# w111liang222/lidar-slam-detection

Measured on AMD Instinct MI355X. Metric: registered points/sec (120k-pt scan vs 1e7-pt map, full iterate-to-converge), higher is better.
Workload: dtype f32 per-point geometry / f64 transforms and reductions

## Files before the change

include/lio_hip.h:

```cpp
#ifndef LIO_HIP_H_
#define LIO_HIP_H_

#include <stdint.h>

#ifdef __cplusplus
extern "C" {
#endif

#define LIO_OK 0
#define LIO_E_INVALID (-1)
#define LIO_E_CAPACITY (-2)
#define LIO_E_DEVICE (-3)
#define LIO_E_STATE (-4)

typedef struct lio_map lio_map;
typedef struct lio_scan lio_scan;
typedef struct lio_engine lio_engine;

const char* lio_last_error(void);
const char* lio_last_warning(void);
int lio_device_count(void);
#define LIO_ABI_VERSION 26
int lio_abi_version(void);
void* lio_pinned_alloc(uint64_t bytes);
void lio_pinned_free(void* p);
uint64_t lio_map_bytes(const lio_map*);

lio_map* lio_map_create(int device, float resolution, uint64_t max_points, uint64_t max_voxels, int stencil);
void lio_map_destroy(lio_map*);
int lio_map_set_stencil(lio_map*, int stencil);
int lio_map_insert(lio_map*, const float* world_xyzi, uint64_t n, double travel);
int lio_map_insert_device(lio_map*, const void* d_world_xyzi, uint64_t n, double travel);
int lio_map_clear(lio_map*);
int lio_map_set_lru(lio_map*, uint64_t capacity_voxels, double max_distance);
int lio_map_lru_stats(lio_map*, uint64_t* n_evicted, uint64_t* n_interleaved);
int lio_map_lru_exact_stats(lio_map*, uint64_t* n_recreated, uint64_t* n_batches_not_followed);
int lio_map_set_tie_mode(lio_map*, int mode);
int lio_map_tie_stats(lio_map*, uint64_t* n_boundary_ties, uint64_t* n_unresolved);
int lio_map_pool_stats(lio_map*, uint64_t* pool_top, uint64_t* pool_cap);
int lio_map_stats(lio_map*, uint64_t* n_points, uint64_t* n_voxels);
uint64_t lio_map_knn_candidates(lio_map*);
uint64_t lio_map_knn_touched(lio_map*);
uint64_t lio_map_knn_unique(lio_map*);
int64_t lio_map_dump(lio_map*, float* out_xyzi, uint64_t cap_points);
int lio_map_knn(lio_map*, const float* world_xyzi, uint32_t n, float* out_pts, int32_t* out_cnt);

lio_scan* lio_scan_create(int device, uint32_t max_raw, uint32_t max_ds);
void lio_scan_destroy(lio_scan*);
int lio_scan_reset(lio_scan*);
int lio_scan_upload(lio_scan*, const float* body_xyzi, uint32_t n_raw);
int lio_scan_set_device(lio_scan*, const void* d_body_xyzi, uint32_t n_raw);
int lio_scan_undistort_delta(lio_scan*, const uint32_t* stamp_us, int stamps_on_device, const float delta_pose[16], double scan_period);
int lio_scan_download_raw(lio_scan*, float* out_xyzi, uint32_t cap);
int lio_scan_undistort_poses(lio_scan*, const uint32_t* stamp_us, int stamps_on_device, uint64_t header_stamp_us, const uint64_t* pose_stamp_us,
                             const double* pose_T, uint32_t n_poses);
int lio_scan_undistort_imu(lio_scan*, const uint32_t* stamp_us, int stamps_on_device, const double* poses, uint32_t n_poses, const double* end_pos3,
                           const double* end_rot_xyzw, const double* ril_xyzw, const double* til3, double blind, int filter_num, int undistort);
int lio_scan_voxel_downsample(lio_scan*, float leaf, int sync, uint32_t* n_ds);
int lio_scan_voxel_downsample_batch(lio_scan** scans, int n, float leaf, uint32_t* n_ds);
int lio_scan_set_ds(lio_scan*, const float* ds_body_xyzi, uint32_t n_ds);
int lio_scan_num_ds(lio_scan*);
int lio_scan_download_ds(lio_scan*, float* out_xyzi, uint32_t cap);
int lio_scan_download_world(lio_scan*, float* out_xyzi, uint32_t cap);
const void* lio_scan_ds_device(lio_scan*, uint32_t* n);
int lio_scan_download_match(lio_scan*, uint8_t* selected, float* normvec, int32_t* nn_cnt, float* nn_pts);

typedef struct lio_kernel_times {
    double knn_us, linearize_us, finalize_us;
    uint32_t knn_launches, linearize_launches, finalize_launches;
    uint32_t pad;
} lio_kernel_times;
int lio_scan_enable_kernel_timing(lio_scan*, int on);
int lio_scan_kernel_times(lio_scan*, lio_kernel_times* out, int reset);

typedef struct lio_normal_eq {
    double JtJ[36];
    double Jtr[6];
    double nnT[9];
    double eigvec[9];
    double eigval[3];
    double contri[3];
    double strong[3];
    double sum_abs_res;
    uint32_t n_eff;
    uint32_t n_ds;
    uint32_t n_knn_candidates_lo, n_knn_candidates_hi;
    uint32_t n_tie;
    uint32_t seq;
} lio_normal_eq;

int lio_p2plane_linearize(lio_map*, lio_scan*, const double pose_wi[7], const double ext_il[7], int redo_knn,
                          lio_normal_eq* out);
int lio_scan_set_degeneracy_mode(lio_scan*, int mode);
int lio_p2plane_degeneracy(lio_scan*, const double V[9], double contri[3], double strong[3]);
int lio_p2plane_rows(lio_scan*, const double pose_wi[7], const double ext_il[7], double* h_x6, double* h, uint32_t cap_rows);
int lio_map_incremental(lio_map*, lio_scan*, const double pose_wi[7], const double ext_il[7], float map_leaf,
                        int ekf_inited, double travel);
int lio_map_seed(lio_map*, lio_scan*, const double pose_wi[7], const double ext_il[7], double travel);

lio_engine* lio_engine_create(int device, float resolution, int stencil, uint64_t max_points, uint64_t max_voxels,
                              uint32_t max_raw, uint32_t max_ds);
lio_engine* lio_engine_create_shared(lio_map* shared_map, uint32_t max_raw, uint32_t max_ds);
void lio_engine_destroy(lio_engine*);
lio_map* lio_engine_map(lio_engine*);
lio_scan* lio_engine_scan(lio_engine*);
// ... 19 lines not shown
    float downsample_us, knn_us, linearize_us, insert_us, total_device_us;
    float host_solve_us, total_wall_us;
    int32_t n_knn_pass, n_pass, n_ds, n_eff_last;
    int32_t n_added;
    uint64_t knn_candidates;
    float undistort_us;
    float imu_host_us;
} lio_timings;
int lio_engine_timings(lio_engine*, lio_timings* out);
int lio_engine_enable_timing(lio_engine*, int on);
int lio_engine_flush(lio_engine*);
#define LIO_MAIN_FIRST_SCAN 0
#define LIO_MAIN_SEEDED 1
#define LIO_MAIN_SKIPPED 2
#define LIO_MAIN_UPDATED 3
#define LIO_MAIN_IMU_INIT 4
#define LIO_MAIN_IDLE 5
int lio_fastlio_init(lio_engine*, const double extT[3], const double extR[9], int filter_num, int max_point_num, double scan_period,
                     int undistort);
int lio_fastlio_is_init(lio_engine*);
int lio_fastlio_imu_enqueue(lio_engine*, double stamp, const double gyr[3], const double acc_ms2[3]);
int lio_engine_set_device_loop(lio_engine*, int on);

int lio_fastlio_ins_enqueue(lio_engine*, double stamp, const double vel_imu[3]);
int lio_fastlio_set_wheelspeed(lio_engine*, int enable);
int lio_fastlio_pcl_enqueue(lio_engine*, const float* xyzi, const uint32_t* stamp_us, uint32_t n, double header_stamp);
int lio_fastlio_pcl_stage(lio_engine*, uint32_t n, float** xyzi, uint32_t** stamp_us);
int lio_fastlio_pcl_commit(lio_engine*, uint32_t n, double header_stamp);
int lio_fastlio_pcl_enqueue_device(lio_engine*, const void* d_xyzi, const void* d_stamp_us, uint32_t n, double header_stamp);
int lio_fastlio_main(lio_engine*);
int lio_fastlio_odometry(lio_engine*, double odom_s[16], double odom_e[16]);
int lio_fastlio_state(lio_engine*, double out[20]);
int lio_fastlio_start_state(lio_engine*, double s26[26]);
int lio_fastlio_download_undistorted(lio_engine*, float* out_xyzi, uint32_t cap, uint32_t* n);
typedef int (*lio_meas_fn)(void* ctx, const double* s26, int converge, int* n, double* rows6, double* h, int cap);
int lio_eskf_update_cb(const double s26[26], const double P[529], double R, int max_iter, lio_meas_fn fn, void* ctx, int cap, double s26_out[26],
                       double P_out[529]);
int lio_eskf_update_ws_cb(const double s26[26], const double P[529], double R, int max_iter, lio_meas_fn fn, void* ctx, int cap, const double* ins_vel,
                          int degenerate, double s26_out[26], double P_out[529]);
int lio_state_predict(const double s26[26], const double P[529], double dt, const double Q[12], const double acc[3], const double gyro[3],
                      double s26_out[26], double P_out[529]);
typedef int (*lio_sums_fn)(void* ctx, const double* s26, int converge, double* acc29);
typedef void (*lio_degeneracy_fn)(void* ctx, const double* V9, double* cs6);
int lio_eskf_update_sums_cb(const double s26[26], const double P[529], double R, int max_iter, int degenerate_detect_en, lio_sums_fn fn,
                            lio_degeneracy_fn dfn, void* ctx, double s26_out[26], double P_out[529], lio_pass_log* logs, int cap_logs, int* status);

typedef void (*lio_reduce_fn)(void* ctx, double* buf, int n);
int lio_engine_set_reduce_hook(lio_engine*, lio_reduce_fn fn, void* ctx);
typedef struct lio_comm lio_comm;
int lio_comm_unique_id(uint8_t id[128]);
lio_comm* lio_comm_init(int device, int rank, int world, const uint8_t id[128]);
void lio_comm_destroy(lio_comm*);
int lio_comm_rank(const lio_comm*);
int lio_comm_world(const lio_comm*);
int lio_allgather_normal_eq(lio_comm*, const double* d_local32, double* d_gathered, double* d_sum32, void* stream);
int lio_allgather_records(lio_comm*, const double* d_local, double* d_gathered, uint32_t n_records, void* stream);
int lio_comm_stats(lio_comm*, uint64_t* n_collectives, double* total_us);
int lio_engine_set_joint(lio_engine* e, lio_engine** others, int n_others, lio_comm* comm);
int lio_engine_joint_register(lio_engine* e, const float* raw_body_xyzi, uint32_t n_raw, double lidar_beg_time, double state26[26], double cov[529]);
int lio_engine_joint_register_device(lio_engine* e, const void* d_raw_body_xyzi, uint32_t n_raw, double lidar_beg_time, double state26[26], double cov[529]);
#define LIO_JOB_KEEP_CACHE 1u
#define LIO_JOB_IDLE 2u
#define LIO_JOB_HOST_RAW 4u
#define LIO_JOB_FLAGS_KNOWN 7u
typedef struct lio_scan_job {
    const void* d_raw;
    uint32_t n_raw;
    uint32_t flags;
    double lidar_beg_time;
    const double* state_in;
    const double* cov_in;
    double* state_out;
    int32_t rc;
    int32_t n_ds, n_pass, n_knn_pass;
} lio_scan_job;
int lio_engines_process_batch(lio_engine** engines, int n_engines, lio_scan_job* jobs, int n_jobs);
typedef struct lio_batch lio_batch;
typedef struct lio_batch_result {
    double state[26];
    int32_t status;
    int32_t n_pass, n_knn_pass, n_ds, n_eff, degenerate, radix_passes, err;
    int32_t loop_i, loop_t, loop_converge, pad;
    uint32_t seq, pad2;
} lio_batch_result;
lio_batch* lio_batch_create(lio_map* shared_map, int n_slots, int n_groups, uint32_t max_raw, uint32_t max_ds);
lio_batch* lio_batch_create_joint(lio_map** sub_maps, int n_sub_maps, lio_comm* comm, int n_slots, int n_groups, uint32_t max_raw, uint32_t max_ds);
typedef int (*lio_gather_fn)(void* ctx, const double* d_local, double* d_gathered, uint32_t n_records, void* stream);
int lio_batch_set_gather_hook(lio_batch*, lio_gather_fn fn, void* ctx, int rank, int world);
int lio_batch_exchange_stats(lio_batch*, uint32_t* chunk_points, uint64_t* jobs_rerun, uint64_t* bytes_per_rank_and_round);
lio_batch* lio_batch_create_sequences(int device, float resolution, int stencil, uint64_t max_points, uint64_t max_voxels, int n_slots, int n_groups,
                                      uint32_t max_raw, uint32_t max_ds);
int lio_batch_sequences_step(lio_batch*, lio_scan_job* jobs, int n_jobs, double* cov_out);
int lio_batch_fastlio_main(lio_batch*, int* rc_out);
void lio_batch_destroy(lio_batch*);
int lio_batch_process(lio_batch*, lio_scan_job* jobs, int n_jobs);
typedef struct lio_batch_times {
    double downsample_us, knn_us, linearize_us, step_us;
    uint32_t downsample_launches, knn_launches, linearize_launches, step_launches;
    double insert_us;
    uint32_t insert_launches, pad;
} lio_batch_times;
int lio_batch_enable_kernel_timing(lio_batch*, int on);
int lio_batch_kernel_times(lio_batch*, lio_batch_times* out, int reset);
lio_engine* lio_batch_engine(lio_batch*, int group, int slot);
int lio_engine_set_static_map(lio_engine*, int on);

typedef struct lio_ndt lio_ndt;
lio_ndt* lio_ndt_create(int device, float resolution, int search_method, uint64_t max_points, uint64_t max_voxels, uint32_t max_source_points);
void lio_ndt_destroy(lio_ndt*);
int lio_ndt_set_target(lio_ndt*, const float* xyzi, uint64_t n);
int lio_ndt_set_target_device(lio_ndt*, const void* d_xyzi, uint64_t n);
int lio_ndt_num_voxels(lio_ndt*);
int lio_ndt_voxel_at(lio_ndt*, const float p[3], float mean[3], float cinv[9]);
int lio_ndt_linearize(lio_ndt*, lio_scan* source, const double T[16], int update_corr, int with_derivatives, double H[36], double b[6],
                      double* err, uint32_t* n_corr);
int lio_ndt_fitness_score(lio_ndt*, lio_scan* source, const double T[16], double max_range, double* score, uint32_t* n_inliers);
int lio_ndt_overlap_score(lio_ndt*, lio_scan* source, const double relpose[16], double max_range, double xy_range, double min_z, double* score,
                          double* inlier_ratio);
typedef struct lio_ndt_times {
    double cost_us;
    uint64_t launches, update_launches, pairs, source_points;
} lio_ndt_times;
int lio_ndt_enable_kernel_timing(lio_ndt*, int on);
int lio_ndt_kernel_times(lio_ndt*, lio_ndt_times* out, int reset);
typedef struct lio_ndt_params {
    int32_t max_iterations;
    int32_t lm_max_iterations;
    double rotation_epsilon_deg;
    double transformation_epsilon;
    double lm_init_lambda_factor;
    double max_process_time_ms;
} lio_ndt_params;
void lio_ndt_default_params(lio_ndt_params*);
int lio_ndt_align(lio_ndt*, lio_scan* source, const double guess[16], const lio_ndt_params* params, double out[16], int* iterations,
                  int* converged);

typedef struct lio_align_job {
    lio_ndt* target;
    lio_scan* source;
    const double* guess;
    double out[16];
    int32_t iterations, converged, evaluations, rc;
} lio_align_job;
int lio_ndt_align_batch(lio_ndt*, lio_align_job* jobs, int n_jobs, const lio_ndt_params* params);

typedef struct lio_gicp lio_gicp;
lio_gicp* lio_gicp_create(int device, float grid_resolution, uint32_t max_points, int k_correspondences);
void lio_gicp_destroy(lio_gicp*);
int lio_gicp_set_target(lio_gicp*, const float* xyzi, uint32_t n);
int lio_gicp_set_source(lio_gicp*, const float* xyzi, uint32_t n);
int lio_gicp_set_target_device(lio_gicp*, const void* d_xyzi, uint32_t n);
int lio_gicp_set_source_device(lio_gicp*, const void* d_xyzi, uint32_t n);
int lio_gicp_set_voxel_mode(lio_gicp*, double voxel_resolution, int search_method);
int lio_gicp_voxel_at(lio_gicp*, const float p[3], double mean[3], double cov6[6]);
int lio_gicp_download(lio_gicp*, int which, float* xyzi, double* cov6, uint32_t cap);
int lio_gicp_correspondences(lio_gicp*, int32_t* corr, uint32_t cap);
int lio_gicp_neighbours(lio_gicp*, int which, int32_t* idx, uint32_t cap_points);
int lio_gicp_mahalanobis(lio_gicp*, double* maha6, uint32_t cap);
int lio_gicp_linearize(lio_gicp*, const double T[16], double max_corr_dist, int update_corr, int with_derivatives, double H[36], double b[6], double* err,
                       uint32_t* n_corr);
int lio_gicp_align(lio_gicp*, const double guess[16], const lio_ndt_params* params, double max_corr_dist, double out[16], int* iterations, int* converged);
int lio_gicp_fitness_score(lio_gicp*, const double T[16], double max_range, double* score, uint32_t* nr);

typedef struct lio_pose_estimator lio_pose_estimator;
typedef struct lio_gps_observation {
    double T[16];
    double precision;
    int32_t dimension;
} lio_gps_observation;
lio_pose_estimator* lio_pose_estimator_create(const float imu_ext[16], uint64_t stamp_us, const float pos[3], const float quat_wxyz[4],
                                              double cool_time_duration);
void lio_pose_estimator_destroy(lio_pose_estimator*);
int lio_pose_estimator_predict(lio_pose_estimator*, uint64_t stamp_us, const float acc[3], const float gyro[3]);
int lio_pose_estimator_match(lio_pose_estimator*, lio_ndt* target, lio_scan* source, const lio_ndt_params* params, float observation[7],
                             int* iterations);
int lio_pose_estimator_match_gps(lio_pose_estimator*, lio_ndt* target, lio_scan* source, const lio_ndt_params* params, const lio_gps_observation* gps,
                                 float observation[7], float observation_cov[49], int* iterations);
int lio_pose_estimator_guess(lio_pose_estimator*, const lio_gps_observation* gps, float init_guess[16]);
// ... 568 lines not shown
```

lidar-slam-detection_amd/csrc/batch.hip:

```cpp
#include <sched.h>
#include <stdlib.h>

#include <chrono>
#include <deque>
#include <vector>

#include "eskf.h"
#include "lio_common.h"

using namespace lio;

int engine_resume_update(lio_engine* e, const double* x_now26, const double* x_prop26, const double* P_prop, int i, int converge, int t);
void engine_count_passes(lio_engine* e, int* n_pass, int* n_knn);
int engine_joint_register_device(lio_engine* e, const void* d_raw, uint32_t n_raw, double lidar_beg_time, double state26[26], double cov[529]);
struct lio_comm;
extern "C" int lio_comm_world(const lio_comm*);
extern "C" {
int engine_seq_prepare(lio_engine* e, uint32_t n_raw, double lidar_beg_time, int* ekf_inited);
void engine_seq_params(lio_engine* e, double* laser_cov, int* maximum_iter, int* degenerate_detect_en, float* leaf_surf, float* leaf_map, int* static_map,
                       double* travel, double last_pos_lid[3]);
int engine_seq_finish(lio_engine* e, const double x26[26], const double P529[529], int n_ds, int n_pass, int n_knn, int n_eff, int degenerate, int inserted,
                      uint32_t n_add, uint32_t map_err, uint32_t bound);
int engine_seq_resume(lio_engine* e, const double* x_now26, const double* x_prop26, const double* P_prop, int i, int converge, int t);
int engine_seq_has_lru(lio_engine* e);
int engine_fastlio_front(lio_engine* e, const void** d_raw, uint32_t* n_raw, double* beg, double state26[26], double cov529[529]);
void engine_fastlio_back(lio_engine* e);
}

namespace {

struct Group {
    hipStream_t stream = nullptr;
    std::vector<lio_engine*> eng;
    std::vector<lio_engine*> sub_eng;
    double* d_local32 = nullptr;
    double* d_gathered = nullptr;
    char* d_ds_send = nullptr;
    char* d_ds_all = nullptr;
    int ds_world = 0;
    MapRef* d_rowmaps = nullptr;
    std::vector<MapRef> rowmap_rows;
    char* d_block = nullptr;
    char* h_block = nullptr;
    size_t block_bytes = 0;
    SlotDesc* d_desc = nullptr;
    SlotDesc* h_desc = nullptr;
    EskfDev* d_ctrl = nullptr;
    EskfDev* h_ctrl = nullptr;
    hipGraphExec_t exec[5] = {nullptr, nullptr, nullptr, nullptr, nullptr};
    const void* graph_table = nullptr;
    int graph_stencil = 0;
    lio_batch_result* h_res = nullptr;
    lio_batch_result* h_res_dev = nullptr;
    std::vector<int> job_of_slot;
    float4* d_rawbuf = nullptr;
    MapRef* d_maps = nullptr;
    MapRef* h_maps = nullptr;
    SeqDev* d_seq = nullptr;
    SeqDev* h_seq = nullptr;
    std::vector<int> seq_path;
    int any_lru = 0;
    int n_active = 0;
    int launched_passes = 4;
    uint32_t seq = 0;
    uint32_t max_n_raw = 0;
    BatchTimer* bt = nullptr;
};

}

struct lio_batch {
    lio_map* map = nullptr;
    int device = 0;
    int n_slots = 0;
    uint32_t max_raw = 0, max_ds = 0;
    int pred_passes = 4;
    bool broken = false;
    int use_graph = 1;
    int count_touched = 0;
    std::vector<lio_map*> maps;
    lio_comm* comm = nullptr;
    int world = 1;
    int rank = 0;
    int split_ds = 1;
    uint32_t ds_cap = 0;
    uint32_t ds_seen_max = 0;
    bool ds_cap_full = false;
    uint64_t n_ds_cut = 0;
    int (*gather_hook)(void*, const double*, double*, uint32_t, void*) = nullptr;
    void* gather_ctx = nullptr;
    bool joint = false;
    bool sequences = false;
    std::vector<lio_scan_job> fl_jobs;
    std::vector<double> fl_state, fl_cov;
    std::vector<Group> groups;
    double t_submit = 0, t_wait = 0, t_collect = 0;
    uint64_t n_rounds = 0;
};

static void fill_mapref(MapRef& r, const lio_map* m);

namespace {

const MapRef* joint_rowmaps(lio_batch* b, Group& g) {
    const int M = (int)b->maps.size(), B = b->n_slots;
    if (M < 2) return nullptr;
    for (int m = 1; m < M; m++)
        if (b->maps[m]->stencil_id != b->maps[0]->stencil_id || b->maps[m]->stencil.n != b->maps[0]->stencil.n) return nullptr;
    std::vector<MapRef> now((size_t)M);
    for (int m = 0; m < M; m++) {
        memset(&now[m], 0, sizeof(MapRef));
        fill_mapref(now[m], b->maps[m]);
    }
    bool fresh = g.d_rowmaps != nullptr && (int)g.rowmap_rows.size() == M;
    for (int m = 0; m < M && fresh; m++) fresh = memcmp(&g.rowmap_rows[m], &now[m], sizeof(MapRef)) == 0;
    if (fresh) return g.d_rowmaps;
    std::vector<MapRef> rows((size_t)M * B);
    for (int m = 0; m < M; m++)
        for (int s = 0; s < B; s++) rows[(size_t)m * B + s] = now[m];
    if (!g.d_rowmaps && hipMalloc(reinterpret_cast<void**>(&g.d_rowmaps), sizeof(MapRef) * rows.size()) != hipSuccess) { g.d_rowmaps = nullptr; return nullptr; }
    if (hipMemcpyAsync(g.d_rowmaps, rows.data(), sizeof(MapRef) * rows.size(), hipMemcpyHostToDevice, g.stream) != hipSuccess) return nullptr;
    if (hipStreamSynchronize(g.stream) != hipSuccess) return nullptr;
    g.rowmap_rows = now;
    return g.d_rowmaps;
}

void fill_desc(SlotDesc& d, lio_scan* sc, EskfDev* d_ctrl, lio_batch_result* d_res) {
    d.max_ds = sc->max_ds;
    d.partial_blocks = sc->partial_blocks;
    d.sd = sc->dev;
    d.keys_a = sc->keys_a; d.keys_b = sc->keys_b; d.vals_a = sc->vals_a; d.vals_b = sc->vals_b;
    d.hist = sc->hist; d.blockcnt = sc->blockcnt; d.hpos = sc->hpos; d.longlist = sc->longlist; d.tie_list = sc->tie_list;
    d.sorted = sc->sorted; d.ds_body = sc->ds_body; d.ds_world = sc->ds_world; d.nn_pts = sc->nn_pts; d.normvec = sc->normvec;
    d.nn_cnt = sc->nn_cnt; d.selected = sc->selected; d.partial = sc->partial;
    d.host_nds = sc->host_nds_dev;
    d.ctrl = d_ctrl;
    d.result = d_res;
}

void fill_ctrl(EskfDev& c, const double* x26, const double* P529, double R, int max_iter, int degenerate_detect_en, int joint = 0) {
    c.joint = joint;
    memcpy(c.x, x26, sizeof(double) * 26);
    memcpy(c.P, P529, sizeof(double) * 529);
    for (int k = 0; k < kEkN; k++) c.limit[k] = 0.001;
    c.R = R;
    c.maximum_iter = max_iter;
    c.degenerate_detect_en = degenerate_detect_en;
    c.is_degenerate = 0;
    ek_begin(c);
}

void group_free(Group& g) {
    for (lio_engine* e : g.eng) lio_engine_destroy(e);
    for (lio_engine* e : g.sub_eng) lio_engine_destroy(e);
    if (g.d_local32) hipFree(g.d_local32);
    if (g.d_gathered) hipFree(g.d_gathered);
    if (g.d_ds_send) hipFree(g.d_ds_send);
    if (g.d_ds_all) hipFree(g.d_ds_all);
    if (g.d_rowmaps) hipFree(g.d_rowmaps);
    for (int k = 0; k < 5; k++)
        if (g.exec[k]) hipGraphExecDestroy(g.exec[k]);
    if (g.d_block) hipFree(g.d_block);
    if (g.d_rawbuf) hipFree(g.d_rawbuf);
    if (g.h_block) hipHostFree(g.h_block);
    if (g.d_seq) hipFree(g.d_seq);
    if (g.h_seq) hipHostFree(g.h_seq);
    if (g.h_res) hipHostFree(g.h_res);
    if (g.stream) hipStreamDestroy(g.stream);
    if (g.bt) {
        if (g.bt->created)
            for (int c = 0; c < BatchTimer::kClasses; c++)
                for (int i = 0; i < BatchTimer::kPool; i++) { hipEventDestroy(g.bt->ev[c][i][0]); hipEventDestroy(g.bt->ev[c][i][1]); }
        delete g.bt;
    }
}

const float4* stage_host_raw(lio_batch* b, Group& g, int slot, const lio_scan_job& job, int* rc) {
    *rc = LIO_OK;
    if (!g.d_rawbuf) {
        if (hipMalloc(reinterpret_cast<void**>(&g.d_rawbuf), sizeof(float4) * (size_t)b->max_raw * (size_t)b->n_slots) != hipSuccess) {
            set_error("lio_batch: no memory for the raw ring of LIO_JOB_HOST_RAW jobs (%d x %u points)", b->n_slots, b->max_raw);
            *rc = LIO_E_DEVICE;
            return nullptr;
        }
    }
    float4* dst = g.d_rawbuf + (size_t)slot * b->max_raw;
    if (hipMemcpyAsync(dst, job.d_raw, sizeof(float4) * (size_t)job.n_raw, hipMemcpyHostToDevice, g.stream) != hipSuccess) {
        set_error("lio_batch: copy of a LIO_JOB_HOST_RAW cloud failed: %s", hipGetErrorString(hipGetLastError()));
        *rc = LIO_E_DEVICE;
        return nullptr;
    }
    return dst;
}

int submit(lio_batch* b, Group& g, lio_scan_job* jobs, int first, int n, int passes) {
    const int B = b->n_slots;
    g.seq++;
    g.n_active = 0;
    g.max_n_raw = 0;
    g.launched_passes = passes;
    for (int s = 0; s < B; s++) {
        SlotDesc& d = g.h_desc[s];
        d.active = 0;
        g.job_of_slot[s] = -1;
        if (s >= n) continue;
        lio_scan_job& job = jobs[first + s];
        g.job_of_slot[s] = first + s;
        job.rc = LIO_E_INVALID;
        job.n_ds = job.n_pass = job.n_knn_pass = 0;
        if (job.flags & ~LIO_JOB_FLAGS_KNOWN) { set_error("lio_scan_job.flags = 0x%x: unknown bits (a job array that was not zero-initialised?)", job.flags); continue; }
        if (job.flags & LIO_JOB_IDLE) { job.rc = 0; g.job_of_slot[s] = -1; continue; }
        if (!job.state_in || !job.cov_in || (!job.d_raw && job.n_raw)) continue;
        if (job.n_raw > b->max_raw) { set_error("scan of %u points exceeds max_raw %u", job.n_raw, b->max_raw); job.rc = LIO_E_CAPACITY; continue; }
        if (job.n_raw == 0) { job.rc = 2; continue; }
        d.raw = static_cast<const float4*>(job.d_raw);
        if (job.flags & LIO_JOB_HOST_RAW) {
            int src = LIO_OK;
            d.raw = stage_host_raw(b, g, s, job, &src);
            if (src != LIO_OK) { job.rc = src; continue; }
        }
        d.n_raw = job.n_raw;
        d.nblocks = (job.n_raw + 2047u) / 2048u;
        d.active = 1;
        d.seq = g.seq;
        d.min_ds = 5;
        d.reset_cache = (job.flags & LIO_JOB_KEEP_CACHE) ? 0u : 1u;
        fill_ctrl(g.h_ctrl[s], job.state_in, job.cov_in, 0.001 , 4, 1, b->joint ? 1 : 0);
        g.h_res[s].seq = g.seq - 1;
        g.n_active++;
        if (job.n_raw > g.max_n_raw) g.max_n_raw = job.n_raw;
    }
    const int M = (int)b->maps.size();
    for (int m = 1; m < M; m++)
        for (int s = 0; s < B; s++) {
            SlotDesc& d = g.h_desc[(size_t)m * B + s];
            const SlotDesc& p = g.h_desc[s];
            d.raw = p.raw; d.n_raw = p.n_raw; d.nblocks = p.nblocks; d.active = p.active; d.seq = p.seq; d.min_ds = p.min_ds; d.reset_cache = p.reset_cache;
        }
    if (g.n_active == 0) return LIO_OK;
    const bool timed = g.bt && g.bt->on;
    const MapRef* rowmaps = b->joint ? joint_rowmaps(b, g) : nullptr;
    auto enqueue = [&](BatchTimer* bt) -> int {
        LIO_HIP_TRY(hipMemcpyAsync(g.d_block, g.h_block, g.block_bytes, hipMemcpyHostToDevice, g.stream));
        const uint32_t ds_bound = b->max_raw < b->max_ds ? b->max_raw : b->max_ds;
        int rc = LIO_OK;
        if (b->joint && b->world > 1 && b->split_ds) {
            const int per = (B + b->world - 1) / b->world;
            const int s0 = std::min(B, b->rank * per), s1 = std::min(B, s0 + per);
            if (g.ds_world != b->world) {
                if (g.d_ds_send) hipFree(g.d_ds_send);
                if (g.d_ds_all) hipFree(g.d_ds_all);
                g.d_ds_send = g.d_ds_all = nullptr;
                g.ds_world = 0;
                const size_t chunk = (size_t)per * ds_exchange_slot_bytes(ds_bound);
                LIO_HIP_TRY(hipMalloc(reinterpret_cast<void**>(&g.d_ds_send), chunk));
                LIO_HIP_TRY(hipMalloc(reinterpret_cast<void**>(&g.d_ds_all), chunk * (size_t)b->world));
                g.ds_world = b->world;
            }
            if (bt) bt->begin(0);
            if (s1 > s0) rc = vg_downsample_batch(g.stream, g.d_desc + s0, s1 - s0, b->max_raw, b->max_ds, 0.5f, passes);
            if (bt) bt->end(0);
            if (rc != LIO_OK) return rc;
            if (b->ds_cap == 0) {
                const char* k = getenv("LIO_JOINT_DS_CAP");
                const uint32_t want = k ? (uint32_t)strtoul(k, nullptr, 10) : ((ds_bound / 4u + 1023u) & ~1023u);
                b->ds_cap = std::min(ds_bound, std::max(k ? 1u : 4096u, want));
            }
            const uint32_t cap = b->ds_cap_full ? ds_bound : b->ds_cap;
            rc = p2plane_batch_exchange_ds(b->comm, b->world, b->gather_hook, b->gather_ctx, g.stream, g.d_desc, B, per, s0, s1, cap, g.d_ds_send, g.d_ds_all);
            if (rc == LIO_OK && s0 > 0) rc = scan_begin_rows(g.stream, g.d_desc, s0);
            if (rc == LIO_OK && s1 < B) rc = scan_begin_rows(g.stream, g.d_desc + s1, B - s1);
            if (rc != LIO_OK) return rc;
        } else {
            if (bt) bt->begin(0);
            rc = vg_downsample_batch(g.stream, g.d_desc, B, b->max_raw, b->max_ds, 0.5f, passes);
            if (bt) bt->end(0);
            if (rc != LIO_OK) return rc;
        }
        if (b->joint) {
            rc = p2plane_batch_share(g.stream, g.d_desc, B, M, ds_bound);
            if (rc == LIO_OK) rc = scan_begin_rows(g.stream, g.d_desc + B, B * (M - 1));
            if (rc != LIO_OK) return rc;
            return p2plane_batch_update_joint(b->maps.data(), M, b->comm, b->world, b->gather_hook, b->gather_ctx, g.stream, g.d_desc, B, ds_bound, 5, g.d_local32, g.d_gathered, bt,
                                              rowmaps);
        }
        return p2plane_batch_update(b->map, g.stream, g.d_desc, B, ds_bound, 5, bt, bt ? b->count_touched : 0);
    };
    if (!b->use_graph || timed || b->joint) return enqueue(timed ? g.bt : nullptr);
    if (g.graph_table != b->map->table || g.graph_stencil != b->map->stencil.n) {
        for (int k = 0; k < 5; k++)
            if (g.exec[k]) { hipGraphExecDestroy(g.exec[k]); g.exec[k] = nullptr; }
        g.graph_table = b->map->table;
        g.graph_stencil = b->map->stencil.n;
    }
    if (!g.exec[passes]) {
        hipGraph_t graph = nullptr;
        LIO_HIP_TRY(hipStreamBeginCapture(g.stream, hipStreamCaptureModeThreadLocal));
        const int rc = enqueue(nullptr);
        const hipError_t e2 = hipStreamEndCapture(g.stream, &graph);
        if (rc != LIO_OK) { if (graph) hipGraphDestroy(graph); return rc; }
        LIO_HIP_TRY(e2);
        LIO_HIP_TRY(hipGraphInstantiate(&g.exec[passes], graph, nullptr, nullptr, 0));
        hipGraphDestroy(graph);
    }
    LIO_HIP_TRY(hipGraphLaunch(g.exec[passes], g.stream));
    return LIO_OK;
}

int wait_group(Group& g, int B) {
    for (int s = 0; s < B; s++) {
        if (!g.h_desc[s].active) continue;
        volatile uint32_t* seq = &g.h_res[s].seq;
        for (uint64_t spin = 0; *seq != g.seq; spin++) {
            __builtin_ia32_pause();
            if (spin > 2000 && (spin & 31) == 0) sched_yield();
            if (spin > 40000000ull) {
                LIO_HIP_TRY(hipStreamSynchronize(g.stream));
                if (*seq != g.seq) { set_error("batch slot %d did not report (seq %u, expected %u)", s, *seq, g.seq); return LIO_E_DEVICE; }
                break;
            }
        }
    }
    __atomic_thread_fence(__ATOMIC_ACQUIRE);
    return LIO_OK;
}

}


extern "C" {

static lio_batch* batch_create_impl(lio_map** maps, int n_maps, lio_comm* comm, int n_slots, int n_groups, uint32_t max_raw, uint32_t max_ds) {
    lio_map* map = n_maps > 0 && maps ? maps[0] : nullptr;
    if (!map || n_maps > 64 || n_slots < 1 || n_slots > 256 || n_groups < 1 || n_groups > 8 || max_raw == 0 || max_ds == 0) { set_error("lio_batch_create: bad argument"); return nullptr; }
    for (int m = 1; m < n_maps; m++)
        if (!maps[m] || maps[m]->device != map->device) { set_error("lio_batch_create_joint: the sub-maps of a batch live on one device"); return nullptr; }
    if (hipSetDevice(map->device) != hipSuccess) { set_error("lio_batch_create: no HIP device %d", map->device); return nullptr; }
    lio_batch* b = new lio_batch();
    b->map = map;
    b->device = map->device;
    b->n_slots = n_slots;
    b->max_raw = max_raw;
    b->max_ds = max_ds;
    b->maps.assign(maps, maps + n_maps);
    b->comm = comm;
    b->world = comm ? lio_comm_world(comm) : 1;
    b->rank = comm ? lio_comm_rank(comm) : 0;
    { const char* k = getenv("LIO_JOINT_SPLIT_DS"); b->split_ds = (k && k[0] == '0') ? 0 : 1; }
    b->joint = n_maps > 1 || comm != nullptr;
    b->groups.resize(n_groups);
    { const char* k = getenv("LIO_BATCH_GRAPH"); b->use_graph = (k && k[0] == '0') ? 0 : 1; }
    bool ok = true;
    const int M = n_maps;
    for (Group& g : b->groups) ok = ok && hipStreamCreateWithFlags(&g.stream, hipStreamNonBlocking) == hipSuccess;
    for (Group& g : b->groups) {
        g.job_of_slot.assign(n_slots, -1);
        const size_t desc_bytes = sizeof(SlotDesc) * (size_t)n_slots * (size_t)M;
        g.block_bytes = desc_bytes + sizeof(EskfDev) * (size_t)n_slots;
        ok = ok && hipMalloc(reinterpret_cast<void**>(&g.d_block), g.block_bytes) == hipSuccess;
        ok = ok && hipHostMalloc(reinterpret_cast<void**>(&g.h_block), g.block_bytes, hipHostMallocDefault) == hipSuccess;
        if (ok) {
            g.d_desc = reinterpret_cast<SlotDesc*>(g.d_block);
            g.h_desc = reinterpret_cast<SlotDesc*>(g.h_block);
            g.d_ctrl = reinterpret_cast<EskfDev*>(g.d_block + desc_bytes);
            g.h_ctrl = reinterpret_cast<EskfDev*>(g.h_block + desc_bytes);
        }
        ok = ok && hipHostMalloc(reinterpret_cast<void**>(&g.h_res), sizeof(lio_batch_result) * n_slots, hipHostMallocMapped) == hipSuccess;
        ok = ok && hipHostGetDevicePointer(reinterpret_cast<void**>(&g.h_res_dev), g.h_res, 0) == hipSuccess;
        if (b->joint) {
            ok = ok && hipMalloc(reinterpret_cast<void**>(&g.d_local32), sizeof(double) * 32 * n_slots) == hipSuccess;
            ok = ok && hipMalloc(reinterpret_cast<void**>(&g.d_gathered), sizeof(double) * 32 * n_slots * (size_t)b->world) == hipSuccess;
        }
        if (!ok) break;
        memset(g.h_block, 0, g.block_bytes);
        memset(g.h_res, 0, sizeof(lio_batch_result) * n_slots);
        ok = hipMemset(g.d_block, 0, g.block_bytes) == hipSuccess;
        for (int s = 0; s < n_slots && ok; s++) {
            lio_engine* e = lio_engine_create_shared(map, max_raw, max_ds);
            if (!e) { ok = false; break; }
            lio_engine_set_flags(e, 1, 0, 0.0, -10.0);
            g.eng.push_back(e);
            fill_desc(g.h_desc[s], lio_engine_scan(e), &g.d_ctrl[s], &g.h_res_dev[s]);
        }
        for (int m = 1; m < M && ok; m++)
            for (int s = 0; s < n_slots && ok; s++) {
                lio_engine* e = lio_engine_create_shared(maps[m], max_raw, max_ds);
                if (!e) { ok = false; break; }
                lio_engine_set_flags(e, 1, 0, 0.0, -10.0);
                g.sub_eng.push_back(e);
                fill_desc(g.h_desc[(size_t)m * n_slots + s], lio_engine_scan(e), &g.d_ctrl[s], nullptr);
            }
        for (int s = 0; s < n_slots && ok && b->joint; s++) {
            std::vector<lio_engine*> others;
            for (int m = 1; m < M; m++) others.push_back(g.sub_eng[(size_t)(m - 1) * n_slots + s]);
            ok = lio_engine_set_joint(g.eng[s], others.empty() ? nullptr : others.data(), (int)others.size(), comm) == LIO_OK;
        }
    }
    if (!ok) {
        set_error("lio_batch_create: device setup failed: %s", hipGetErrorString(hipGetLastError()));
        lio_batch_destroy(b);
        return nullptr;
    }
    {
        const char* q = getenv("GPU_MAX_HW_QUEUES");
        if (n_groups > 1 && (!q || atoi(q) < 8))
            set_warning("lio_batch_create: GPU_MAX_HW_QUEUES=%s -- with fewer than 8 hardware queues the %d rounds in flight mostly serialise (~20 %% slower); "
                        "export GPU_MAX_HW_QUEUES=8 before the process's first HIP call", q ? q : "(unset: 4)", n_groups);
    }
    return b;
}

lio_batch* lio_batch_create(lio_map* map, int n_slots, int n_groups, uint32_t max_raw, uint32_t max_ds) {
    return batch_create_impl(&map, map ? 1 : 0, nullptr, n_slots, n_groups, max_raw, max_ds);
}

lio_batch* lio_batch_create_joint(lio_map** sub_maps, int n_sub_maps, lio_comm* comm, int n_slots, int n_groups, uint32_t max_raw, uint32_t max_ds) {
    return batch_create_impl(sub_maps, n_sub_maps, comm, n_slots, n_groups, max_raw, max_ds);
}

int lio_batch_set_gather_hook(lio_batch* b, lio_gather_fn fn, void* ctx, int rank, int world) {
    if (!b || !fn || world < 1 || rank < 0 || rank >= world) return LIO_E_INVALID;
    if (!b->joint || b->comm) { set_error("lio_batch_set_gather_hook: for a batch made by lio_batch_create_joint without a communicator"); return LIO_E_STATE; }
    hipSetDevice(b->map->device);
    for (auto& g : b->groups) {
        LIO_HIP_TRY(hipStreamSynchronize(g.stream));
        if (g.d_gathered) hipFree(g.d_gathered);
        g.d_gathered = nullptr;
        LIO_HIP_TRY(hipMalloc(reinterpret_cast<void**>(&g.d_gathered), sizeof(double) * 32 * b->n_slots * (size_t)world));
    }
    b->gather_hook = fn;
    b->gather_ctx = ctx;
    b->world = world;
    b->rank = rank;
    return LIO_OK;
}

int lio_batch_exchange_stats(lio_batch* b, uint32_t* chunk_points, uint64_t* jobs_rerun, uint64_t* bytes_per_rank_and_round) {
    if (!b) return LIO_E_INVALID;
    const bool on = b->joint && b->world > 1 && b->split_ds;
    if (chunk_points) *chunk_points = on ? b->ds_cap : 0u;
    if (jobs_rerun) *jobs_rerun = b->n_ds_cut;
    if (bytes_per_rank_and_round) {
        const int per = (b->n_slots + b->world - 1) / b->world;
        *bytes_per_rank_and_round = on && b->ds_cap ? (uint64_t)per * ds_exchange_slot_bytes(b->ds_cap) : 0u;
    }
    return LIO_OK;
}

void lio_batch_destroy(lio_batch* b) {
    if (!b) return;
    hipSetDevice(b->device);
    if (getenv("LIO_BATCH_PROFILE") && b->n_rounds)
        fprintf(stderr, "lio_batch: %llu rounds of %d slots; host per round: submit %.1f us, wait %.1f us, collect %.1f us\n", (unsigned long long)b->n_rounds,
                b->n_slots, 1e6 * b->t_submit / b->n_rounds, 1e6 * b->t_wait / b->n_rounds, 1e6 * b->t_collect / b->n_rounds);
    for (Group& g : b->groups) {
        if (g.stream) hipStreamSynchronize(g.stream);
        group_free(g);
    }
    delete b;
}

int lio_batch_enable_kernel_timing(lio_batch* b, int on) {
    if (!b) return LIO_E_INVALID;
    hipSetDevice(b->device);
    for (Group& g : b->groups) {
        if (!g.bt) { g.bt = new BatchTimer(); g.bt->stream = g.stream; }
        if (on && !g.bt->created) {
            for (int c = 0; c < BatchTimer::kClasses; c++)
                for (int i = 0; i < BatchTimer::kPool; i++) {
                    LIO_HIP_TRY(hipEventCreate(&g.bt->ev[c][i][0]));
                    LIO_HIP_TRY(hipEventCreate(&g.bt->ev[c][i][1]));
                }
            g.bt->created = true;
        }
        g.bt->on = on != 0;
    }
    b->count_touched = (on & 2) ? 1 : 0;
    if (b->count_touched && b->map) { const int rc = map_enable_touch_bits(b->map); if (rc != LIO_OK) return rc; }
    return LIO_OK;
}

int lio_batch_kernel_times(lio_batch* b, lio_batch_times* out, int reset) {
    if (!b || !out) return LIO_E_INVALID;
    memset(out, 0, sizeof(*out));
    for (Group& g : b->groups) {
        if (!g.bt) continue;
        out->downsample_us += g.bt->us[0]; out->knn_us += g.bt->us[1]; out->linearize_us += g.bt->us[2]; out->step_us += g.bt->us[3];
        out->downsample_launches += g.bt->launches[0]; out->knn_launches += g.bt->launches[1]; out->linearize_launches += g.bt->launches[2];
        out->step_launches += g.bt->launches[3];
        out->insert_us += g.bt->us[4];
        out->insert_launches += g.bt->launches[4];
        if (reset)
            for (int c = 0; c < BatchTimer::kClasses; c++) { g.bt->us[c] = 0; g.bt->launches[c] = 0; }
    }
    return LIO_OK;
}

lio_engine* lio_batch_engine(lio_batch* b, int group, int slot) {
    if (!b || group < 0 || group >= (int)b->groups.size() || slot < 0 || slot >= b->n_slots) return nullptr;
    return b->groups[group].eng[slot];
}

int lio_batch_process(lio_batch* b, lio_scan_job* jobs, int n_jobs) {
    if (!b || (!jobs && n_jobs) || n_jobs < 0) return LIO_E_INVALID;
    if (b->sequences) { set_error("lio_batch_process: a sequence batch is driven by lio_batch_sequences_step"); return LIO_E_STATE; }
    hipSetDevice(b->device);
    const int B = b->n_slots;
    int next = 0, first_err = 0;
    std::deque<int> inflight;
    std::vector<int> retry;
    auto note = [&](int rc) { if (rc < 0 && !first_err) first_err = rc; };
    auto collect = [&](Group& g) {
        int need_max = 1;
        for (int s = 0; s < B; s++) {
            const int j = g.job_of_slot[s];
            if (j < 0) continue;
            if (!g.h_desc[s].active) { note(jobs[j].rc); continue; }
            lio_scan_job& job = jobs[j];
            const lio_batch_result& r = g.h_res[s];
            if (r.radix_passes > need_max) need_max = r.radix_passes;
            if (r.radix_passes > g.launched_passes) { retry.push_back(j); continue; }
            lio_engine* e = g.eng[s];
            lio_scan* sc = lio_engine_scan(e);
            sc->have_ds = r.n_ds;
            sc->n_raw = g.h_desc[s].n_raw;
            job.n_ds = r.n_ds;
            job.n_pass = r.n_pass;
            job.n_knn_pass = r.n_knn_pass;
            if (r.err & 4) {
                hipMemsetAsync(&sc->dev->err, 0, 4, g.stream);
                b->n_ds_cut++;
                retry.push_back(j);
                continue;
            }
            if (r.err & 1) {
                set_error("downsampled scan exceeds max_ds %u", b->max_ds);
                hipMemsetAsync(&sc->dev->err, 0, 4, g.stream);
                job.rc = LIO_E_CAPACITY;
                note(job.rc);
                continue;
            }
            if ((uint32_t)r.n_ds > b->ds_seen_max) b->ds_seen_max = (uint32_t)r.n_ds;
            if (r.status == EK_SKIPPED) { job.rc = 2; continue; }
            if (r.status == EK_NEEDS_HOST && b->joint && b->gather_hook) {
                set_error("lio_batch (gather hook mode): a scan needs the host-driven joint path, which only exists over a lio_comm");
                job.rc = LIO_E_STATE;
                note(job.rc);
                continue;
            }
            if (r.status == EK_NEEDS_HOST && b->joint) {
                if (!(job.flags & LIO_JOB_KEEP_CACHE)) {
                    scan_forget_cache(sc);
                    for (int m = 1; m < (int)b->maps.size(); m++) scan_forget_cache(lio_engine_scan(g.sub_eng[(size_t)(m - 1) * B + s]));
                }
                double st26[26], cov[529];
                memcpy(st26, job.state_in, sizeof(st26));
                memcpy(cov, job.cov_in, sizeof(cov));
                const void* d_cloud = (job.flags & LIO_JOB_HOST_RAW) ? static_cast<const void*>(g.d_rawbuf + (size_t)s * b->max_raw) : job.d_raw;
                const int rc = engine_joint_register_device(e, d_cloud, job.n_raw, job.lidar_beg_time, st26, cov);
                if (rc < 0) { job.rc = rc; note(rc); continue; }
                engine_count_passes(e, &job.n_pass, &job.n_knn_pass);
                if (job.state_out) memcpy(job.state_out, st26, sizeof(st26));
                job.rc = rc;
                continue;
            }
            if (r.status == EK_NEEDS_HOST) {
                const int rc = engine_resume_update(e, r.state, job.state_in, job.cov_in, r.loop_i, r.loop_converge, r.loop_t);
                if (rc != LIO_OK) { job.rc = rc; note(rc); continue; }
                int np = 0, nk = 0;
                engine_count_passes(e, &np, &nk);
                job.n_pass += np;
                job.n_knn_pass += nk;
                if (job.state_out) lio_engine_get_state(e, job.state_out);
                job.rc = 3;
                continue;
            }
            if (job.state_out) memcpy(job.state_out, r.state, sizeof(double) * 26);
            job.rc = 3;
        }
        if (need_max > 4) need_max = 4;
        b->pred_passes = need_max;
        if (b->joint && b->world > 1 && b->split_ds && b->ds_seen_max && !getenv("LIO_JOINT_DS_CAP")) {
            const uint32_t ds_bound = b->max_raw < b->max_ds ? b->max_raw : b->max_ds;
            const uint32_t want = (b->ds_seen_max + b->ds_seen_max / 4u + 1023u) & ~1023u;
            b->ds_cap = std::min(ds_bound, std::max(4096u, want));
        }
    };
    using clk = std::chrono::steady_clock;
    auto secs = [](clk::time_point a, clk::time_point c) { return std::chrono::duration<double>(c - a).count(); };
    auto bail = [&](int rc) {
        for (auto& gg : b->groups) hipStreamSynchronize(gg.stream);
        inflight.clear();
        return rc;
    };
    for (size_t gi = 0; gi < b->groups.size() && next < n_jobs; gi++) {
        const int n = n_jobs - next < B ? n_jobs - next : B;
        const auto t0 = clk::now();
        const int rc = submit(b, b->groups[gi], jobs, next, n, b->pred_passes);
        b->t_submit += secs(t0, clk::now());
        b->n_rounds++;
        if (rc != LIO_OK) return bail(rc);
        next += n;
        inflight.push_back((int)gi);
    }
    while (!inflight.empty()) {
        const int gi = inflight.front();
        inflight.pop_front();
        Group& g = b->groups[gi];
        const auto t0 = clk::now();
        if (g.n_active) {
            const int rc = wait_group(g, B);
            if (rc != LIO_OK) return bail(rc);
        }
        if (g.bt && g.bt->on) { hipStreamSynchronize(g.stream); g.bt->resolve(); }
        const auto t1 = clk::now();
        collect(g);
        const auto t2 = clk::now();
        b->t_wait += secs(t0, t1);
        b->t_collect += secs(t1, t2);
        if (next < n_jobs) {
            const int n = n_jobs - next < B ? n_jobs - next : B;
            const int rc = submit(b, g, jobs, next, n, b->pred_passes);
            b->t_submit += secs(t2, clk::now());
            b->n_rounds++;
            if (rc != LIO_OK) return bail(rc);
            next += n;
            inflight.push_back(gi);
        }
    }
    const std::vector<int> todo = retry;
    retry.clear();
    b->ds_cap_full = true;
    for (const int j : todo) {
        Group& g = b->groups[0];
        int rc = submit(b, g, jobs, j, 1, 4);
        if (rc == LIO_OK && g.n_active) rc = wait_group(g, B);
        if (rc != LIO_OK) { b->ds_cap_full = false; return bail(rc); }
        collect(g);
    }
    b->ds_cap_full = false;
    for (const int j : retry) { jobs[j].rc = LIO_E_DEVICE; note(LIO_E_DEVICE); }
    return first_err;
}

static void fill_mapref(MapRef& r, const lio_map* m) {
    r.table = m->table; r.cap = m->cap; r.pending = m->pending; r.created = m->created; r.pool = m->pool; r.pool_seq = m->pool_seq; r.tie_mode = m->tie_mode; r.md = m->dev;
    r.slot_of_point = m->slot_of_point; r.stage = m->stage; r.pool_cap = m->pool_cap;
    r.touch = m->touch; r.prev_touch = m->prev_touch; r.lru_log = m->lru_log; r.log_mask = m->lru_log_cap ? m->lru_log_cap - 1 : 0;
    r.free_items = m->free_items; r.free_in = m->free_in; r.free_cap = m->free_cap;
    r.first_touch = m->first_touch; r.lru_g = m->lru_g; r.lru_rec = m->lru_rec;
    r.lru_capacity = (uint32_t)m->lru_capacity; r.lru_max_distance = m->lru_max_distance;
    r.mask = m->table_mask; r.inv_res = m->inv_res; r.res = m->res; r.key_mode = m->key_mode; r.max_voxels = (uint32_t)m->max_voxels;
    r.stencil_id = m->stencil_id;
}

lio_batch* lio_batch_create_sequences(int device, float resolution, int stencil, uint64_t max_points, uint64_t max_voxels, int n_slots, int n_groups,
                                      uint32_t max_raw, uint32_t max_ds) {
    if (n_slots < 1 || n_slots > 256 || n_groups < 1 || n_groups > 8 || max_raw == 0 || max_ds == 0 || max_points == 0 || max_voxels == 0) {
        set_error("lio_batch_create_sequences: bad argument");
        return nullptr;
    }
    const uint32_t ds_bound = max_raw < max_ds ? max_raw : max_ds;
    if (ds_bound > max_points || ds_bound > (1u << 20)) { set_error("lio_batch_create_sequences: a scan's %u downsampled points exceed the maps' insert scratch", ds_bound); return nullptr; }
    if (hipSetDevice(device) != hipSuccess) { set_error("lio_batch_create_sequences: no HIP device %d", device); return nullptr; }
    lio_batch* b = new lio_batch();
    b->device = device;
    b->n_slots = n_slots;
    b->max_raw = max_raw;
    b->max_ds = max_ds;
    b->sequences = true;
    { const char* k = getenv("LIO_BATCH_GRAPH"); b->use_graph = (k && k[0] == '0') ? 0 : 1; }
    b->groups.resize(n_groups);
    bool ok = true;
    for (Group& g : b->groups) ok = ok && hipStreamCreateWithFlags(&g.stream, hipStreamNonBlocking) == hipSuccess;
    for (Group& g : b->groups) {
        g.job_of_slot.assign(n_slots, -1);
        g.seq_path.assign(n_slots, 0);
        const size_t desc_bytes = sizeof(SlotDesc) * (size_t)n_slots, ctrl_bytes = sizeof(EskfDev) * (size_t)n_slots;
        g.block_bytes = desc_bytes + ctrl_bytes + sizeof(MapRef) * (size_t)n_slots;
        ok = ok && hipMalloc(reinterpret_cast<void**>(&g.d_block), g.block_bytes) == hipSuccess;
        ok = ok && hipHostMalloc(reinterpret_cast<void**>(&g.h_block), g.block_bytes, hipHostMallocDefault) == hipSuccess;
        ok = ok && hipMalloc(reinterpret_cast<void**>(&g.d_seq), sizeof(SeqDev) * (size_t)n_slots) == hipSuccess;
        ok = ok && hipHostMalloc(reinterpret_cast<void**>(&g.h_seq), sizeof(SeqDev) * (size_t)n_slots, hipHostMallocDefault) == hipSuccess;
        ok = ok && hipHostMalloc(reinterpret_cast<void**>(&g.h_res), sizeof(lio_batch_result) * n_slots, hipHostMallocMapped) == hipSuccess;
        ok = ok && hipHostGetDevicePointer(reinterpret_cast<void**>(&g.h_res_dev), g.h_res, 0) == hipSuccess;
        if (!ok) break;
        g.d_desc = reinterpret_cast<SlotDesc*>(g.d_block);
        g.h_desc = reinterpret_cast<SlotDesc*>(g.h_block);
        g.d_ctrl = reinterpret_cast<EskfDev*>(g.d_block + desc_bytes);
        g.h_ctrl = reinterpret_cast<EskfDev*>(g.h_block + desc_bytes);
        g.d_maps = reinterpret_cast<MapRef*>(g.d_block + desc_bytes + ctrl_bytes);
        g.h_maps = reinterpret_cast<MapRef*>(g.h_block + desc_bytes + ctrl_bytes);
        memset(g.h_block, 0, g.block_bytes);
        memset(g.h_res, 0, sizeof(lio_batch_result) * n_slots);
        memset(g.h_seq, 0, sizeof(SeqDev) * (size_t)n_slots);
        ok = hipMemset(g.d_block, 0, g.block_bytes) == hipSuccess && hipMemset(g.d_seq, 0, sizeof(SeqDev) * (size_t)n_slots) == hipSuccess;
        for (int s = 0; s < n_slots && ok; s++) {
            lio_engine* e = lio_engine_create(device, resolution, stencil, max_points, max_voxels, max_raw, max_ds);
            if (!e) { ok = false; break; }
            lio_engine_set_device_loop(e, 1);
            g.eng.push_back(e);
            fill_desc(g.h_desc[s], lio_engine_scan(e), &g.d_ctrl[s], &g.h_res_dev[s]);
        }
    }
    if (!ok) {
        set_error("lio_batch_create_sequences: device setup failed: %s", hipGetErrorString(hipGetLastError()));
        lio_batch_destroy(b);
        return nullptr;
    }
    b->map = lio_engine_map(b->groups[0].eng[0]);
    return b;
}

int lio_batch_sequences_step(lio_batch* b, lio_scan_job* jobs, int n_jobs, double* cov_out) {
    if (!b || !jobs) return LIO_E_INVALID;
    if (!b->sequences) { set_error("lio_batch_sequences_step: for a batch made by lio_batch_create_sequences"); return LIO_E_STATE; }
    if (b->broken) { set_error("lio_batch_sequences_step: an earlier step failed after part of it had run on the device; the sessions' maps hold that sweep, their engines do not -- destroy the batch"); return LIO_E_STATE; }
    const int B = b->n_slots, G = (int)b->groups.size();
    if (n_jobs != B * G) { set_error("lio_batch_sequences_step: %d jobs for %d sessions (job j is the next scan of session j; LIO_JOB_IDLE marks a session without one)", n_jobs, B * G); return LIO_E_INVALID; }
    hipSetDevice(b->device);
    int first_err = 0;
// ... 352 lines not shown
```

lidar-slam-detection_amd/csrc/lio_common.h:

```cpp
#pragma once
#include <hip/hip_runtime.h>
#include <stdint.h>
#include <stdio.h>
#include <string.h>

#include "../../include/lio_hip.h"
#include "eskf_dev.h"

struct LruEntry;

namespace lio {

#if defined(__HIP_DEVICE_COMPILE__)
#define LIO_PIN4(r) asm volatile("" : "+v"((r).x), "+v"((r).y), "+v"((r).z), "+v"((r).w))
#define LIO_PIN1(r) asm volatile("" : "+v"(r))
#else
#define LIO_PIN4(r) ((void)(r))
#define LIO_PIN1(r) ((void)(r))
#endif
__host__ __device__ __forceinline__ void pin_loaded(float4& r) { LIO_PIN4(r); }
__host__ __device__ __forceinline__ void pin_loaded(uint4& r) { LIO_PIN4(r); }
__host__ __device__ __forceinline__ void pin_loaded(uint32_t& r) { LIO_PIN1(r); }
__host__ __device__ __forceinline__ void pin_loaded(float& r) { LIO_PIN1(r); }

template <int CTRL>
__device__ inline double dpp_f64(double v) {
    const unsigned long long u = (unsigned long long)__double_as_longlong(v);
    const uint32_t lo = (uint32_t)__builtin_amdgcn_update_dpp(0, (int)(uint32_t)u, CTRL, 0xF, 0xF, false);
    const uint32_t hi = (uint32_t)__builtin_amdgcn_update_dpp(0, (int)(uint32_t)(u >> 32), CTRL, 0xF, 0xF, false);
    return __longlong_as_double((long long)(((unsigned long long)hi << 32) | lo));
}

void set_error(const char* fmt, ...);
void set_warning(const char* fmt, ...);

#define LIO_HIP_TRY(expr)                                                                         \
    do {                                                                                          \
        hipError_t e__ = (expr);                                                                  \
        if (e__ != hipSuccess) {                                                                  \
            ::lio::set_error("%s:%d: %s -> %s", __FILE__, __LINE__, #expr, hipGetErrorString(e__)); \
            return LIO_E_DEVICE;                                                                  \
        }                                                                                         \
    } while (0)

constexpr uint64_t kEmptyKey = 0xFFFFFFFFFFFFFFFFull;
constexpr uint64_t kTombKey = 0xFFFFFFFFFFFFFFFEull;
constexpr uint32_t kNoIdx = 0xFFFFFFFFu;
constexpr int kMaxStencil = 75;
constexpr int kLinThreads = 64;
constexpr int kAcc = 29;

struct __attribute__((aligned(16))) Slot {
    unsigned long long key;
    uint32_t ptr;
    uint32_t cnt;
};

struct MapDev {
    unsigned long long pool_top;
    unsigned long long n_points;
    uint32_t n_voxels;
    uint32_t err;
    uint32_t n_add;
    uint32_t n_tombs;
    unsigned long long log_head, log_tail, log_head_prev;
    unsigned long long n_evicted;
    unsigned long long n_lru_interleaved;
    unsigned long long n_lru_recreated;
    unsigned long long n_lru_inexact;
    int free_top[24];
    int free_in_top[24];
    uint32_t seq_cur;
    uint32_t seq_acc;
    unsigned long long n_tie_boundary;
    unsigned long long n_tie_unresolved;
    uint32_t* touch_bits;
    unsigned long long knn_cand[64 * 16];
};

struct PoseArgs {
    double qw[4];
    double tw[3];
    double ql[4];
    double tl[3];
};

struct ScanDev {
    uint32_t bbox_min[3];
    uint32_t bbox_max[3];
    uint32_t n_valid;
    uint32_t n_long;
    uint32_t n_tie;
    uint32_t n_tie_done;
    uint32_t lin_ticket;
    uint32_t seq;
    uint32_t n_ds;
    uint32_t n_ds_prev;
    uint32_t cache_n;
    uint32_t passthrough;
    uint32_t nbits;
    uint32_t err;
    int32_t minb[3];
    int32_t mul1, mul2;
    uint32_t total_cells;
    uint32_t n_monster;
};

struct StencilArgs {
    int n;
    signed char off[kMaxStencil][3];
};

struct SlotDesc {
    const float4* raw;
    uint32_t n_raw;
    uint32_t nblocks;
    uint32_t active;
    uint32_t seq;
    uint32_t max_ds, partial_blocks;
    uint32_t min_ds;
    uint32_t reset_cache;
    ScanDev* sd;
    uint32_t *keys_a, *keys_b, *vals_a, *vals_b, *hist, *blockcnt, *hpos, *longlist, *tie_list;
    float4 *sorted, *ds_body, *ds_world, *nn_pts, *normvec;
    int32_t* nn_cnt;
    uint8_t* selected;
    double* partial;
    uint32_t* host_nds;
    EskfDev* ctrl;
    lio_batch_result* result;
};

struct MapRef {
    Slot* table;
    uint32_t* cap;
    uint32_t* pending;
    float* created;
    float4* pool;
    uint32_t* pool_seq;
    MapDev* md;
    uint32_t* slot_of_point;
    float4* stage;
    unsigned long long pool_cap;
    unsigned long long stamp_base;
    unsigned long long* touch;
    unsigned long long* prev_touch;
    struct ::LruEntry* lru_log;
    unsigned long long log_mask;
    uint32_t* free_items;
    uint32_t* free_in;
    unsigned long long* first_touch;
    uint32_t* lru_g;
    uint32_t* lru_rec;
    uint32_t free_cap;
    uint32_t lru_capacity;
    float lru_max_distance;
    uint32_t mask;
    float inv_res, res;
    int key_mode;
    uint32_t max_voxels;
    int tie_mode;
    int stencil_id;
    uint32_t do_insert;
    uint32_t ekf_inited;
    float map_leaf;
    double travel_prev;
    double last_pos_lid[3];
};

struct SeqDev {
    double travel;
    uint32_t go;
    uint32_t map_err;
    uint32_t n_add;
    uint32_t n_voxels;
    unsigned long long n_points;
    double P[kEkN * kEkN];
};

}

struct LruEntry {
    unsigned long long stamp;
    uint32_t slot, pad;
};
constexpr int kStampIdxBits = 26;
constexpr unsigned long long kStampIdxMask = (1ull << kStampIdxBits) - 1ull;
constexpr uint32_t kLruRecCap = 4096;

struct lio_map {
    uint64_t lru_capacity;
    float lru_max_distance;
    unsigned long long* touch;
    unsigned long long* prev_touch;
    LruEntry* lru_log;
    uint64_t lru_log_cap;
    uint32_t* free_items;
    uint32_t* free_in;
    unsigned long long* first_touch;
    uint32_t *lru_g, *lru_rec;
    uint32_t free_cap;
    uint64_t tomb_bound;
    lio::Slot* table2;
    uint32_t *cap2, *pending2, *remap;
    float* created2;
    unsigned long long *touch2, *prev_touch2;
    int device;
    hipStream_t stream;
    float res, inv_res;
    int key_mode;
    uint64_t max_points, max_voxels, pool_cap;
    uint32_t table_cap, table_mask;
    lio::Slot* table;
// ... 17 lines not shown
    lio::StencilArgs stencil;
    int stencil_id;
    int own_stream;
    uint64_t n_batches;
    uint64_t bytes;
};

namespace lio {
struct KernelTimer;
namespace ground {
const float4* inliers_view(lio_ground* g, uint32_t* n);
}
}
struct lio_scan {
    lio::KernelTimer* kt;
    int force_degeneracy;
    int device;
    hipStream_t stream;
    uint32_t max_raw, max_ds;
    uint32_t n_raw;
    const float4* raw;
    float4* raw_own;
    float4* ds_body;
    float4* ds_world;
    float4* nn_pts;
    int32_t* nn_cnt;
    uint8_t* selected;
    float4* normvec;
    uint32_t *keys_a, *keys_b, *vals_a, *vals_b;
    uint32_t* hist;
    uint32_t* blockcnt;
    uint32_t* hpos;
    uint32_t* longlist;
    uint32_t* tie_list;
    float4* sorted;
    double* partial;
    uint32_t partial_blocks;
    lio::ScanDev* dev;
    lio::ScanDev* host_dev;
    lio_normal_eq* d_result;
    uint32_t* host_nds;
    int pred_passes;
    lio::SlotDesc* d_batch_desc = nullptr;
    lio::SlotDesc* h_batch_desc = nullptr;
    uint32_t batch_desc_cap = 0;
    uint32_t* host_nds_dev;
    lio_normal_eq* h_result;
    lio_normal_eq* h_result_dev;
    uint32_t seq_expected;
    int have_ds;
    uint32_t resize_min;
    uint64_t bytes;
};

namespace lio {
constexpr int kMaxImuPoses = 128;
struct ImuPoseDev {
    double off;
    double acc[3], gyr[3], vel[3], pos[3], R[9];
};
struct UndistortArgs {
    double pos_e[3], rot_e[4], ril[4], til[3];
    double blind2;
    int n_poses, filter_num, undistort;
};
struct DeltaArgs {
    float t[3];
    float aa[3];
    double scan_period;
};
constexpr int kMaxPoseList = 64;
struct PoseListArgs {
    int n_poses;
    unsigned long long limit[kMaxPoseList];
    DeltaArgs d[kMaxPoseList];
};
int undistort_poses_launch(hipStream_t stream, const float4* d_in, const uint32_t* d_stamp_us, uint32_t n, float4* d_out, const PoseListArgs& args,
                           uint32_t* d_tile_max);
int undistort_delta_launch(hipStream_t stream, const float4* d_in, const uint32_t* d_stamp_us, uint32_t n, float4* d_out, const DeltaArgs& args);
int undistort_launch(hipStream_t stream, const float4* d_in, const uint32_t* d_stamp_us, uint32_t n, float4* d_out, const ImuPoseDev* d_poses,
                     const UndistortArgs& args, unsigned long long* d_block_min );

int vg_downsample(lio_scan* s, float leaf, int passes );
int vg_downsample_batch(hipStream_t st, const SlotDesc* d_slots, int n_slots, uint32_t max_raw, uint32_t max_ds, float leaf, int passes);
int knn_batch_launch(lio_map* m, hipStream_t st, const SlotDesc* d_slots, int n_slots, uint32_t grid_x, int count_touched);
struct BatchTimer {
    static constexpr int kClasses = 5;
    static constexpr int kPool = 256;
    hipEvent_t ev[kClasses][kPool][2];
    int used[kClasses] = {0, 0, 0, 0, 0};
    double us[kClasses] = {0, 0, 0, 0, 0};
    uint32_t launches[kClasses] = {0, 0, 0, 0, 0};
    bool on = false, created = false;
    hipStream_t stream = nullptr;
    void begin(int c) { if (on && used[c] < kPool) hipEventRecord(ev[c][used[c]][0], stream); }
    void end(int c) { if (on && used[c] < kPool) { hipEventRecord(ev[c][used[c]][1], stream); used[c]++; } }
    void resolve() {
        for (int c = 0; c < kClasses; c++) {
            for (int i = 0; i < used[c]; i++) {
                float ms = 0.f;
                if (hipEventElapsedTime(&ms, ev[c][i][0], ev[c][i][1]) == hipSuccess) { us[c] += (double)ms * 1000.0; launches[c]++; }
            }
            used[c] = 0;
        }
    }
};
int p2plane_batch_update(lio_map* m, hipStream_t st, const SlotDesc* d_slots, int n_slots, uint32_t ds_bound, int n_passes, BatchTimer* bt, int count_touched);
int knn_seq_launch(hipStream_t st, const MapRef* d_maps, const SlotDesc* d_slots, int n_slots, uint32_t grid_x, const StencilArgs* stencils, const int* stencil_ids,
                   int n_stencils);
int p2plane_seq_update(hipStream_t st, const MapRef* d_maps, const SlotDesc* d_slots, int n_slots, uint32_t ds_bound, int n_passes, const StencilArgs* stencils,
                       const int* stencil_ids, int n_stencils, BatchTimer* bt);
int p2plane_seq_insert(hipStream_t st, const MapRef* d_maps, const SlotDesc* d_slots, SeqDev* d_seq, int n_slots, uint32_t ds_bound, int any_lru);
int map_insert_seq(hipStream_t st, const MapRef* d_maps, const SeqDev* d_seq, int n_slots, uint32_t bound, int any_lru);
int map_rebuild(lio_map* m, hipStream_t stream);
}
struct lio_comm;
namespace lio {
int p2plane_batch_share(hipStream_t st, const SlotDesc* d_descs, int n_slots, int n_maps, uint32_t ds_bound);
int p2plane_batch_update_joint(lio_map** maps, int n_maps, ::lio_comm* comm, int world, int (*gather_hook)(void*, const double*, double*, uint32_t, void*), void* gather_ctx, hipStream_t st, const SlotDesc* d_descs, int n_slots, uint32_t ds_bound,
                               int n_passes, double* d_local32, double* d_gathered, BatchTimer* bt, const MapRef* d_rowmaps = nullptr);
int scan_begin_rows(hipStream_t st, const SlotDesc* d_descs, int n_rows);
size_t ds_exchange_slot_bytes(uint32_t cap);
int p2plane_batch_exchange_ds(::lio_comm* comm, int world, int (*gather_hook)(void*, const double*, double*, uint32_t, void*), void* gather_ctx, hipStream_t st,
                              const SlotDesc* d_descs, int n_slots, int per, int s0, int s1, uint32_t cap, char* d_send, char* d_all);
int scan_begin(lio_scan* s);
int scan_set_nds(lio_scan* s, uint32_t n);
void kt_begin(lio_scan* s, int which);
void kt_end(lio_scan* s, int which);
int map_enable_touch_bits(lio_map* m);
lio_map* map_create_mode(int device, float resolution, uint64_t max_points, uint64_t max_voxels, int stencil, int key_mode);
int map_insert_dev(lio_map* m, hipStream_t stream, const float4* d_pts, uint64_t n, const uint32_t* d_n, double travel);
int map_knn_plane(lio_map* m, lio_scan* s, const PoseArgs& pose, int redo_knn);
int knn_batch(lio_map* m, const float4* d_q, uint32_t n, float4* d_out, int32_t* d_cnt, uint32_t* d_tie);
int map_knn_exact(lio_map* m, lio_scan* s, const PoseArgs& pose, uint32_t n_tie_host);
int p2plane_reduce(lio_map* m, lio_scan* s, const PoseArgs& pose, int redo_knn);
int p2plane_degeneracy(lio_scan* s);
int incremental_classify(lio_map* m, lio_scan* s, const PoseArgs& pose, float map_leaf, int ekf_inited, int seed_all);
PoseArgs make_pose(const double pose_wi[7], const double ext_il[7]);
}

extern "C" {
int p2plane_linearize_begin(lio_map* m, lio_scan* s, const double pose_wi[7], const double ext_il[7], int redo_knn);
int p2plane_linearize_end(lio_map* m, lio_scan* s, const double pose_wi[7], const double ext_il[7], int redo_knn, lio_normal_eq* out);
int scan_share_ds(lio_scan* dst, lio_scan* src, uint32_t n);
int scan_forget_cache(lio_scan* s);
int map_clear(lio_map* m);
int map_incremental_async(lio_map* m, lio_scan* s, const double pose_wi[7], const double ext_il[7], float map_leaf, int ekf_inited, double travel);
int map_settle(lio_map* m);
int map_settle_if_done(lio_map* m);
}
```

lidar-slam-detection_amd/csrc/p2plane.hip:

```cpp
#include "knn_dev.h"
#include "lio_common.h"

namespace lio {


__device__ inline void body_to_world_d(const PoseArgs& P, const float4 pb, double pi[3], float4& pw) {
    const double vx = (double)pb.x, vy = (double)pb.y, vz = (double)pb.z;
    double ux = P.ql[1] * vz - P.ql[2] * vy, uy = P.ql[2] * vx - P.ql[0] * vz, uz = P.ql[0] * vy - P.ql[1] * vx;
    ux += ux; uy += uy; uz += uz;
    double cx = P.ql[1] * uz - P.ql[2] * uy, cy = P.ql[2] * ux - P.ql[0] * uz, cz = P.ql[0] * uy - P.ql[1] * ux;
    pi[0] = ((vx + P.ql[3] * ux) + cx) + P.tl[0];
    pi[1] = ((vy + P.ql[3] * uy) + cy) + P.tl[1];
    pi[2] = ((vz + P.ql[3] * uz) + cz) + P.tl[2];
    ux = P.qw[1] * pi[2] - P.qw[2] * pi[1]; uy = P.qw[2] * pi[0] - P.qw[0] * pi[2]; uz = P.qw[0] * pi[1] - P.qw[1] * pi[0];
    ux += ux; uy += uy; uz += uz;
    cx = P.qw[1] * uz - P.qw[2] * uy; cy = P.qw[2] * ux - P.qw[0] * uz; cz = P.qw[0] * uy - P.qw[1] * ux;
    pw.x = (float)(((pi[0] + P.qw[3] * ux) + cx) + P.tw[0]);
    pw.y = (float)(((pi[1] + P.qw[3] * uy) + cy) + P.tw[1]);
    pw.z = (float)(((pi[2] + P.qw[3] * uz) + cz) + P.tw[2]);
    pw.w = pb.w;
}

__device__ inline bool esti_plane_dev(const float4 pt[5], float threshold, float pabcd[4]) {
    float A[5][3], b[5];
// ... 449 lines not shown
            if (comp < kAcc && l == 0) acc[comp] = s;
        }
    }
    __syncthreads();
    EK_STAMP(1);
    if (tid == 0) d.sd->n_tie = 0;
    const int log0 = c.n_log;
    if (skip) {
        if (tid == 0) c.status = EK_SKIPPED;
    } else if (tid < 64) {
        ek_measure_head(c, w, acc, c.converge);
        EK_STAMP(20);
        if constexpr (JOINT) {
            if (w.flag[1]) {
                if (tid == 0) { c.status = EK_NEEDS_HOST; c.n_pass--; if (c.converge) c.n_knn--; w.flag[0] = 0; w.flag[5] = 1; }
                EK_SYNC();
            } else {
                ek_measure_tail(c, w);
            }
        } else {
            if (!w.flag[1]) ek_measure_tail(c, w);
            EK_STAMP(21);
        }
    } else if (tid < 128) {
        ek_step_prep(c, w);
    }
    __syncthreads();
    EK_STAMP(2);
    if (!JOINT && !skip && w.flag[1]) {
        double s6[6] = {0, 0, 0, 0, 0, 0};
        for (uint32_t i = tid; i < n; i += kStepThreads) {
            if (!d.selected[i]) continue;
            const float4 nv = d.normvec[i];
            double f0 = (double)nv.x, f1 = (double)nv.y, f2 = (double)nv.z;
            const double nn = sqrt(f0 * f0 + f1 * f1 + f2 * f2);
            if (nn > 0) { f0 /= nn; f1 /= nn; f2 /= nn; }
#pragma unroll
            for (int e = 0; e < 3; e++) {
                const float dotp = (float)fabs(f0 * w.eigvec[0 * 3 + e] + f1 * w.eigvec[1 * 3 + e] + f2 * w.eigvec[2 * 3 + e]);
                if (dotp > 0.1736f) s6[e] += (double)dotp;
                if (dotp > 0.7070f) s6[3 + e] += (double)dotp;
            }
        }
#pragma unroll
        for (int e = 0; e < 6; e++) {
            const double v = wave_sum(s6[e]);
            if ((tid & 63) == 0) red6[tid >> 6][e] = v;
        }
        __syncthreads();
        if (tid < 6) {
            double v = 0.0;
            for (int k = 0; k < kStepThreads / 64; k++) v += red6[k][tid];
            w.cs[tid] = v;
        }
        __syncthreads();
        if (tid < 64) ek_measure_tail(c, w);
    }
    if (tid >= 64) return;
    EK_STAMP(3);
    if (!skip && c.status == EK_RUNNING && w.flag[0]) ek_step_solve(c, w);
    EK_SYNC();
    EK_STAMP(5);
    {
        const double* src = reinterpret_cast<const double*>(&c);
        double* dst = reinterpret_cast<double*>(&cg);
        for (int k = tid; k < kCoreWords; k += 64) dst[k] = src[k];
        constexpr int kLogWords = (int)(sizeof(EkPassLog) / 8);
        const int log1 = c.n_log < kEkMaxPass ? c.n_log : kEkMaxPass;
        for (int e = log0; e < log1 + (c.status == EK_NEEDS_HOST ? 1 : 0) && e < kEkMaxPass; e++) {
            const double* ls = reinterpret_cast<const double*>(&c.log[e]);
            double* ld = reinterpret_cast<double*>(&cg.log[e]);
            for (int k = tid; k < kLogWords; k += 64) ld[k] = ls[k];
        }
    }
    EK_STAMP(6);
    if (c.status != EK_RUNNING) {
        lio_batch_result* r = d.result;
        if (tid < 26) r->state[tid] = c.x[tid];
        if (tid == 32) {
            r->status = c.status; r->n_pass = c.n_pass; r->n_knn_pass = c.n_knn; r->n_ds = (int32_t)n;
            r->n_eff = c.n_eff_last; r->degenerate = c.is_degenerate; r->radix_passes = (int32_t)((d.sd->nbits + 7u) >> 3); r->err = (int32_t)d.sd->err;
            r->loop_i = c.i; r->loop_t = c.t; r->loop_converge = c.converge; r->pad = 0;
        }
        __threadfence_system();
        EK_SYNC();
        if (tid == 0) *reinterpret_cast<volatile uint32_t*>(&r->seq) = d.seq;
    }
    EK_STAMP(7);
}

#ifdef LIO_STEP_TRACE
extern "C" int lio_debug_step_trace(unsigned long long* out64, int reset) {
    hipDeviceSynchronize();
    if (hipMemcpyFromSymbol(out64, HIP_SYMBOL(g_ek_trace), 64 * sizeof(unsigned long long)) != hipSuccess) return -1;
    if (reset) { unsigned long long z[64] = {0}; hipMemcpyToSymbol(HIP_SYMBOL(g_ek_trace), z, sizeof(z)); }
    return 0;
}
#endif


__global__ void __launch_bounds__(256) share_ds_batch(const SlotDesc* __restrict__ descs, uint32_t n_slots) {
    const uint32_t slot = blockIdx.y % n_slots, m = 1u + blockIdx.y / n_slots;
    const SlotDesc& src = descs[slot];
    const SlotDesc& dst = descs[(size_t)m * n_slots + slot];
    if (!src.active) return;
    const uint32_t n = src.sd->n_ds;
    for (uint32_t i = blockIdx.x * blockDim.x + threadIdx.x; i < n; i += gridDim.x * blockDim.x) dst.ds_body[i] = src.ds_body[i];
    if (blockIdx.x == 0 && threadIdx.x == 0) {
        dst.sd->n_ds_prev = dst.sd->cache_n;
        dst.sd->n_ds = n;
        dst.sd->err = src.sd->err;
        dst.sd->n_tie = 0;
    }
}

int lio_allgather_records_internal(::lio_comm* c, const double* d_local, double* d_gathered, uint32_t n_records, hipStream_t st);
constexpr uint32_t kDsHdrBytes = 256;

__global__ void __launch_bounds__(256) pack_ds_batch(const SlotDesc* __restrict__ descs, uint32_t s0, char* __restrict__ send, size_t slot_bytes, uint32_t cap) {
    const SlotDesc& d = descs[s0 + blockIdx.y];
    char* chunk = send + (size_t)blockIdx.y * slot_bytes;
    uint32_t* hdr = reinterpret_cast<uint32_t*>(chunk);
    float4* pts = reinterpret_cast<float4*>(chunk + kDsHdrBytes);
    uint32_t n = d.active ? d.sd->n_ds : 0u;
    const bool cut = n > cap;
    if (cut) n = cap;
    if (blockIdx.x == 0 && threadIdx.x == 0) {
        hdr[0] = n;
        hdr[1] = d.active ? (d.sd->err | (cut ? 4u : 0u)) : 0u;
        hdr[2] = d.active ? d.sd->nbits : 0u;
        hdr[3] = d.active;
        if (cut) d.sd->err |= 4u;
    }
    for (uint32_t i = blockIdx.x * blockDim.x + threadIdx.x; i < n; i += gridDim.x * blockDim.x) pts[i] = d.ds_body[i];
}
__global__ void __launch_bounds__(256) unpack_ds_batch(const SlotDesc* __restrict__ descs, uint32_t s0, uint32_t s1, const char* __restrict__ all, size_t slot_bytes) {
    const uint32_t slot = blockIdx.y;
    if (slot >= s0 && slot < s1) return;
    const SlotDesc& d = descs[slot];
    if (!d.active) return;
    const char* chunk = all + (size_t)slot * slot_bytes;
    const uint32_t* hdr = reinterpret_cast<const uint32_t*>(chunk);
    const float4* pts = reinterpret_cast<const float4*>(chunk + kDsHdrBytes);
    const uint32_t n = hdr[0];
    for (uint32_t i = blockIdx.x * blockDim.x + threadIdx.x; i < n; i += gridDim.x * blockDim.x) d.ds_body[i] = pts[i];
    if (blockIdx.x == 0 && threadIdx.x == 0) {
        d.sd->n_ds_prev = d.sd->cache_n;
        d.sd->n_ds = n;
        d.sd->err = hdr[1];
        d.sd->nbits = hdr[2];
        d.sd->n_tie = 0;
    }
}

size_t ds_exchange_slot_bytes(uint32_t cap) { return ((size_t)kDsHdrBytes + (size_t)cap * sizeof(float4) + 255u) & ~(size_t)255u; }

int p2plane_batch_exchange_ds(::lio_comm* comm, int world, int (*gather_hook)(void*, const double*, double*, uint32_t, void*), void* gather_ctx, hipStream_t st,
                              const SlotDesc* d_descs, int n_slots, int per, int s0, int s1, uint32_t cap, char* d_send, char* d_all) {
    const size_t slot_bytes = ds_exchange_slot_bytes(cap);
    uint32_t bx = (cap + 255u) / 256u;
    if (bx > 64u) bx = 64u;
    if (bx == 0) bx = 1;
    if (s1 > s0) hipLaunchKernelGGL(pack_ds_batch, dim3(bx, (uint32_t)(s1 - s0)), 256, 0, st, d_descs, (uint32_t)s0, d_send, slot_bytes, cap);
    LIO_HIP_TRY(hipGetLastError());
    const size_t n_records = (size_t)per * slot_bytes / 256u;
    if (n_records > 0xFFFFFFFFull) { set_error("joint batch: a rank's share of a round's downsampled clouds exceeds the transport's record count"); return LIO_E_CAPACITY; }
// ... 369 lines not shown
```

lidar-slam-detection_amd/csrc/voxelgrid.hip:

```cpp
#include "device_prims.h"

namespace lio {

constexpr int kThreads = 256;
constexpr int kItems = 8;
constexpr int kTile = kThreads * kItems;
constexpr int kWaves = kThreads / 64;

__device__ __forceinline__ void vg_bbox_atomic_body(const float4* __restrict__ in, uint32_t n, ScanDev* sd) {
    float mn0 = INFINITY, mn1 = INFINITY, mn2 = INFINITY, mx0 = -INFINITY, mx1 = -INFINITY, mx2 = -INFINITY;
    uint32_t cnt = 0;
    const uint32_t stride = gridDim.x * blockDim.x;
    for (uint32_t i = blockIdx.x * blockDim.x + threadIdx.x; i < n; i += 4u * stride) {
        float4 q[4];
#pragma unroll
        for (int k = 0; k < 4; k++) {
            const uint32_t j = i + (uint32_t)k * stride;
            q[k] = in[j < n ? j : i];
        }
#pragma unroll
        for (int k = 0; k < 4; k++) {
            const float4 p = q[k];
            if (i + (uint32_t)k * stride < n && isfinite(p.x) && isfinite(p.y) && isfinite(p.z)) {
                mn0 = fminf(mn0, p.x); mx0 = fmaxf(mx0, p.x);
                mn1 = fminf(mn1, p.y); mx1 = fmaxf(mx1, p.y);
                mn2 = fminf(mn2, p.z); mx2 = fmaxf(mx2, p.z);
                cnt++;
            }
        }
    }
#pragma unroll
    for (int off = 32; off > 0; off >>= 1) {
        mn0 = fminf(mn0, __shfl_xor(mn0, off)); mx0 = fmaxf(mx0, __shfl_xor(mx0, off));
        mn1 = fminf(mn1, __shfl_xor(mn1, off)); mx1 = fmaxf(mx1, __shfl_xor(mx1, off));
        mn2 = fminf(mn2, __shfl_xor(mn2, off)); mx2 = fmaxf(mx2, __shfl_xor(mx2, off));
        cnt += __shfl_xor(cnt, off);
    }
    __shared__ float red[kWaves][6];
    __shared__ uint32_t redc[kWaves];
    const int wave = threadIdx.x >> 6, lane = threadIdx.x & 63;
    if (lane == 0) {
        red[wave][0] = mn0; red[wave][1] = mn1; red[wave][2] = mn2;
        red[wave][3] = mx0; red[wave][4] = mx1; red[wave][5] = mx2;
        redc[wave] = cnt;
    }
    __syncthreads();
    if (threadIdx.x == 0) {
        for (int w = 1; w < kWaves; w++) {
            mn0 = fminf(mn0, red[w][0]); mn1 = fminf(mn1, red[w][1]); mn2 = fminf(mn2, red[w][2]);
            mx0 = fmaxf(mx0, red[w][3]); mx1 = fmaxf(mx1, red[w][4]); mx2 = fmaxf(mx2, red[w][5]);
            cnt += redc[w];
        }
        if (cnt > 0) {
            atomicMin(&sd->bbox_min[0], f2ord(mn0)); atomicMax(&sd->bbox_max[0], f2ord(mx0));
            atomicMin(&sd->bbox_min[1], f2ord(mn1)); atomicMax(&sd->bbox_max[1], f2ord(mx1));
            atomicMin(&sd->bbox_min[2], f2ord(mn2)); atomicMax(&sd->bbox_max[2], f2ord(mx2));
            atomicAdd(&sd->n_valid, cnt);
        }
    }
}

__device__ __forceinline__ void vg_bbox_body(const float4* __restrict__ in, uint32_t n, uint32_t* __restrict__ parts) {
    float mn0 = INFINITY, mn1 = INFINITY, mn2 = INFINITY, mx0 = -INFINITY, mx1 = -INFINITY, mx2 = -INFINITY;
    uint32_t cnt = 0;
    const uint32_t base = blockIdx.x * kTile;
    float4 p[kItems];
#pragma unroll
    for (int r = 0; r < kItems; r++) {
        const uint32_t i = base + r * kThreads + threadIdx.x;
        if (i < n) p[r] = in[i];
    }
#pragma unroll
    for (int r = 0; r < kItems; r++) {
        const uint32_t i = base + r * kThreads + threadIdx.x;
        if (i < n && isfinite(p[r].x) && isfinite(p[r].y) && isfinite(p[r].z)) {
            mn0 = fminf(mn0, p[r].x); mx0 = fmaxf(mx0, p[r].x);
            mn1 = fminf(mn1, p[r].y); mx1 = fmaxf(mx1, p[r].y);
            mn2 = fminf(mn2, p[r].z); mx2 = fmaxf(mx2, p[r].z);
            cnt++;
        }
    }
#pragma unroll
    for (int off = 32; off > 0; off >>= 1) {
        mn0 = fminf(mn0, __shfl_xor(mn0, off)); mx0 = fmaxf(mx0, __shfl_xor(mx0, off));
        mn1 = fminf(mn1, __shfl_xor(mn1, off)); mx1 = fmaxf(mx1, __shfl_xor(mx1, off));
        mn2 = fminf(mn2, __shfl_xor(mn2, off)); mx2 = fmaxf(mx2, __shfl_xor(mx2, off));
        cnt += __shfl_xor(cnt, off);
    }
    __shared__ float red[kWaves][6];
    __shared__ uint32_t redc[kWaves];
    const int wave = threadIdx.x >> 6, lane = threadIdx.x & 63;
    if (lane == 0) {
        red[wave][0] = mn0; red[wave][1] = mn1; red[wave][2] = mn2;
        red[wave][3] = mx0; red[wave][4] = mx1; red[wave][5] = mx2;
        redc[wave] = cnt;
    }
    __syncthreads();
    if (threadIdx.x == 0) {
        for (int w = 1; w < kWaves; w++) {
            mn0 = fminf(mn0, red[w][0]); mn1 = fminf(mn1, red[w][1]); mn2 = fminf(mn2, red[w][2]);
            mx0 = fmaxf(mx0, red[w][3]); mx1 = fmaxf(mx1, red[w][4]); mx2 = fmaxf(mx2, red[w][5]);
            cnt += redc[w];
        }
        uint4* out = reinterpret_cast<uint4*>(parts + 8u * blockIdx.x);
        out[0] = make_uint4(f2ord(mn0), f2ord(mn1), f2ord(mn2), f2ord(mx0));
        out[1] = make_uint4(f2ord(mx1), f2ord(mx2), cnt, 0u);
    }
}

struct VgGrid {
    int minb[3];
    int mul1, mul2;
    uint32_t total;
    uint32_t pass;
};

__device__ inline VgGrid vg_derive(const uint32_t bmin[3], const uint32_t bmax[3], uint32_t n_valid, float inv) {
    VgGrid g;
    g.pass = 0;
    if (n_valid == 0) {
        g.minb[0] = g.minb[1] = g.minb[2] = 0;
        g.mul1 = g.mul2 = 0;
        g.total = 0;
        return g;
    }
    float mn[3], mx[3];
    for (int a = 0; a < 3; a++) { mn[a] = ord2f(bmin[a]); mx[a] = ord2f(bmax[a]); }
    const long long dx = (long long)((mx[0] - mn[0]) * inv) + 1;
    const long long dy = (long long)((mx[1] - mn[1]) * inv) + 1;
    const long long dz = (long long)((mx[2] - mn[2]) * inv) + 1;
    long long divb[3];
    for (int a = 0; a < 3; a++) {
        g.minb[a] = (int)floorf(mn[a] * inv);
        divb[a] = (long long)((int)floorf(mx[a] * inv)) - g.minb[a] + 1;
    }
    const long long total = divb[0] * divb[1] * divb[2];
    if (dx * dy * dz > 2147483647LL || total > 0xFFFFFFF0LL) g.pass = 1;
    g.mul1 = (int)divb[0];
    g.mul2 = (int)(divb[0] * divb[1]);
    g.total = g.pass ? 0u : (uint32_t)total;
    return g;
}

template <bool FOLD>
__device__ __forceinline__ void vg_keys_body(const float4* __restrict__ in, uint32_t n, float inv, ScanDev* sd,
                                                           uint32_t* __restrict__ keys, uint32_t* __restrict__ hist,
                                                           uint32_t nblocks, const uint32_t* __restrict__ parts, uint32_t bx = 0xFFFFFFFFu) {
    if (bx == 0xFFFFFFFFu) bx = blockIdx.x;
    const uint32_t base = bx * kTile;
    float4 p[kItems];
#pragma unroll
    for (int r = 0; r < kItems; r++) {
        const uint32_t i = base + r * kThreads + threadIdx.x;
        if (i < n) p[r] = in[i];
    }
    __shared__ uint32_t h[256];
    __shared__ uint32_t sbox[kWaves][8];
    h[threadIdx.x] = 0;
    uint32_t bmin[3] = {0xFFFFFFFFu, 0xFFFFFFFFu, 0xFFFFFFFFu}, bmax[3] = {0u, 0u, 0u}, n_valid = 0;
    if (!FOLD) {
        for (int a = 0; a < 3; a++) { bmin[a] = sd->bbox_min[a]; bmax[a] = sd->bbox_max[a]; }
        n_valid = sd->n_valid;
        __syncthreads();
    } else {
    for (uint32_t b = threadIdx.x; b < nblocks; b += kThreads) {
        const uint4 r0 = reinterpret_cast<const uint4*>(parts)[2 * b], r1 = reinterpret_cast<const uint4*>(parts)[2 * b + 1];
        if (r1.z) {
            bmin[0] = min(bmin[0], r0.x); bmin[1] = min(bmin[1], r0.y); bmin[2] = min(bmin[2], r0.z);
            bmax[0] = max(bmax[0], r0.w); bmax[1] = max(bmax[1], r1.x); bmax[2] = max(bmax[2], r1.y);
            n_valid += r1.z;
        }
    }
#pragma unroll
    for (int off = 32; off > 0; off >>= 1) {
#pragma unroll
        for (int a = 0; a < 3; a++) { bmin[a] = min(bmin[a], (uint32_t)__shfl_xor((int)bmin[a], off)); bmax[a] = max(bmax[a], (uint32_t)__shfl_xor((int)bmax[a], off)); }
        n_valid += (uint32_t)__shfl_xor((int)n_valid, off);
    }
    if ((threadIdx.x & 63) == 0) {
        uint32_t* o = sbox[threadIdx.x >> 6];
        o[0] = bmin[0]; o[1] = bmin[1]; o[2] = bmin[2]; o[3] = bmax[0]; o[4] = bmax[1]; o[5] = bmax[2]; o[6] = n_valid;
    }
    __syncthreads();
#pragma unroll
    for (int a = 0; a < 3; a++) { bmin[a] = 0xFFFFFFFFu; bmax[a] = 0u; }
    n_valid = 0;
#pragma unroll
    for (int w = 0; w < kWaves; w++) {
#pragma unroll
        for (int a = 0; a < 3; a++) { bmin[a] = min(bmin[a], sbox[w][a]); bmax[a] = max(bmax[a], sbox[w][3 + a]); }
        n_valid += sbox[w][6];
    }
    }
    const VgGrid g = vg_derive(bmin, bmax, n_valid, inv);
    if (bx == 0 && threadIdx.x == 0) {
        if (FOLD) {
            for (int a = 0; a < 3; a++) { sd->bbox_min[a] = bmin[a]; sd->bbox_max[a] = bmax[a]; }
            sd->n_valid = n_valid;
        }
        sd->n_ds_prev = sd->cache_n;
        sd->passthrough = g.pass;
        sd->total_cells = g.total;
        sd->nbits = g.total ? (32 - __clz(g.total)) : 0;
        sd->minb[0] = g.minb[0]; sd->minb[1] = g.minb[1]; sd->minb[2] = g.minb[2];
        sd->mul1 = g.mul1; sd->mul2 = g.mul2;
    }
#pragma unroll
    for (int r = 0; r < kItems; r++) {
        const uint32_t i = base + r * kThreads + threadIdx.x;
        if (i >= n) continue;
        uint32_t key = g.total;
        if (g.total && isfinite(p[r].x) && isfinite(p[r].y) && isfinite(p[r].z)) {
            const int i0 = (int)(floorf(p[r].x * inv) - (float)g.minb[0]);
            const int i1 = (int)(floorf(p[r].y * inv) - (float)g.minb[1]);
            const int i2 = (int)(floorf(p[r].z * inv) - (float)g.minb[2]);
            key = (uint32_t)(i0 + i1 * g.mul1 + i2 * g.mul2);
        }
        keys[i] = key;
        atomicAdd(&h[key & 255u], 1u);
    }
    __syncthreads();
    hist[bx * 256u + threadIdx.x] = h[threadIdx.x];
}

__device__ inline uint32_t active_passes(const ScanDev* sd) { return (sd->nbits + 7u) >> 3; }

__device__ __forceinline__ void radix_hist_body(const uint32_t* __restrict__ ka, const uint32_t* __restrict__ kb, uint32_t n,
                                                              int pass, uint32_t* __restrict__ hist, uint32_t nblocks, const ScanDev* sd, uint32_t bx = 0xFFFFFFFFu) {
    if (bx == 0xFFFFFFFFu) bx = blockIdx.x;
    uint32_t nbits_w = sd->nbits;
    const uint32_t* keys = (pass & 1) ? kb : ka;
    const int shift = pass * 8;
    __shared__ uint32_t h[256];
    const uint32_t base = bx * kTile;
    uint4 kq[kItems / 4];
#pragma unroll
    for (int r = 0; r < kItems / 4; r++) {
        const uint32_t i = base + 4u * (uint32_t)(r * kThreads + threadIdx.x);
        kq[r] = *reinterpret_cast<const uint4*>(keys + (i + 3u < n ? i : 0u));
    }
    pin_loaded(nbits_w);
#pragma unroll
    for (int r = 0; r < kItems / 4; r++) pin_loaded(kq[r]);
    if ((uint32_t)pass >= ((nbits_w + 7u) >> 3)) return;
    h[threadIdx.x] = 0;
    __syncthreads();
#pragma unroll
    for (int r = 0; r < kItems / 4; r++) {
        const uint32_t i = base + 4u * (uint32_t)(r * kThreads + threadIdx.x);
        if (i + 3u < n) {
            atomicAdd(&h[(kq[r].x >> shift) & 255u], 1u);
            atomicAdd(&h[(kq[r].y >> shift) & 255u], 1u);
            atomicAdd(&h[(kq[r].z >> shift) & 255u], 1u);
            atomicAdd(&h[(kq[r].w >> shift) & 255u], 1u);
        } else {
            for (uint32_t e = 0; e < 3u; e++)
                if (i + e < n) atomicAdd(&h[(keys[i + e] >> shift) & 255u], 1u);
        }
    }
    __syncthreads();
    hist[bx * 256u + threadIdx.x] = h[threadIdx.x];
}

template <bool PREFIXED>
__device__ __forceinline__ void radix_scatter_body(uint32_t* __restrict__ ka, uint32_t* __restrict__ va,
                                                                 uint32_t* __restrict__ kb, uint32_t* __restrict__ vb, uint32_t n, int pass,
                                                                 const uint32_t* __restrict__ hist, uint32_t nblocks, const ScanDev* sd, uint32_t bx = 0xFFFFFFFFu) {
    if (bx == 0xFFFFFFFFu) bx = blockIdx.x;
    uint32_t nbits_w = sd->nbits;
    const uint32_t* kin = (pass & 1) ? kb : ka;
    const uint32_t* vin = (pass & 1) ? vb : va;
    uint32_t* kout = (pass & 1) ? ka : kb;
    uint32_t* vout = (pass & 1) ? va : vb;
    const int shift = pass * 8;
    const int tid = threadIdx.x, wave = tid >> 6, lane = tid & 63;
    __shared__ uint32_t wcnt[kWaves][256];
    __shared__ uint32_t wsum[kWaves];
    const uint32_t base = bx * kTile + wave * (64 * kItems);
    uint32_t k[kItems], v[kItems];
    bool ok[kItems];
#pragma unroll
    for (int r = 0; r < kItems; r++) {
        const uint32_t i = base + r * 64 + lane;
        ok[r] = i < n;
        const uint32_t ic = ok[r] ? i : 0u;
        k[r] = kin[ic];
        v[r] = i;
    }
    if (pass != 0) {
#pragma unroll
        for (int r = 0; r < kItems; r++) v[r] = vin[ok[r] ? base + r * 64 + lane : 0u];
    }
    pin_loaded(nbits_w);
#pragma unroll
    for (int r = 0; r < kItems; r++) { pin_loaded(k[r]); pin_loaded(v[r]); }
    if ((uint32_t)pass >= ((nbits_w + 7u) >> 3)) return;
#pragma unroll
    for (int r = 0; r < kItems; r++)
        if (!ok[r]) { k[r] = 0u; v[r] = 0u; }
    uint32_t tot = 0, pre = 0;
    if (PREFIXED) {
        pre = hist[(size_t)bx * 256u + tid];
        tot = hist[(size_t)nblocks * 256u + tid];
    } else {
        const uint32_t* col = hist + tid;
        uint32_t b = 0;
        for (; b + 16 <= nblocks; b += 16) {
            uint32_t hv[16];
#pragma unroll
            for (int k = 0; k < 16; k++) hv[k] = col[(size_t)(b + k) * 256u];
#pragma unroll
            for (int k = 0; k < 16; k++) {
                tot += hv[k];
                pre += (b + k < bx) ? hv[k] : 0u;
            }
        }
        for (; b + 4 <= nblocks; b += 4) {
            const uint32_t h0 = col[(size_t)b * 256u], h1 = col[(size_t)(b + 1) * 256u], h2 = col[(size_t)(b + 2) * 256u], h3 = col[(size_t)(b + 3) * 256u];
            tot += (h0 + h1) + (h2 + h3);
            pre += (b < bx ? h0 : 0u) + (b + 1 < bx ? h1 : 0u) + (b + 2 < bx ? h2 : 0u) + (b + 3 < bx ? h3 : 0u);
        }
        for (; b < nblocks; b++) {
            const uint32_t h0 = col[(size_t)b * 256u];
            tot += h0;
            pre += b < bx ? h0 : 0u;
        }
    }
    uint32_t inc = tot;
#pragma unroll
    for (int off = 1; off < 64; off <<= 1) {
        const uint32_t t = __shfl_up(inc, off);
        if (lane >= off) inc += t;
    }
    if (lane == 63) wsum[wave] = inc;
    for (int j = tid; j < kWaves * 256; j += kThreads) (&wcnt[0][0])[j] = 0;
    __syncthreads();
    uint32_t gbase = inc - tot + pre;
    for (int w = 0; w < wave; w++) gbase += wsum[w];

    const unsigned long long lt = (lane == 0) ? 0ull : (~0ull >> (64 - lane));
    uint32_t below[kItems], total[kItems];
#pragma unroll
    for (int r = 0; r < kItems; r++) {
        const uint32_t d = (k[r] >> shift) & 255u;
// ... 5 lines not shown
    }
    __syncthreads();
    {
        uint32_t g = gbase;
#pragma unroll
        for (int w = 0; w < kWaves; w++) {
            const uint32_t t = wcnt[w][tid];
            wcnt[w][tid] = g;
            g += t;
        }
    }
    __syncthreads();
#pragma unroll
    for (int r = 0; r < kItems; r++) {
        const uint32_t d = (k[r] >> shift) & 255u;
        uint32_t pos = 0;
        if (ok[r]) pos = wcnt[wave][d] + below[r];
        __builtin_amdgcn_wave_barrier();
        if (ok[r] && below[r] == 0) wcnt[wave][d] += total[r];
        __builtin_amdgcn_wave_barrier();
        if (ok[r]) { kout[pos] = k[r]; vout[pos] = v[r]; }
    }
}

__device__ __forceinline__ void vg_count_heads_body(const uint32_t* __restrict__ ka, const uint32_t* __restrict__ kb, uint32_t n,
                                                                  const ScanDev* sd, uint32_t* __restrict__ blockcnt, uint32_t bx = 0xFFFFFFFFu) {
    if (bx == 0xFFFFFFFFu) bx = blockIdx.x;
    const uint32_t* keys = (active_passes(sd) & 1) ? kb : ka;
    __shared__ uint32_t c;
    if (threadIdx.x == 0) c = 0;
    __syncthreads();
    const uint32_t total = sd->total_cells;
    const uint32_t base = bx * kTile;
    uint32_t mine = 0;
    uint32_t kc[kItems], kp[kItems];
#pragma unroll
    for (int r = 0; r < kItems; r++) {
        const uint32_t i = base + r * kThreads + threadIdx.x;
        const uint32_t ic = i < n ? i : (n ? n - 1u : 0u);
        kc[r] = keys[ic];
        kp[r] = keys[ic ? ic - 1u : 0u];
    }
#pragma unroll
    for (int r = 0; r < kItems; r++) {
        const uint32_t i = base + r * kThreads + threadIdx.x;
        const bool head = i < n && kc[r] < total && (i == 0 || kp[r] != kc[r]);
        mine += __popcll(__ballot(head));
    }
    if ((threadIdx.x & 63) == 0) atomicAdd(&c, mine);
    __syncthreads();
    if (threadIdx.x == 0) blockcnt[bx] = c;
}

constexpr uint32_t kLongRun = 32;
constexpr int kStageItems = 4;
constexpr int kStages = kItems / kStageItems;
constexpr uint32_t kStagePts = kStageItems * kThreads;
static_assert(kStageItems % 4 == 0 && kItems % kStageItems == 0, "the gathers go out four at a time");
constexpr uint32_t kMonsterRun = 2048;
constexpr uint32_t kMonsterBlocks = 16;
constexpr uint32_t kMonsterBlocksBatch = 16;

__device__ __forceinline__ void vg_heads_body(const float4* __restrict__ in, const uint32_t* __restrict__ ka,
                                                            const uint32_t* __restrict__ kb, const uint32_t* __restrict__ va,
                                                            const uint32_t* __restrict__ vb, uint32_t n, ScanDev* sd,
                                                            const uint32_t* __restrict__ blockcnt, uint32_t* __restrict__ hpos,
                                                            float4* __restrict__ sorted, float4* __restrict__ out, uint32_t* __restrict__ longlist,
                                                            uint32_t max_ds, uint32_t* __restrict__ host_nds,
                                                            uint32_t launched_passes, uint32_t last_block, uint32_t bx = 0xFFFFFFFFu) {
    if (bx == 0xFFFFFFFFu) bx = blockIdx.x;
    const int tid = threadIdx.x, wave = tid >> 6, lane = tid & 63;
    if (sd->passthrough) {
        if (bx == 0 && tid == 0) host_nds[2] = 0u;
        if (n > max_ds) {
            if (bx == 0 && tid == 0) { sd->err |= 1u; sd->n_ds = 0; host_nds[0] = 0; host_nds[1] = 1u; }
            return;
        }
        const uint32_t base = bx * kTile;
        for (int r = 0; r < kItems; r++) {
            const uint32_t i = base + r * kThreads + tid;
            if (i < n) out[i] = in[i];
        }
        if (bx == 0 && tid == 0) { sd->n_ds = n; host_nds[0] = n; host_nds[1] = 0u; }
        return;
    }
    const uint32_t act = active_passes(sd);
    const bool odd = act & 1;
    const uint32_t* keys = odd ? kb : ka;
    const uint32_t* vals = odd ? vb : va;
    const bool sorted_ok = act != 0u && act <= launched_passes;
    __shared__ uint32_t red[kWaves];
    __shared__ uint32_t n_lq;
    uint32_t pre = 0;
    for (uint32_t b = tid; b < bx; b += kThreads) pre += blockcnt[b];
#pragma unroll
    for (int off = 32; off > 0; off >>= 1) pre += __shfl_xor(pre, off);
    if (lane == 0) red[wave] = pre;
    __syncthreads();
    uint32_t run = 0;
    for (int w = 0; w < kWaves; w++) run += red[w];
    __syncthreads();
    const uint32_t run0 = run;

    const uint32_t total = sd->total_cells;
    const uint32_t n_valid = sd->n_valid;
    const uint32_t base = bx * kTile;
    const unsigned long long lt = (lane == 0) ? 0ull : (~0ull >> (64 - lane));
    uint32_t kc[kItems], kp[kItems], vv[kItems];
#pragma unroll
    for (int r = 0; r < kItems; r++) {
        const uint32_t i = base + r * kThreads + tid;
        const uint32_t ic = i < n ? i : (n ? n - 1u : 0u);
        kc[r] = keys[ic];
        kp[r] = keys[ic ? ic - 1u : 0u];
        vv[r] = vals[ic];
    }
    uint32_t efirst[kStages + 1], eprev[kStages + 1];
    bool ecross[kStages + 1];
#pragma unroll
    for (int e = 0; e <= kStages; e++) {
        const uint32_t g = base + (uint32_t)e * kStagePts;
        efirst[e] = keys[g < n ? g : n - 1u];
        eprev[e] = keys[(g < n ? g : n) ? (g < n ? g : n) - 1u : 0u];
    }
#pragma unroll
    for (int e = 0; e <= kStages; e++) {
        const uint32_t g = base + (uint32_t)e * kStagePts;
        ecross[e] = g != 0u && g < n && efirst[e] < total && eprev[e] == efirst[e];
    }
    __shared__ uint32_t wcnt[kItems][kWaves];
    __shared__ uint16_t tab[kTile];
    unsigned long long hm[kItems];
#pragma unroll
    for (int r = 0; r < kItems; r++) {
        const uint32_t i = base + r * kThreads + tid;
        const bool head = i < n && kc[r] < total && (i == 0 || kp[r] != kc[r]);
        hm[r] = __ballot(head);
        if (lane == 0) wcnt[r][wave] = (uint32_t)__popcll(hm[r]);
    }
    __syncthreads();
    uint32_t hcum[kStages + 1];
    hcum[0] = 0;
#pragma unroll
    for (int r = 0; r < kItems; r++) {
        uint32_t woff = 0, rtot = 0;
#pragma unroll
        for (int w = 0; w < kWaves; w++) {
            const uint32_t t = wcnt[r][w];
            if (w < wave) woff += t;
            rtot += t;
        }
        if ((hm[r] >> lane) & 1ull) {
            const uint32_t slot = run + woff + (uint32_t)__popcll(hm[r] & lt);
            if (slot < max_ds) hpos[slot] = base + r * kThreads + tid;
            tab[slot - run0] = (uint16_t)(r * kThreads + tid);
        }
        run += rtot;
        if ((r + 1) % kStageItems == 0) hcum[(r + 1) / kStageItems] = run - run0;
    }
    __shared__ float4 pts[kStagePts];
    __shared__ uint16_t lq[kStagePts / kLongRun];
    if (sorted_ok) {
#pragma unroll
        for (int st = 0; st < kStages; st++) {
            const bool left_cross = ecross[st], right_cross = ecross[st + 1];
            const uint32_t kfirst = efirst[st], klast = eprev[st + 1];
// ... 222 lines not shown
            for (int k = 0; k < kAhead; k++) {
                const uint32_t c0 = c + (uint32_t)k * 64u;
                if (c0 >= rb) break;
                pk[0][lane] = p[k].x; pk[1][lane] = p[k].y; pk[2][lane] = p[k].z; pk[3][lane] = p[k].w;
                const uint32_t cn = c0 + 64u * kAhead;
                if (cn < rb) p[k] = sorted[(cn + lane) < rb ? cn + lane : rb - 1];
                __builtin_amdgcn_fence(__ATOMIC_RELEASE, "wavefront");
                __builtin_amdgcn_wave_barrier();
                __builtin_amdgcn_fence(__ATOMIC_ACQUIRE, "wavefront");
                const int m = (rb - c0) < 64u ? (int)(rb - c0) : 64;
                if (lane < 4) {
                    const float* q = pk[lane];
                    int j = 0;
                    for (; j + 4 <= m; j += 4) {
                        const float4 a = *reinterpret_cast<const float4*>(q + j);
                        t = t + a.x; t = t + a.y; t = t + a.z; t = t + a.w;
                    }
                    for (; j < m; j++) t = t + q[j];
                }
                __builtin_amdgcn_fence(__ATOMIC_RELEASE, "wavefront");
                __builtin_amdgcn_wave_barrier();
                __builtin_amdgcn_fence(__ATOMIC_ACQUIRE, "wavefront");
            }
        }
        const float cnt = (float)(rb - ra);
        if (lane < 4) reinterpret_cast<float*>(&out[v])[lane] = t / cnt;
    }
}

__global__ void scan_set_nds_kernel(ScanDev* sd, uint32_t n) {
    sd->n_ds_prev = sd->cache_n;
    sd->n_ds = n;
}

__device__ __forceinline__ void scan_begin_body(ScanDev* sd, int32_t* __restrict__ nn_cnt, uint32_t min_ds, uint32_t reset) {
    const uint32_t n = sd->n_ds, hi = sd->n_ds_prev;
    const uint32_t lo = reset ? 0u : n;
    if (n >= min_ds) {
        for (uint32_t i = lo + blockIdx.x * blockDim.x + threadIdx.x; i < hi; i += gridDim.x * blockDim.x) nn_cnt[i] = 0;
        if (blockIdx.x == 0 && threadIdx.x == 0) sd->cache_n = n;
    }
    if (blockIdx.x == 0 && threadIdx.x < 3) {
        sd->bbox_min[threadIdx.x] = 0xFFFFFFFFu;
        sd->bbox_max[threadIdx.x] = 0u;
        if (threadIdx.x == 0) { sd->n_valid = 0; sd->n_long = 0; sd->n_monster = 0; }
    }
}


#ifndef LIO_VG_XCD
#define LIO_VG_XCD 1
#endif
__device__ __forceinline__ void vg_slot_tile(uint32_t n_slots, uint32_t& slot, uint32_t& bx) {
    slot = blockIdx.y;
    bx = blockIdx.x;
#if LIO_VG_XCD
    const uint32_t T = gridDim.x, L = blockIdx.x + T * blockIdx.y, full = n_slots & ~7u;
    if (L < full * T) {
        const uint32_t j = L >> 3;
        slot = (j / T) * 8u + (L & 7u);
        bx = j % T;
    }
#endif
}

__global__ void __launch_bounds__(kThreads) vg_bbox_kernel(const float4* __restrict__ in, uint32_t n, uint32_t* __restrict__ parts) { vg_bbox_body(in, n, parts); }
__global__ void __launch_bounds__(kThreads) vg_bbox_batch(const SlotDesc* __restrict__ slots) {
    const SlotDesc& d = slots[blockIdx.y];
    if (!d.active) return;
    vg_bbox_atomic_body(d.raw, d.n_raw, d.sd);
}
__global__ void __launch_bounds__(kThreads) vg_keys_kernel(const float4* __restrict__ in, uint32_t n, float inv, ScanDev* sd,
                                                           uint32_t* __restrict__ keys, uint32_t* __restrict__ hist,
                                                           uint32_t nblocks, const uint32_t* __restrict__ parts) {
    vg_keys_body<true>(in, n, inv, sd, keys, hist, nblocks, parts);
}
__global__ void __launch_bounds__(kThreads) vg_keys_batch(const SlotDesc* __restrict__ slots, float inv) {
    uint32_t slot, bx;
    vg_slot_tile(gridDim.y, slot, bx);
    const SlotDesc& d = slots[slot];
    if (!d.active || bx >= d.nblocks) return;
    vg_keys_body<false>(d.raw, d.n_raw, inv, d.sd, d.keys_a, d.hist, d.nblocks, nullptr, bx);
}
__global__ void __launch_bounds__(kThreads) radix_hist_kernel(const uint32_t* __restrict__ ka, const uint32_t* __restrict__ kb, uint32_t n,
                                                              int pass, uint32_t* __restrict__ hist, uint32_t nblocks, const ScanDev* sd) {
    radix_hist_body(ka, kb, n, pass, hist, nblocks, sd);
}
__global__ void __launch_bounds__(kThreads) radix_hist_batch(const SlotDesc* __restrict__ slots, int pass) {
    uint32_t slot, bx;
    vg_slot_tile(gridDim.y, slot, bx);
    const SlotDesc& d = slots[slot];
    if (!d.active || bx >= d.nblocks) return;
    radix_hist_body(d.keys_a, d.keys_b, d.n_raw, pass, d.hist, d.nblocks, d.sd, bx);
}
__global__ void __launch_bounds__(kThreads) radix_scatter_kernel(uint32_t* __restrict__ ka, uint32_t* __restrict__ va,
                                                                 uint32_t* __restrict__ kb, uint32_t* __restrict__ vb, uint32_t n, int pass,
                                                                 const uint32_t* __restrict__ hist, uint32_t nblocks, const ScanDev* sd) {
    radix_scatter_body<false>(ka, va, kb, vb, n, pass, hist, nblocks, sd);
}
__global__ void __launch_bounds__(kThreads) radix_scatter_batch(const SlotDesc* __restrict__ slots, int pass) {
    uint32_t slot, bx;
    vg_slot_tile(gridDim.y, slot, bx);
    const SlotDesc& d = slots[slot];
    if (!d.active || bx >= d.nblocks) return;
    radix_scatter_body<true>(d.keys_a, d.vals_a, d.keys_b, d.vals_b, d.n_raw, pass, d.hist, d.nblocks, d.sd, bx);
}
__global__ void __launch_bounds__(256) radix_prefix_batch(const SlotDesc* __restrict__ slots, int pass) {
    const SlotDesc& d = slots[blockIdx.x];
    if (!d.active) return;
    if ((uint32_t)pass >= active_passes(d.sd)) return;
    const uint32_t nb = d.nblocks;
    uint32_t* col = d.hist + threadIdx.x;
    uint32_t run = 0;
    for (uint32_t b = 0; b < nb; b += 16) {
        uint32_t hv[16];
#pragma unroll
        for (int k = 0; k < 16; k++) hv[k] = col[(size_t)(b + k < nb ? b + k : b) * 256u];
#pragma unroll
        for (int k = 0; k < 16; k++)
            if (b + k < nb) {
                col[(size_t)(b + k) * 256u] = run;
                run += hv[k];
            }
    }
    col[(size_t)nb * 256u] = run;
}
__global__ void __launch_bounds__(kThreads) vg_count_heads_kernel(const uint32_t* __restrict__ ka, const uint32_t* __restrict__ kb, uint32_t n,
                                                                  const ScanDev* sd, uint32_t* __restrict__ blockcnt) {
    vg_count_heads_body(ka, kb, n, sd, blockcnt);
}
__global__ void __launch_bounds__(kThreads) vg_count_heads_batch(const SlotDesc* __restrict__ slots) {
    uint32_t slot, bx;
    vg_slot_tile(gridDim.y, slot, bx);
    const SlotDesc& d = slots[slot];
    if (!d.active || bx >= d.nblocks) return;
    vg_count_heads_body(d.keys_a, d.keys_b, d.n_raw, d.sd, d.blockcnt, bx);
}
__global__ void __launch_bounds__(kThreads) vg_heads_kernel(const float4* __restrict__ in, const uint32_t* __restrict__ ka,
                                                            const uint32_t* __restrict__ kb, const uint32_t* __restrict__ va,
                                                            const uint32_t* __restrict__ vb, uint32_t n, ScanDev* sd,
                                                            const uint32_t* __restrict__ blockcnt, uint32_t* __restrict__ hpos,
                                                            float4* __restrict__ sorted, float4* __restrict__ out, uint32_t* __restrict__ longlist,
                                                            uint32_t max_ds, uint32_t* __restrict__ host_nds, uint32_t launched_passes) {
    vg_heads_body(in, ka, kb, va, vb, n, sd, blockcnt, hpos, sorted, out, longlist, max_ds, host_nds, launched_passes, gridDim.x - 1);
}
__global__ void __launch_bounds__(kThreads) vg_heads_batch(const SlotDesc* __restrict__ slots, uint32_t launched_passes) {
    uint32_t slot, bx;
    vg_slot_tile(gridDim.y, slot, bx);
    const SlotDesc& d = slots[slot];
    if (!d.active || bx >= d.nblocks) return;
    vg_heads_body(d.raw, d.keys_a, d.keys_b, d.vals_a, d.vals_b, d.n_raw, d.sd, d.blockcnt, d.hpos, d.sorted, d.ds_body, d.longlist, d.max_ds, d.host_nds,
                  launched_passes, d.nblocks - 1, bx);
}
__global__ void __launch_bounds__(kThreads) vg_centroid_long_kernel(const float4* __restrict__ sorted, const uint32_t* __restrict__ hpos,
                                                                    const ScanDev* __restrict__ sd, float4* __restrict__ out,
                                                                    const uint32_t* __restrict__ longlist, uint32_t max_ds, uint32_t n_long_blocks) {
    vg_centroid_long_body<0>(sorted, hpos, sd, out, longlist, max_ds, n_long_blocks);
}
__global__ void __launch_bounds__(kThreads) vg_centroid_long_batch(const SlotDesc* __restrict__ slots) {
    const SlotDesc& d = slots[blockIdx.y];
    if (!d.active) return;
    vg_centroid_long_body<1>(d.sorted, d.hpos, d.sd, d.ds_body, d.longlist, d.max_ds, gridDim.x);
}
__global__ void __launch_bounds__(kThreads) vg_centroid_both_batch(const SlotDesc* __restrict__ slots) {
    const SlotDesc& d = slots[blockIdx.y];
    if (!d.active) return;
    vg_centroid_long_body<0>(d.sorted, d.hpos, d.sd, d.ds_body, d.longlist, d.max_ds, gridDim.x - kMonsterBlocksBatch);
}
__global__ void __launch_bounds__(kThreads) vg_centroid_monster_batch(const SlotDesc* __restrict__ slots) {
    const SlotDesc& d = slots[blockIdx.y];
    if (!d.active || d.sd->n_monster == 0) return;
    vg_centroid_long_body<2>(d.sorted, d.hpos, d.sd, d.ds_body, d.longlist, d.max_ds, 0u);
}
__global__ void scan_begin_kernel(ScanDev* sd, int32_t* __restrict__ nn_cnt, uint32_t min_ds) { scan_begin_body(sd, nn_cnt, min_ds, 0u); }
__global__ void scan_begin_batch(const SlotDesc* __restrict__ slots) {
    const SlotDesc& d = slots[blockIdx.y];
    if (!d.active) return;
    scan_begin_body(d.sd, d.nn_cnt, d.min_ds, d.reset_cache);
}

int vg_downsample(lio_scan* s, float leaf, int passes) {
    const uint32_t n = s->n_raw;
    const float inv = 1.0f / leaf;
    hipStream_t st = s->stream;
    const uint32_t nblocks = (n + kTile - 1) / kTile;
    if (n == 0) {
        hipLaunchKernelGGL(scan_set_nds_kernel, 1, 1, 0, st, s->dev, 0u);
        s->host_nds[0] = 0;
        s->host_nds[1] = 0;
        s->host_nds[2] = 0;
        return LIO_OK;
    }
    uint32_t* parts = reinterpret_cast<uint32_t*>(s->sorted);
    hipLaunchKernelGGL(vg_bbox_kernel, nblocks, kThreads, 0, st, s->raw, n, parts);
    hipLaunchKernelGGL(vg_keys_kernel, nblocks, kThreads, 0, st, s->raw, n, inv, s->dev, s->keys_a, s->hist, nblocks, parts);
    for (int pass = 0; pass < passes; pass++) {
        if (pass > 0) hipLaunchKernelGGL(radix_hist_kernel, nblocks, kThreads, 0, st, s->keys_a, s->keys_b, n, pass, s->hist, nblocks, s->dev);
        hipLaunchKernelGGL(radix_scatter_kernel, nblocks, kThreads, 0, st, s->keys_a, s->vals_a, s->keys_b, s->vals_b, n, pass, s->hist, nblocks,
                           s->dev);
    }
    hipLaunchKernelGGL(vg_count_heads_kernel, nblocks, kThreads, 0, st, s->keys_a, s->keys_b, n, s->dev, s->blockcnt);
    hipLaunchKernelGGL(vg_heads_kernel, nblocks, kThreads, 0, st, s->raw, s->keys_a, s->keys_b, s->vals_a, s->vals_b, n, s->dev, s->blockcnt,
                       s->hpos, s->sorted, s->ds_body, s->longlist, s->max_ds, s->host_nds_dev, (uint32_t)passes);
    hipLaunchKernelGGL(vg_centroid_long_kernel, 256 + kMonsterBlocks, kThreads, 0, st, s->sorted, s->hpos, s->dev, s->ds_body, s->longlist, s->max_ds, 256u);
    LIO_HIP_TRY(hipGetLastError());
    return LIO_OK;
}

int vg_downsample_batch(hipStream_t st, const SlotDesc* d_slots, int n_slots, uint32_t max_raw, uint32_t max_ds, float leaf, int passes) {
    const float inv = 1.0f / leaf;
    const uint32_t nblocks = (max_raw + kTile - 1) / kTile;
    if (nblocks == 0 || n_slots <= 0) return LIO_OK;
    const uint32_t B = (uint32_t)n_slots;
    hipLaunchKernelGGL(vg_bbox_batch, dim3(nblocks < 48 ? nblocks : 48, B), kThreads, 0, st, d_slots);
    hipLaunchKernelGGL(vg_keys_batch, dim3(nblocks, B), kThreads, 0, st, d_slots, inv);
    for (int pass = 0; pass < passes; pass++) {
        if (pass > 0) hipLaunchKernelGGL(radix_hist_batch, dim3(nblocks, B), kThreads, 0, st, d_slots, pass);
        hipLaunchKernelGGL(radix_prefix_batch, dim3(B), 256, 0, st, d_slots, pass);
        hipLaunchKernelGGL(radix_scatter_batch, dim3(nblocks, B), kThreads, 0, st, d_slots, pass);
    }
    hipLaunchKernelGGL(vg_count_heads_batch, dim3(nblocks, B), kThreads, 0, st, d_slots);
    hipLaunchKernelGGL(vg_heads_batch, dim3(nblocks, B), kThreads, 0, st, d_slots, (uint32_t)passes);
    static const bool split = []() { const char* e = getenv("LIO_VG_MONSTER_SPLIT"); return e && e[0] == '1'; }();
    if (split) {
        hipLaunchKernelGGL(vg_centroid_long_batch, dim3(64, B), kThreads, 0, st, d_slots);
        hipLaunchKernelGGL(vg_centroid_monster_batch, dim3(kMonsterBlocksBatch, B), kThreads, 0, st, d_slots);
    } else {
        hipLaunchKernelGGL(vg_centroid_both_batch, dim3(64 + kMonsterBlocksBatch, B), kThreads, 0, st, d_slots);
    }
    hipLaunchKernelGGL(scan_begin_batch, dim3(16, B), 256, 0, st, d_slots);
    LIO_HIP_TRY(hipGetLastError());
    return LIO_OK;
}

int scan_begin_rows(hipStream_t st, const SlotDesc* d_descs, int n_rows) {
    if (n_rows <= 0) return LIO_OK;
    hipLaunchKernelGGL(scan_begin_batch, dim3(16, (uint32_t)n_rows), 256, 0, st, d_descs);
    LIO_HIP_TRY(hipGetLastError());
    return LIO_OK;
}

int scan_begin(lio_scan* s) {
    hipLaunchKernelGGL(scan_begin_kernel, 64, 256, 0, s->stream, s->dev, s->nn_cnt, s->resize_min);
    LIO_HIP_TRY(hipGetLastError());
    return LIO_OK;
}

int scan_set_nds(lio_scan* s, uint32_t n) {
    hipLaunchKernelGGL(scan_set_nds_kernel, 1, 1, 0, s->stream, s->dev, n);
    LIO_HIP_TRY(hipGetLastError());
    return LIO_OK;
}

}
```

lidar-slam-detection_amd/python/lsd_amd/capi.py:

```python
import ctypes as C
import os

import numpy as np

_HERE = os.path.dirname(os.path.abspath(__file__))
os.environ.setdefault("GPU_MAX_HW_QUEUES", "8")
LIB_PATH = os.environ.get("LIO_HIP_LIB") or os.path.join(_HERE, "liblio_hip.so")

LIO_OK, LIO_E_INVALID, LIO_E_CAPACITY, LIO_E_DEVICE, LIO_E_STATE = 0, -1, -2, -3, -4
MAIN_FIRST_SCAN, MAIN_SEEDED, MAIN_SKIPPED, MAIN_UPDATED, MAIN_IMU_INIT, MAIN_IDLE = 0, 1, 2, 3, 4, 5

SYMBOLS = [
    "lio_last_warning",
    "lio_last_error", "lio_device_count", "lio_map_bytes",
    "lio_map_create", "lio_map_destroy", "lio_map_set_lru", "lio_map_lru_stats", "lio_map_lru_exact_stats", "lio_map_set_tie_mode", "lio_map_tie_stats", "lio_map_clear", "lio_map_pool_stats", "lio_map_set_stencil", "lio_map_insert", "lio_map_insert_device", "lio_map_stats",
    "lio_abi_version", "lio_pinned_alloc", "lio_pinned_free",
    "lio_map_dump", "lio_map_knn", "lio_map_knn_candidates", "lio_map_knn_touched", "lio_map_knn_unique",
    "lio_scan_create", "lio_scan_destroy", "lio_scan_reset", "lio_scan_upload", "lio_scan_set_device", "lio_scan_undistort_delta", "lio_scan_undistort_poses", "lio_scan_undistort_imu", "lio_scan_download_raw", "lio_scan_voxel_downsample", "lio_scan_voxel_downsample_batch", "lio_scan_set_ds",
    "lio_scan_num_ds", "lio_scan_download_ds", "lio_scan_download_world", "lio_scan_download_match",
    "lio_p2plane_linearize", "lio_scan_set_degeneracy_mode", "lio_p2plane_degeneracy", "lio_engine_set_reduce_hook", "lio_p2plane_rows", "lio_map_incremental", "lio_map_seed",
    "lio_engine_create", "lio_engine_create_shared", "lio_engine_destroy", "lio_engine_map", "lio_engine_scan", "lio_engine_set_state", "lio_engine_get_state",
    "lio_engine_set_cov", "lio_engine_get_cov", "lio_engine_set_flags", "lio_engine_travel", "lio_engine_is_degenerate",
    "lio_engine_update", "lio_engine_pass_log", "lio_engine_process_scan", "lio_engine_process_scan_device", "lio_engine_timings", "lio_engine_flush",
    "lio_engine_enable_timing", "lio_comm_unique_id", "lio_comm_init", "lio_comm_destroy", "lio_comm_rank", "lio_comm_world", "lio_allgather_normal_eq", "lio_comm_stats", "lio_engine_set_joint", "lio_engine_joint_register", "lio_engine_joint_register_device", "lio_allgather_records", "lio_engines_process_batch", "lio_batch_create", "lio_batch_create_joint", "lio_batch_create_sequences", "lio_batch_sequences_step", "lio_batch_fastlio_main", "lio_batch_set_gather_hook", "lio_batch_exchange_stats", "lio_batch_destroy", "lio_batch_process", "lio_batch_engine", "lio_batch_enable_kernel_timing", "lio_batch_kernel_times", "lio_engine_set_static_map", "lio_scan_enable_kernel_timing", "lio_scan_kernel_times",
    "lio_state_boxplus", "lio_state_boxminus",
    "lio_localmap_create", "lio_localmap_destroy", "lio_localmap_add_keyframe", "lio_localmap_num_keyframes", "lio_localmap_update",
    "lio_localmap_download",
    "lio_localmap_nearest", "lio_localmap_gather", "lio_localmap_z_mean", "lio_localmap_download_gather", "lio_localmap_gather_device", "lio_localmap_store_frame",
    "lio_localmap_frame", "lio_estimate_matcher_params", "lio_localmap_estimate_pose", "lio_scan_ds_device", "lio_gicp_set_target_device", "lio_gicp_set_source_device",
    "lio_cloud_create", "lio_cloud_destroy", "lio_cloud_clear", "lio_cloud_size", "lio_cloud_append_scan", "lio_cloud_append_host",
    "lio_cloud_voxel_downsample", "lio_cloud_download", "lio_cloud_scratch_bytes", "lio_cloud_last_times",
    "lio_knn_index_create", "lio_knn_index_destroy", "lio_knn_index_build", "lio_knn_index_query", "lio_knn_index_colour", "lio_knn_index_last_times",
    "lio_ground_default_params", "lio_ground_draw", "lio_ground_create", "lio_ground_destroy", "lio_ground_detect_scan", "lio_ground_detect_host",
    "lio_ground_download_indices", "lio_ground_download_normals", "lio_ground_download_inliers", "lio_ground_download_draws", "lio_ground_last_run",
    "lio_ground_last_times",
    "lio_bev_create", "lio_bev_destroy", "lio_bev_preprocess_host", "lio_bev_preprocess_cloud", "lio_bev_upload_pixels", "lio_bev_convert", "lio_bev_get_info",
    "lio_bev_download_pixel_coords", "lio_bev_download_kept", "lio_bev_download_pixels", "lio_bev_download_nodes", "lio_bev_download_equalised",
    "lio_bev_download_image", "lio_bev_grey_table", "lio_bev_last_times",
    "lio_keyframe_decide", "lio_keyframer_default_params", "lio_keyframer_create", "lio_keyframer_destroy", "lio_keyframer_reset", "lio_keyframer_push_host",
    "lio_keyframer_pending", "lio_keyframer_pop", "lio_radius_outlier_host", "lio_keyframe_filter_host", "lio_keyframer_fitness_host",
    "lio_keyframer_append_local_map_host", "lio_keyframer_download_local_map", "lio_keyframer_last_times",
    "lio_pose_estimator_create", "lio_pose_estimator_destroy", "lio_pose_estimator_predict", "lio_pose_estimator_match", "lio_pose_estimator_match_gps", "lio_pose_estimator_guess", "lio_pose_estimator_observe",
    "lio_pose_estimator_match_gps_only", "lio_pose_estimator_get_timed_pose", "lio_pose_estimator_predict_nostate",
    "lio_pose_estimator_correct", "lio_pose_estimator_get_dt", "lio_pose_estimator_get", "lio_pose_estimator_set", "lio_pose_estimator_matrix",
    "lio_fastlio_init", "lio_fastlio_is_init", "lio_fastlio_imu_enqueue", "lio_engine_set_device_loop", "lio_fastlio_ins_enqueue", "lio_fastlio_set_wheelspeed", "lio_fastlio_pcl_enqueue", "lio_fastlio_pcl_enqueue_device", "lio_fastlio_pcl_stage", "lio_fastlio_pcl_commit",
    "lio_fastlio_main", "lio_fastlio_odometry", "lio_fastlio_state", "lio_fastlio_start_state", "lio_fastlio_download_undistorted",
    "lio_state_predict", "lio_eskf_update_cb", "lio_eskf_update_ws_cb", "lio_eskf_update_sums_cb",
    "lio_ndt_create", "lio_ndt_destroy", "lio_ndt_set_target", "lio_ndt_set_target_device", "lio_ndt_num_voxels", "lio_ndt_fitness_score", "lio_ndt_overlap_score", "lio_ndt_voxel_at",
    "lio_ndt_linearize", "lio_ndt_default_params", "lio_ndt_align", "lio_ndt_align_batch", "lio_ndt_enable_kernel_timing", "lio_ndt_kernel_times",
    "lio_gicp_create", "lio_gicp_destroy", "lio_gicp_set_target", "lio_gicp_set_source", "lio_gicp_set_voxel_mode", "lio_gicp_voxel_at", "lio_gicp_download", "lio_gicp_correspondences", "lio_gicp_neighbours", "lio_gicp_mahalanobis", "lio_gicp_linearize", "lio_gicp_align", "lio_gicp_fitness_score",
    "lio_loop_default_params", "lio_loop_find_candidates", "lio_loop_information_matrix", "lio_loop_create", "lio_loop_destroy", "lio_loop_reset",
    "lio_loop_add_keyframe_host", "lio_loop_set_pose", "lio_loop_num_keyframes", "lio_loop_download_keyframe", "lio_loop_detect", "lio_loop_edges",
    "lio_loop_last_report", "lio_loop_last_times", "lio_loop_align_candidates", "lio_loop_align_fine", "lio_loop_pair_information",
    "lio_overlap_default_params", "lio_overlap_connection_count", "lio_overlap_find_candidates", "lio_overlap_create", "lio_overlap_destroy",
    "lio_overlap_gate_batch", "lio_overlap_align_pairs", "lio_overlap_accumulate", "lio_overlap_download_accum", "lio_overlap_detect",
    "lio_overlap_last_report", "lio_overlap_last_times",
    "lio_sc_create", "lio_sc_destroy", "lio_sc_reset", "lio_sc_num_frames", "lio_sc_add_frames_host", "lio_sc_download_frame", "lio_sc_describe_host", "lio_sc_set_active",
    "lio_sc_distance", "lio_sc_search", "lio_sc_global_search_host", "lio_sc_shift_to_yaw", "lio_sc_last_dropped", "lio_sc_last_times",
    "lio_sc_set_positions", "lio_sc_local_search", "lio_sc_last_local", "lio_update_origin",
    "lio_graph_default_params", "lio_graph_create", "lio_graph_destroy", "lio_graph_reset", "lio_graph_add_node", "lio_graph_set_fixed", "lio_graph_set_estimate",
    "lio_graph_num_nodes", "lio_graph_get_fixed", "lio_graph_add_edge", "lio_graph_remove_edge", "lio_graph_optimize", "lio_graph_estimates", "lio_graph_edges",
    "lio_graph_chi2", "lio_graph_linearize", "lio_graph_last_times", "lio_se3_from_mqt", "lio_se3_to_mqt", "lio_graph_edge_error",
    "lio_graph_add_prior", "lio_graph_set_kernel", "lio_graph_priors", "lio_graph_prior_error", "lio_graph_remove_gnss_outliers",
    "lio_graph_remove_node", "lio_graph_node_live", "lio_graph_edge_records", "lio_loop_retire",
    "lio_graph_estimate_gnss_moment", "lio_graph_moment_begin", "lio_graph_moment_end", "lio_graph_moment_get", "lio_graph_moment_linearize",
    "lio_render_create", "lio_render_destroy", "lio_render_clear", "lio_render_set_cameras", "lio_render_set_active", "lio_render_frame", "lio_render_size",
    "lio_render_download", "lio_render_download_voxels", "lio_render_download_points", "lio_render_download_last_image", "lio_render_last_times",
    "lio_utm_create", "lio_utm_destroy", "lio_utm_zone", "lio_utm_forward", "lio_utm_inverse", "lio_utm_longitude0", "lio_grid_convergence",
    "lio_transform_from_rpyt", "lio_quat_of_transform", "lio_interpolate_transform", "lio_rtk_transform_utm", "lio_rtk_transform_origin",
    "lio_rtk_track_create", "lio_rtk_track_destroy", "lio_rtk_track_set_origin", "lio_rtk_track_origin", "lio_rtk_track_feed", "lio_rtk_track_size",
    "lio_rtk_track_interpolate",
    "lio_gnss_queue_create", "lio_gnss_queue_destroy", "lio_gnss_queue_set_origin", "lio_gnss_queue_push", "lio_gnss_queue_size", "lio_gnss_queue_stamps",
    "lio_gnss_queue_flush",
    "lio_scan_merge_create", "lio_scan_merge_destroy", "lio_scan_merge_set_transform", "lio_scan_merge_run_host", "lio_scan_merge_download",
    "lio_scan_merge_device", "lio_scan_merge_last_times",
    "lio_calib_subsample", "lio_se3f_exp", "lio_se3f_log", "lio_se3f_mul", "lio_se3f_inverse", "lio_se3f_matrix", "lio_se3f_from_matrix",
    "lio_calib_interpolate", "lio_dfo_default_params", "lio_dfo_direct_l", "lio_dfo_nelder_mead", "lio_calib_default_params",
    "lio_calib_ins_create", "lio_calib_ins_destroy", "lio_calib_ins_reset", "lio_calib_ins_add_scan", "lio_calib_ins_add_odom", "lio_calib_ins_counts",
    "lio_calib_ins_set_transform", "lio_calib_ins_scan_matrices", "lio_calib_ins_combined", "lio_calib_ins_error", "lio_calib_ins_error_terms",
    "lio_calib_ins_calibrate", "lio_calib_ins_progress", "lio_calib_ins_result", "lio_calib_ins_last_times",
    "lio_calib_ground_default_params", "lio_calib_ground_create", "lio_calib_ground_destroy", "lio_calib_ground_crop_host",
    "lio_calib_ground_set_points_host", "lio_calib_ground_fit", "lio_calib_ground_download_indices", "lio_calib_ground_download_points",
    "lio_calib_ground_download_draws", "lio_calib_ground_last_run", "lio_calib_ground_last_times",
]
ABI_VERSION = 22
ABI_REQUIRED = 23
RTK_INTERPOLATED, RTK_EXACT, RTK_NO_ORIGIN, RTK_TOO_FEW, RTK_EARLY, RTK_LATE = 0, 1, 2, 3, 4, 5


class NormalEq(C.Structure):
    _fields_ = [("JtJ", C.c_double * 36), ("Jtr", C.c_double * 6), ("nnT", C.c_double * 9), ("eigvec", C.c_double * 9),
                ("eigval", C.c_double * 3), ("contri", C.c_double * 3), ("strong", C.c_double * 3), ("sum_abs_res", C.c_double),
                ("n_eff", C.c_uint32), ("n_ds", C.c_uint32), ("n_knn_candidates_lo", C.c_uint32), ("n_knn_candidates_hi", C.c_uint32),
                ("n_tie", C.c_uint32), ("seq", C.c_uint32)]


class BatchTimes(C.Structure):
    _fields_ = [("downsample_us", C.c_double), ("knn_us", C.c_double), ("linearize_us", C.c_double), ("step_us", C.c_double),
                ("downsample_launches", C.c_uint32), ("knn_launches", C.c_uint32), ("linearize_launches", C.c_uint32), ("step_launches", C.c_uint32),
                ("insert_us", C.c_double), ("insert_launches", C.c_uint32), ("pad", C.c_uint32)]


class PassLog(C.Structure):
    _fields_ = [("knn", C.c_int32), ("n_eff", C.c_int32), ("valid", C.c_int32), ("degenerate", C.c_int32), ("sum_abs_res", C.c_double),
                ("JtJ", C.c_double * 36), ("Jtr", C.c_double * 6), ("dx", C.c_double * 23)]


# ... 212 lines not shown
    sig("lio_map_destroy", None, vp)
    sig("lio_map_set_stencil", cint, vp, cint)
    sig("lio_map_insert", cint, vp, f32p, u64, dbl)
    sig("lio_map_insert_device", cint, vp, vp, u64, dbl)
    sig("lio_map_stats", cint, vp, C.POINTER(u64), C.POINTER(u64))
    sig("lio_map_dump", C.c_int64, vp, f32p, u64)
    sig("lio_map_set_lru", cint, vp, u64, dbl)
    sig("lio_map_lru_stats", cint, vp, C.POINTER(u64), C.POINTER(u64))
    sig("lio_map_lru_exact_stats", cint, vp, C.POINTER(u64), C.POINTER(u64))
    sig("lio_map_clear", cint, vp)
    sig("lio_map_set_tie_mode", cint, vp, cint)
    sig("lio_map_tie_stats", cint, vp, C.POINTER(u64), C.POINTER(u64))
    sig("lio_map_pool_stats", cint, vp, C.POINTER(u64), C.POINTER(u64))
    sig("lio_map_knn_candidates", u64, vp)
    sig("lio_map_knn_touched", u64, vp)
    sig("lio_map_knn_unique", u64, vp)
    sig("lio_map_knn", cint, vp, f32p, u32, f32p, i32p)
    sig("lio_scan_create", vp, cint, u32, u32)
    sig("lio_scan_destroy", None, vp)
    sig("lio_scan_reset", cint, vp)
    sig("lio_scan_upload", cint, vp, f32p, u32)
    sig("lio_scan_set_device", cint, vp, vp, u32)
    sig("lio_scan_undistort_delta", cint, vp, vp, cint, f32p, C.c_double)
    sig("lio_scan_undistort_poses", cint, vp, vp, cint, u64, C.POINTER(u64), f64p, u32)
    sig("lio_scan_undistort_imu", cint, vp, vp, cint, f64p, u32, f64p, f64p, f64p, f64p, dbl, cint, cint)
    sig("lio_scan_download_raw", cint, vp, f32p, u32)
    sig("lio_scan_voxel_downsample", cint, vp, flt, cint, C.POINTER(u32))
    sig("lio_scan_voxel_downsample_batch", cint, C.POINTER(vp), cint, flt, C.POINTER(u32))
    sig("lio_scan_set_ds", cint, vp, f32p, u32)
    sig("lio_scan_num_ds", cint, vp)
    sig("lio_scan_download_ds", cint, vp, f32p, u32)
    sig("lio_scan_download_world", cint, vp, f32p, u32)
    sig("lio_scan_download_match", cint, vp, u8p, f32p, i32p, f32p)
    sig("lio_p2plane_linearize", cint, vp, vp, f64p, f64p, cint, C.POINTER(NormalEq))
    sig("lio_scan_set_degeneracy_mode", cint, vp, cint)
    sig("lio_p2plane_degeneracy", cint, vp, f64p, f64p, f64p)
    sig("lio_engine_set_reduce_hook", cint, vp, REDUCE_FN, vp)
    sig("lio_p2plane_rows", cint, vp, f64p, f64p, f64p, f64p, u32)
    sig("lio_map_incremental", cint, vp, vp, f64p, f64p, flt, cint, dbl)
    sig("lio_map_seed", cint, vp, vp, f64p, f64p, dbl)
    sig("lio_engine_create", vp, cint, flt, cint, u64, u64, u32, u32)
    sig("lio_engine_create_shared", vp, vp, u32, u32)
    sig("lio_engine_destroy", None, vp)
    sig("lio_engine_map", vp, vp)
    sig("lio_engine_scan", vp, vp)
    sig("lio_engine_set_state", cint, vp, f64p)
    sig("lio_engine_get_state", cint, vp, f64p)
    sig("lio_engine_set_cov", cint, vp, f64p)
    sig("lio_engine_get_cov", cint, vp, f64p)
    sig("lio_engine_set_flags", cint, vp, cint, cint, dbl, dbl)
    sig("lio_engine_travel", dbl, vp)
    sig("lio_engine_is_degenerate", cint, vp)
    sig("lio_engine_update", cint, vp)
    sig("lio_engine_pass_log", cint, vp, cint, C.POINTER(PassLog))
    sig("lio_engine_process_scan", cint, vp, f32p, u32, dbl)
    sig("lio_engine_process_scan_device", cint, vp, vp, u32, dbl)
    sig("lio_engine_timings", cint, vp, C.POINTER(Timings))
    sig("lio_engine_flush", cint, vp)
    sig("lio_engine_enable_timing", cint, vp, cint)
    sig("lio_engines_process_batch", cint, C.POINTER(vp), cint, C.POINTER(ScanJob), cint)
    sig("lio_comm_unique_id", cint, C.POINTER(C.c_uint8))
    sig("lio_comm_init", vp, cint, cint, cint, C.POINTER(C.c_uint8))
    sig("lio_comm_destroy", None, vp)
    sig("lio_comm_rank", cint, vp)
    sig("lio_comm_world", cint, vp)
    sig("lio_allgather_normal_eq", cint, vp, vp, vp, vp, vp)
    sig("lio_comm_stats", cint, vp, C.POINTER(u64), f64p)
    sig("lio_engine_set_joint", cint, vp, C.POINTER(vp), cint, vp)
    sig("lio_engine_joint_register", cint, vp, f32p, u32, dbl, f64p, f64p)
    sig("lio_engine_joint_register_device", cint, vp, vp, u32, dbl, f64p, f64p)
    sig("lio_allgather_records", cint, vp, vp, vp, u32, vp)
    sig("lio_batch_create_joint", vp, C.POINTER(vp), cint, vp, cint, cint, u32, u32)
    sig("lio_batch_set_gather_hook", cint, vp, GATHER_FN, vp, cint, cint)
    sig("lio_batch_exchange_stats", cint, vp, C.POINTER(C.c_uint32), C.POINTER(C.c_uint64), C.POINTER(C.c_uint64))
    sig("lio_batch_create", vp, vp, cint, cint, u32, u32)
    sig("lio_batch_create_sequences", vp, cint, C.c_float, cint, u64, u64, cint, cint, u32, u32)
    sig("lio_batch_sequences_step", cint, vp, C.POINTER(ScanJob), cint, C.POINTER(C.c_double))
    sig("lio_batch_fastlio_main", cint, vp, C.POINTER(cint))
    sig("lio_batch_destroy", None, vp)
    sig("lio_batch_process", cint, vp, C.POINTER(ScanJob), cint)
    sig("lio_batch_engine", vp, vp, cint, cint)
    sig("lio_batch_enable_kernel_timing", cint, vp, cint)
    sig("lio_batch_kernel_times", cint, vp, C.POINTER(BatchTimes), cint)
    sig("lio_engine_set_static_map", cint, vp, cint)
    sig("lio_localmap_create", vp, cint, u64, u32, u32)
    sig("lio_localmap_destroy", None, vp)
    sig("lio_localmap_add_keyframe", cint, vp, f32p, u32, f32p)
    sig("lio_localmap_num_keyframes", cint, vp)
    sig("lio_localmap_update", cint, vp, vp, f64p, dbl, dbl, dbl, flt, C.POINTER(cint), C.POINTER(u32))
    sig("lio_localmap_download", cint, vp, f32p, u32)
    sig("lio_localmap_nearest", cint, vp, f64p, u32, i32p, f32p)
    sig("lio_localmap_gather", cint, vp, i32p, u32, C.POINTER(u32), f64p)
    sig("lio_localmap_z_mean", cint, vp, vp, u32, f64p)
    sig("lio_localmap_download_gather", cint, vp, f32p, u32)
    sig("lio_localmap_gather_device", vp, vp, C.POINTER(u32))
    sig("lio_localmap_store_frame", cint, vp, cint, vp, u32)
    sig("lio_localmap_frame", vp, vp, cint, C.POINTER(u32))
    sig("lio_estimate_matcher_params", None, C.POINTER(NdtParams))
    sig("lio_localmap_estimate_pose", cint, vp, vp, vp, u32, f64p, C.POINTER(EstimateReport), f64p)
    sig("lio_scan_ds_device", vp, vp, C.POINTER(u32))
    sig("lio_cloud_create", vp, cint, u64)
    sig("lio_cloud_destroy", None, vp)
    sig("lio_cloud_clear", cint, vp)
    sig("lio_cloud_size", cint, vp, C.POINTER(u64))
    sig("lio_cloud_append_scan", cint, vp, vp, f64p, flt, cint, dbl, dbl)
    sig("lio_cloud_append_host", cint, vp, f32p, u64, f64p, flt, cint, dbl, dbl)
    sig("lio_cloud_voxel_downsample", cint, vp, flt, C.POINTER(u64))
    sig("lio_cloud_download", C.c_int64, vp, f32p, u64)
    sig("lio_cloud_scratch_bytes", cint, vp, C.POINTER(u64))
    sig("lio_cloud_last_times", cint, vp, f64p, f64p)
    sig("lio_knn_index_create", vp, cint)
    sig("lio_knn_index_destroy", None, vp)
    sig("lio_knn_index_build", cint, vp, f32p, C.POINTER(C.c_uint32), u64, C.POINTER(u64))
    sig("lio_knn_index_query", cint, vp, f32p, u64, cint, i32p, f32p)
    sig("lio_knn_index_colour", cint, vp, f32p, u64, cint, u8p)
    sig("lio_knn_index_last_times", cint, vp, f64p, f64p)
    gp, u32p = C.POINTER(GroundParams), C.POINTER(u32)
    sig("lio_ground_default_params", None, gp, cint)
    sig("lio_ground_draw", None, u32, u32, u32, u32p)
    sig("lio_ground_create", vp, cint)
    sig("lio_ground_destroy", None, vp)
    sig("lio_ground_detect_scan", cint, vp, vp, gp, cint, C.POINTER(cint), f32p, u32p, u32p, u32p)
    sig("lio_ground_detect_host", cint, vp, f32p, u64, gp, C.POINTER(cint), f32p, u32p, u32p, u32p)
    sig("lio_ground_download_indices", C.c_int64, vp, cint, u32p, u64)
    sig("lio_ground_download_normals", C.c_int64, vp, f32p, u64)
    sig("lio_ground_download_inliers", C.c_int64, vp, f32p, u64)
    sig("lio_ground_download_draws", C.c_int64, vp, u32p, u32p, f32p, u64)
    sig("lio_ground_last_run", cint, vp, C.POINTER(cint), C.POINTER(cint), C.POINTER(cint), C.POINTER(cint))
    sig("lio_ground_last_times", cint, vp, f64p, f64p)
    kp, kr, u64p = C.POINTER(KeyframerParams), C.POINTER(KeyframeReport), C.POINTER(u64)
    sig("lio_keyframe_decide", cint, f64p, f64p, dbl, dbl, C.POINTER(cint), C.POINTER(cint), f64p, f64p)
    sig("lio_keyframer_default_params", None, kp)
    sig("lio_keyframer_create", vp, cint, kp)
    sig("lio_keyframer_destroy", None, vp)
    sig("lio_keyframer_reset", cint, vp)
    sig("lio_keyframer_push_host", cint, vp, f32p, u32p, u32, u64, f64p, f64p, u64p, f64p, u32, kr)
    sig("lio_keyframer_pending", cint, vp)
    sig("lio_keyframer_pop", C.c_int64, vp, f32p, u64, f64p, u64p, f64p, u32p, u32p)
    sig("lio_radius_outlier_host", C.c_int64, vp, f32p, u64, dbl, cint, u32p, u64, u32p)
    sig("lio_keyframe_filter_host", C.c_int64, vp, f32p, u64, dbl, cint, dbl, u32p, u64, u32p, u32p)
    sig("lio_keyframer_fitness_host", cint, vp, f32p, u32, f64p, f64p, u32p)
    sig("lio_keyframer_append_local_map_host", cint, vp, f32p, u32, f64p)
    sig("lio_keyframer_download_local_map", C.c_int64, vp, f32p, u64)
    sig("lio_keyframer_last_times", cint, vp, f64p, f64p, f64p, f64p)
    u16p = C.POINTER(C.c_uint16)
    sig("lio_bev_create", vp, cint)
    sig("lio_bev_destroy", None, vp)
    sig("lio_bev_preprocess_host", cint, vp, f32p, u64, dbl)
    sig("lio_bev_preprocess_cloud", cint, vp, vp, dbl)
    sig("lio_bev_upload_pixels", cint, vp, u32p, f32p, f32p, u64, u32, u32)
    sig("lio_bev_convert", cint, vp, dbl, dbl)
    sig("lio_bev_get_info", cint, vp, C.POINTER(BevInfo))
    sig("lio_bev_download_pixel_coords", C.c_int64, vp, i32p, u64)
    sig("lio_bev_download_kept", C.c_int64, vp, u32p, u64)
    sig("lio_bev_download_pixels", C.c_int64, vp, u32p, f32p, f32p, u64)
    sig("lio_bev_download_nodes", C.c_int64, vp, u32p, i32p, f64p, u64)
    sig("lio_bev_download_equalised", C.c_int64, vp, f32p, u64)
    sig("lio_bev_download_image", C.c_int64, vp, u16p, u64)
    sig("lio_bev_grey_table", None, u16p)
    sig("lio_bev_last_times", cint, vp, f64p, f64p)
    sig("lio_pose_estimator_create", vp, f32p, u64, f32p, f32p, dbl)
    sig("lio_pose_estimator_destroy", None, vp)
    sig("lio_pose_estimator_predict", cint, vp, u64, f32p, f32p)
    sig("lio_pose_estimator_match", cint, vp, vp, vp, C.POINTER(NdtParams), f32p, C.POINTER(cint))
    sig("lio_pose_estimator_match_gps", cint, vp, vp, vp, C.POINTER(NdtParams), C.POINTER(GpsObservation), f32p, f32p, C.POINTER(cint))
    sig("lio_pose_estimator_guess", cint, vp, C.POINTER(GpsObservation), f32p)
# ... 258 lines not shown
```

lidar-slam-detection_amd/python/lsd_amd/lio.py:

```python
import ctypes as C

import numpy as np

from . import capi
from .capi import check, f32, f64, lib, ptr

STATE_DIM = 26
DOF = 23
G_LEN = 9.809


def default_state():
    s = np.zeros(STATE_DIM)
    s[6] = 1.0
    s[10] = 1.0
    s[23] = G_LEN
    return s


def init_cov():
    P = np.eye(23)
    for i in (6, 7, 8, 9, 10, 11):
        P[i, i] = 0.00001
    for i in (15, 16, 17):
# ... 1682 lines not shown
        u = (C.c_uint8 * 128)()
        check(lib().lio_comm_unique_id(u), "comm unique id")
        return bytes(u)

    def allgather(self, d_local, d_gathered, d_sum=None, stream=None):
        check(lib().lio_allgather_normal_eq(self.h, d_local, d_gathered, d_sum, stream), "allgather")

    def stats(self):
        n, t = C.c_uint64(), C.c_double()
        check(lib().lio_comm_stats(self.h, C.byref(n), C.byref(t)))
        return n.value, t.value

    def close(self):
        if getattr(self, "h", None) and lib is not None:
            lib().lio_comm_destroy(self.h)
        self.h = None

    __del__ = close


class Batch:

    def __init__(self, shared_map, n_slots=8, n_groups=3, max_raw=262144, max_ds=100000, sub_maps=None, comm=None):
        self.map = shared_map
        self.n_slots, self.n_groups = n_slots, n_groups
        self._keep = (list(sub_maps or []), comm)
        if sub_maps or comm is not None:
            ms = [shared_map] + list(sub_maps or [])
            hs = (C.c_void_p * len(ms))(*[m.h for m in ms])
            self.h = lib().lio_batch_create_joint(hs, len(ms), comm.h if comm is not None else None, n_slots, n_groups, max_raw, max_ds)
        else:
            self.h = lib().lio_batch_create(shared_map.h, n_slots, n_groups, max_raw, max_ds)
        if not self.h:
            raise capi.LioError("lio_batch_create failed: " + lib().lio_last_error().decode())

    def close(self):
        if getattr(self, "h", None) and lib is not None:
            lib().lio_batch_destroy(self.h)
        self.h = None

    __del__ = close

    def set_gather_hook(self, fn, rank, world):

        def _cb(_ctx, d_local, d_gathered, n, stream):
            try:
                return int(fn(int(d_local or 0), int(d_gathered or 0), int(n), int(stream or 0)) or 0)
            except Exception:
                import traceback

                traceback.print_exc()
                return -1

        self._gather = capi.GATHER_FN(_cb)
        check(lib().lio_batch_set_gather_hook(self.h, self._gather, None, int(rank), int(world)), "set_gather_hook")

    def exchange_stats(self):
        cap, again, nbytes = C.c_uint32(0), C.c_uint64(0), C.c_uint64(0)
        check(lib().lio_batch_exchange_stats(self.h, C.byref(cap), C.byref(again), C.byref(nbytes)))
        return {"chunk_points": cap.value, "jobs_rerun": again.value, "bytes_per_rank_and_round": nbytes.value}

    def enable_kernel_timing(self, on=True):
        check(lib().lio_batch_enable_kernel_timing(self.h, int(on)))

    def kernel_times(self, reset=True):
        t = capi.BatchTimes()
        check(lib().lio_batch_kernel_times(self.h, C.byref(t), int(reset)))
        return {k: getattr(t, k) for k, _ in t._fields_}

    def engine(self, group, slot):
        h = lib().lio_batch_engine(self.h, group, slot)
        if not h:
            raise capi.LioError("no such slot")
        e = Engine.__new__(Engine)
        e.h = h
        e._own = False
        e.map = self.map
        e.scan = Scan(max_ds=100000, _borrow=lib().lio_engine_scan(h))
        return e

    def process(self, jobs):
        return process_batch(None, jobs, batch=self)


JOB_KEEP_CACHE = 1
JOB_IDLE = 2
JOB_HOST_RAW = 4


class PinnedCloud:

    def __init__(self, pts):
        pts = np.ascontiguousarray(pts, dtype=np.float32).reshape(-1, 4)
        self.n = len(pts)
        self.nbytes = max(pts.nbytes, 16)
        self.ptr = lib().lio_pinned_alloc(self.nbytes)
        if not self.ptr:
            raise MemoryError((lib().lio_last_error() or b'').decode())
        self.array = np.ctypeslib.as_array(C.cast(self.ptr, C.POINTER(C.c_float)), shape=(max(self.n, 1), 4))[: self.n]
        self.array[...] = pts

    def __del__(self):
        try:
            if getattr(self, "ptr", None):
                self.array = None
                lib().lio_pinned_free(self.ptr)
                self.ptr = None
        except Exception:
            pass


class SequenceBatch:

    def __init__(self, n_slots=8, n_groups=1, resolution=0.5, stencil=19, max_points=2_000_000, max_voxels=1_000_000, max_raw=262144, max_ds=100000, device=0):
        self.n_slots, self.n_groups = n_slots, n_groups
        self.n = n_slots * n_groups
        self.h = lib().lio_batch_create_sequences(device, resolution, stencil, max_points, max_voxels, n_slots, n_groups, max_raw, max_ds)
        if not self.h:
            raise capi.LioError("lio_batch_create_sequences failed: " + lib().lio_last_error().decode())
        self.arr = (capi.ScanJob * self.n)()
        self.states_in = np.zeros((self.n, STATE_DIM))
        self.covs_in = np.zeros((self.n, 23 * 23))
        self.states_out = np.zeros((self.n, STATE_DIM))
        self.covs_out = np.zeros((self.n, 23 * 23))
        for i in range(self.n):
            a = self.arr[i]
            a.state_in = self.states_in[i].ctypes.data_as(C.POINTER(C.c_double))
            a.cov_in = self.covs_in[i].ctypes.data_as(C.POINTER(C.c_double))
            a.state_out = self.states_out[i].ctypes.data_as(C.POINTER(C.c_double))

    def close(self):
        if getattr(self, "h", None) and lib is not None:
            lib().lio_batch_destroy(self.h)
        self.h = None

    __del__ = close

    def engine(self, session):
        h = lib().lio_batch_engine(self.h, session // self.n_slots, session % self.n_slots)
        if not h:
            raise capi.LioError("no such session")
        e = Engine.__new__(Engine)
        e.h = h
        e._own = False
        e.map = Map(_borrow=lib().lio_engine_map(h))
        e.scan = Scan(max_ds=100000, _borrow=lib().lio_engine_scan(h))
        return e

    def enable_kernel_timing(self, on=True):
        check(lib().lio_batch_enable_kernel_timing(self.h, int(on)))

    def kernel_times(self, reset=True):
        t = capi.BatchTimes()
        check(lib().lio_batch_kernel_times(self.h, C.byref(t), int(reset)))
        return {k: getattr(t, k) for k, _ in t._fields_}

    def fastlio_main(self):
        if not hasattr(self, "_fl_rc"):
            self._fl_rc = (C.c_int * self.n)()
        rc = lib().lio_batch_fastlio_main(self.h, self._fl_rc)
        return rc, list(self._fl_rc)

    def load(self, jobs):
        assert len(jobs) == self.n
        for i, j in enumerate(jobs):
            a = self.arr[i]
# ... 834 lines not shown
```

Baseline: 6.131 billion.

## Predict voxel-grid cell box from prior scans to skip bbox pass

Adds a predicted-box path to the batched voxel downsample. The batch keeps a union of per-scan cell bounds from earlier rounds and uses it to compute voxel keys directly, which skips the separate bbox reduction kernel. The true bbox is then checked inside the prefix kernel, and scans whose cells fall outside the box are flagged and redone on the exact path. This is on by default (box_mode=1) and adds separate graph instances, an ABI bump, and a risk of redo rounds when scans move outside the predicted box.

```diff
diff --git a/include/lio_hip.h b/include/lio_hip.h
--- a/include/lio_hip.h
+++ b/include/lio_hip.h
@@ -20,7 +20,7 @@
 const char* lio_last_error(void);
 const char* lio_last_warning(void);
 int lio_device_count(void);
-#define LIO_ABI_VERSION 26
+#define LIO_ABI_VERSION 27
 int lio_abi_version(void);
 void* lio_pinned_alloc(uint64_t bytes);
 void lio_pinned_free(void* p);
@@ -206,6 +206,7 @@
     int32_t n_pass, n_knn_pass, n_ds, n_eff, degenerate, radix_passes, err;
     int32_t loop_i, loop_t, loop_converge, pad;
     uint32_t seq, pad2;
+    int32_t cell_lo[3], cell_hi[3];
 } lio_batch_result;
 lio_batch* lio_batch_create(lio_map* shared_map, int n_slots, int n_groups, uint32_t max_raw, uint32_t max_ds);
 lio_batch* lio_batch_create_joint(lio_map** sub_maps, int n_sub_maps, lio_comm* comm, int n_slots, int n_groups, uint32_t max_raw, uint32_t max_ds);
@@ -218,6 +219,10 @@
 int lio_batch_fastlio_main(lio_batch*, int* rc_out);
 void lio_batch_destroy(lio_batch*);
 int lio_batch_process(lio_batch*, lio_scan_job* jobs, int n_jobs);
+void lio_box_union(int32_t* state7, const int32_t* cells6, int n);
+int lio_box_decide(int32_t* state7, int passes, int drop, int32_t* minb3, int32_t* divb3);
+int lio_batch_set_box_prediction(lio_batch*, int mode, const int32_t* minb3, const int32_t* divb3);
+int lio_batch_box_stats(lio_batch*, uint64_t* rounds_exact, uint64_t* rounds_predicted, uint64_t* scans_flagged);
 typedef struct lio_batch_times {
     double downsample_us, knn_us, linearize_us, step_us;
     uint32_t downsample_launches, knn_launches, linearize_launches, step_launches;
diff --git a/lidar-slam-detection_amd/csrc/batch.hip b/lidar-slam-detection_amd/csrc/batch.hip
--- a/lidar-slam-detection_amd/csrc/batch.hip
+++ b/lidar-slam-detection_amd/csrc/batch.hip
@@ -48,6 +48,7 @@
     EskfDev* d_ctrl = nullptr;
     EskfDev* h_ctrl = nullptr;
     hipGraphExec_t exec[5] = {nullptr, nullptr, nullptr, nullptr, nullptr};
+    hipGraphExec_t exec_pred[5] = {nullptr, nullptr, nullptr, nullptr, nullptr};
     const void* graph_table = nullptr;
     int graph_stencil = 0;
     lio_batch_result* h_res = nullptr;
@@ -62,6 +63,7 @@
     int any_lru = 0;
     int n_active = 0;
     int launched_passes = 4;
+    int launched_pred = 0;
     uint32_t seq = 0;
     uint32_t max_n_raw = 0;
     BatchTimer* bt = nullptr;
@@ -75,6 +77,10 @@
     int n_slots = 0;
     uint32_t max_raw = 0, max_ds = 0;
     int pred_passes = 4;
+    int box_mode = 1;
+    int32_t box_state[7] = {0, 0, 0, 0, 0, 0, 0};
+    int32_t forced_box[6] = {0, 0, 0, 0, 0, 0};
+    uint64_t n_rounds_exact = 0, n_rounds_pred = 0, n_box_miss = 0;
     bool broken = false;
     int use_graph = 1;
     int count_touched = 0;
@@ -158,8 +164,10 @@
     if (g.d_ds_send) hipFree(g.d_ds_send);
     if (g.d_ds_all) hipFree(g.d_ds_all);
     if (g.d_rowmaps) hipFree(g.d_rowmaps);
-    for (int k = 0; k < 5; k++)
+    for (int k = 0; k < 5; k++) {
         if (g.exec[k]) hipGraphExecDestroy(g.exec[k]);
+        if (g.exec_pred[k]) hipGraphExecDestroy(g.exec_pred[k]);
+    }
     if (g.d_block) hipFree(g.d_block);
     if (g.d_rawbuf) hipFree(g.d_rawbuf);
     if (g.h_block) hipHostFree(g.h_block);
@@ -193,12 +201,14 @@
     return dst;
 }
 
-int submit(lio_batch* b, Group& g, lio_scan_job* jobs, int first, int n, int passes) {
+int submit(lio_batch* b, Group& g, lio_scan_job* jobs, int first, int n, int passes, const int32_t* box = nullptr) {
     const int B = b->n_slots;
+    const int pred = box ? 1 : 0;
     g.seq++;
     g.n_active = 0;
     g.max_n_raw = 0;
     g.launched_passes = passes;
+    g.launched_pred = pred;
     for (int s = 0; s < B; s++) {
         SlotDesc& d = g.h_desc[s];
         d.active = 0;
@@ -225,6 +235,8 @@
         d.seq = g.seq;
         d.min_ds = 5;
         d.reset_cache = (job.flags & LIO_JOB_KEEP_CACHE) ? 0u : 1u;
+        d.box_pred = (uint32_t)pred;
+        for (int a = 0; a < 3; a++) { d.box_min[a] = box ? box[a] : 0; d.box_div[a] = box ? box[3 + a] : 0; }
         fill_ctrl(g.h_ctrl[s], job.state_in, job.cov_in, 0.001 , 4, 1, b->joint ? 1 : 0);
         g.h_res[s].seq = g.seq - 1;
         g.n_active++;
@@ -238,6 +250,7 @@
             d.raw = p.raw; d.n_raw = p.n_raw; d.nblocks = p.nblocks; d.active = p.active; d.seq = p.seq; d.min_ds = p.min_ds; d.reset_cache = p.reset_cache;
         }
     if (g.n_active == 0) return LIO_OK;
+    (pred ? b->n_rounds_pred : b->n_rounds_exact)++;
     const bool timed = g.bt && g.bt->on;
     const MapRef* rowmaps = b->joint ? joint_rowmaps(b, g) : nullptr;
     auto enqueue = [&](BatchTimer* bt) -> int {
@@ -273,7 +286,7 @@
             if (rc != LIO_OK) return rc;
         } else {
             if (bt) bt->begin(0);
-            rc = vg_downsample_batch(g.stream, g.d_desc, B, b->max_raw, b->max_ds, 0.5f, passes);
+            rc = vg_downsample_batch(g.stream, g.d_desc, B, b->max_raw, b->max_ds, 0.5f, passes, pred);
             if (bt) bt->end(0);
             if (rc != LIO_OK) return rc;
         }
@@ -288,22 +301,25 @@
     };
     if (!b->use_graph || timed || b->joint) return enqueue(timed ? g.bt : nullptr);
     if (g.graph_table != b->map->table || g.graph_stencil != b->map->stencil.n) {
-        for (int k = 0; k < 5; k++)
+        for (int k = 0; k < 5; k++) {
             if (g.exec[k]) { hipGraphExecDestroy(g.exec[k]); g.exec[k] = nullptr; }
+            if (g.exec_pred[k]) { hipGraphExecDestroy(g.exec_pred[k]); g.exec_pred[k] = nullptr; }
+        }
         g.graph_table = b->map->table;
         g.graph_stencil = b->map->stencil.n;
     }
-    if (!g.exec[passes]) {
+    hipGraphExec_t& exec = pred ? g.exec_pred[passes] : g.exec[passes];
+    if (!exec) {
         hipGraph_t graph = nullptr;
         LIO_HIP_TRY(hipStreamBeginCapture(g.stream, hipStreamCaptureModeThreadLocal));
         const int rc = enqueue(nullptr);
         const hipError_t e2 = hipStreamEndCapture(g.stream, &graph);
         if (rc != LIO_OK) { if (graph) hipGraphDestroy(graph); return rc; }
         LIO_HIP_TRY(e2);
-        LIO_HIP_TRY(hipGraphInstantiate(&g.exec[passes], graph, nullptr, nullptr, 0));
+        LIO_HIP_TRY(hipGraphInstantiate(&exec, graph, nullptr, nullptr, 0));
         hipGraphDestroy(graph);
     }
-    LIO_HIP_TRY(hipGraphLaunch(g.exec[passes], g.stream));
+    LIO_HIP_TRY(hipGraphLaunch(exec, g.stream));
     return LIO_OK;
 }
 
@@ -453,6 +469,9 @@
     if (getenv("LIO_BATCH_PROFILE") && b->n_rounds)
         fprintf(stderr, "lio_batch: %llu rounds of %d slots; host per round: submit %.1f us, wait %.1f us, collect %.1f us\n", (unsigned long long)b->n_rounds,
                 b->n_slots, 1e6 * b->t_submit / b->n_rounds, 1e6 * b->t_wait / b->n_rounds, 1e6 * b->t_collect / b->n_rounds);
+    if (getenv("LIO_BATCH_PROFILE") && b->n_rounds && !b->sequences)
+        fprintf(stderr, "lio_batch: downsample chain: %llu rounds exact, %llu on the predicted box, %llu scans flagged and redone exact\n",
+                (unsigned long long)b->n_rounds_exact, (unsigned long long)b->n_rounds_pred, (unsigned long long)b->n_box_miss);
     for (Group& g : b->groups) {
         if (g.stream) hipStreamSynchronize(g.stream);
         group_free(g);
@@ -499,6 +518,63 @@
 lio_engine* lio_batch_engine(lio_batch* b, int group, int slot) {
     if (!b || group < 0 || group >= (int)b->groups.size() || slot < 0 || slot >= b->n_slots) return nullptr;
     return b->groups[group].eng[slot];
+}
+
+static int box_passes(const int32_t lo[3], const int32_t hi[3]) {
+    const long long lim = 1LL << 24;
+    unsigned long long total = 1;
+    for (int a = 0; a < 3; a++) {
+        const long long l = lo[a], h = hi[a], dv = h - l + 1;
+        if (dv < 1 || dv > lim || l <= -lim || l >= lim || h <= -lim || h >= lim) return 0;
+        total *= (unsigned long long)dv;
+        if (total > 0xFFFFFFF0ull) return 0;
+    }
+    int nbits = 0;
+    while (nbits < 32 && (total >> nbits)) nbits++;
+    return (nbits + 7) >> 3;
+}
+
+void lio_box_union(int32_t* st, const int32_t* cells6, int n) {
+    if (!st || !cells6) return;
+    for (int i = 0; i < n; i++) {
+        const int32_t* c = cells6 + 6 * (size_t)i;
+        if (c[0] > c[3] || c[1] > c[4] || c[2] > c[5]) continue;
+        for (int a = 0; a < 3; a++) {
+            st[1 + a] = st[0] ? std::min(st[1 + a], c[a]) : c[a];
+            st[4 + a] = st[0] ? std::max(st[4 + a], c[3 + a]) : c[3 + a];
+        }
+        st[0] = 1;
+    }
+}
+
+int lio_box_decide(int32_t* st, int passes, int drop, int32_t* minb3, int32_t* divb3) {
+    if (!st || !st[0]) return 0;
+    const int need = box_passes(st + 1, st + 4);
+    if (need == 0 || need > passes) {
+        if (drop) st[0] = 0;
+        return 0;
+    }
+    for (int a = 0; a < 3; a++) {
+        if (minb3) minb3[a] = st[1 + a];
+        if (divb3) divb3[a] = st[4 + a] - st[1 + a] + 1;
+    }
+    return 1;
+}
+
+int lio_batch_set_box_prediction(lio_batch* b, int mode, const int32_t* minb3, const int32_t* divb3) {
+    if (!b || mode < 0 || mode > 2 || (mode == 2 && (!minb3 || !divb3))) return LIO_E_INVALID;
+    b->box_mode = mode;
+    b->box_state[0] = 0;
+    for (int a = 0; a < 3 && mode == 2; a++) { b->forced_box[a] = minb3[a]; b->forced_box[3 + a] = divb3[a]; }
+    return LIO_OK;
+}
+
+int lio_batch_box_stats(lio_batch* b, uint64_t* rounds_exact, uint64_t* rounds_predicted, uint64_t* scans_flagged) {
+    if (!b) return LIO_E_INVALID;
+    if (rounds_exact) *rounds_exact = b->n_rounds_exact;
+    if (rounds_predicted) *rounds_predicted = b->n_rounds_pred;
+    if (scans_flagged) *scans_flagged = b->n_box_miss;
+    return LIO_OK;
 }
 
 int lio_batch_process(lio_batch* b, lio_scan_job* jobs, int n_jobs) {
@@ -518,10 +594,22 @@
             if (!g.h_desc[s].active) { note(jobs[j].rc); continue; }
             lio_scan_job& job = jobs[j];
             const lio_batch_result& r = g.h_res[s];
-            if (r.radix_passes > need_max) need_max = r.radix_passes;
-            if (r.radix_passes > g.launched_passes) { retry.push_back(j); continue; }
             lio_engine* e = g.eng[s];
             lio_scan* sc = lio_engine_scan(e);
+            if (g.launched_pred) {
+                const int own = box_passes(r.cell_lo, r.cell_hi);
+                if (own > need_max) need_max = own;
+                if (r.err & (int32_t)kErrBoxMiss) {
+                    hipMemsetAsync(&sc->dev->err, 0, 4, g.stream);
+                    b->n_box_miss++;
+                    retry.push_back(j);
+                    continue;
+                }
+            } else {
+                if (r.radix_passes > need_max) need_max = r.radix_passes;
+                if (r.radix_passes > g.launched_passes) { retry.push_back(j); continue; }
+            }
+            if (b->box_mode == 1 && !b->joint) lio_box_union(b->box_state, r.cell_lo, 1);
             sc->have_ds = r.n_ds;
             sc->n_raw = g.h_desc[s].n_raw;
             job.n_ds = r.n_ds;
@@ -586,6 +674,19 @@
             b->ds_cap = std::min(ds_bound, std::max(4096u, want));
         }
     };
+    int32_t box6[6];
+    auto round_box = [&]() -> const int32_t* {
+        if (b->joint || b->box_mode == 0) return nullptr;
+        if (b->box_mode == 1) return lio_box_decide(b->box_state, b->pred_passes, 1, box6, box6 + 3) ? box6 : nullptr;
+        int32_t st[7] = {1, 0, 0, 0, 0, 0, 0};
+        for (int a = 0; a < 3; a++) {
+            const long long hi = (long long)b->forced_box[a] + b->forced_box[3 + a] - 1;
+            if (hi < INT32_MIN || hi > INT32_MAX) return nullptr;
+            st[1 + a] = b->forced_box[a];
+            st[4 + a] = (int32_t)hi;
+        }
+        return lio_box_decide(st, b->pred_passes, 0, box6, box6 + 3) ? box6 : nullptr;
+    };
     using clk = std::chrono::steady_clock;
     auto secs = [](clk::time_point a, clk::time_point c) { return std::chrono::duration<double>(c - a).count(); };
     auto bail = [&](int rc) {
@@ -596,7 +697,7 @@
     for (size_t gi = 0; gi < b->groups.size() && next < n_jobs; gi++) {
         const int n = n_jobs - next < B ? n_jobs - next : B;
         const auto t0 = clk::now();
-        const int rc = submit(b, b->groups[gi], jobs, next, n, b->pred_passes);
+        const int rc = submit(b, b->groups[gi], jobs, next, n, b->pred_passes, round_box());
         b->t_submit += secs(t0, clk::now());
         b->n_rounds++;
         if (rc != LIO_OK) return bail(rc);
@@ -620,7 +721,7 @@
         b->t_collect += secs(t1, t2);
         if (next < n_jobs) {
             const int n = n_jobs - next < B ? n_jobs - next : B;
-            const int rc = submit(b, g, jobs, next, n, b->pred_passes);
+            const int rc = submit(b, g, jobs, next, n, b->pred_passes, round_box());
             b->t_submit += secs(t2, clk::now());
             b->n_rounds++;
             if (rc != LIO_OK) return bail(rc);
@@ -636,7 +737,9 @@
         int rc = submit(b, g, jobs, j, 1, 4);
         if (rc == LIO_OK && g.n_active) rc = wait_group(g, B);
         if (rc != LIO_OK) { b->ds_cap_full = false; return bail(rc); }
+        const int before = b->pred_passes;
         collect(g);
+        if (b->pred_passes < before) b->pred_passes = before;
     }
     b->ds_cap_full = false;
     for (const int j : retry) { jobs[j].rc = LIO_E_DEVICE; note(LIO_E_DEVICE); }
diff --git a/lidar-slam-detection_amd/csrc/lio_common.h b/lidar-slam-detection_amd/csrc/lio_common.h
--- a/lidar-slam-detection_amd/csrc/lio_common.h
+++ b/lidar-slam-detection_amd/csrc/lio_common.h
@@ -104,7 +104,9 @@
     int32_t mul1, mul2;
     uint32_t total_cells;
     uint32_t n_monster;
-};
+    int32_t cell_lo[3], cell_hi[3];
+};
+constexpr uint32_t kErrBoxMiss = 8u;
 
 struct StencilArgs {
     int n;
@@ -129,6 +131,8 @@
     uint32_t* host_nds;
     EskfDev* ctrl;
     lio_batch_result* result;
+    uint32_t box_pred;
+    int32_t box_min[3], box_div[3];
 };
 
 struct MapRef {
@@ -312,7 +316,8 @@
                      const UndistortArgs& args, unsigned long long* d_block_min );
 
 int vg_downsample(lio_scan* s, float leaf, int passes );
-int vg_downsample_batch(hipStream_t st, const SlotDesc* d_slots, int n_slots, uint32_t max_raw, uint32_t max_ds, float leaf, int passes);
+int vg_downsample_batch(hipStream_t st, const SlotDesc* d_slots, int n_slots, uint32_t max_raw, uint32_t max_ds, float leaf, int passes,
+                        int predicted_box = 0 );
 int knn_batch_launch(lio_map* m, hipStream_t st, const SlotDesc* d_slots, int n_slots, uint32_t grid_x, int count_touched);
 struct BatchTimer {
     static constexpr int kClasses = 5;
diff --git a/lidar-slam-detection_amd/csrc/p2plane.hip b/lidar-slam-detection_amd/csrc/p2plane.hip
--- a/lidar-slam-detection_amd/csrc/p2plane.hip
+++ b/lidar-slam-detection_amd/csrc/p2plane.hip
@@ -555,6 +555,7 @@
             r->n_eff = c.n_eff_last; r->degenerate = c.is_degenerate; r->radix_passes = (int32_t)((d.sd->nbits + 7u) >> 3); r->err = (int32_t)d.sd->err;
             r->loop_i = c.i; r->loop_t = c.t; r->loop_converge = c.converge; r->pad = 0;
         }
+        if (tid >= 33 && tid < 36) { r->cell_lo[tid - 33] = d.sd->cell_lo[tid - 33]; r->cell_hi[tid - 33] = d.sd->cell_hi[tid - 33]; }
         __threadfence_system();
         EK_SYNC();
         if (tid == 0) *reinterpret_cast<volatile uint32_t*>(&r->seq) = d.seq;
diff --git a/lidar-slam-detection_amd/csrc/voxelgrid.hip b/lidar-slam-detection_amd/csrc/voxelgrid.hip
--- a/lidar-slam-detection_amd/csrc/voxelgrid.hip
+++ b/lidar-slam-detection_amd/csrc/voxelgrid.hip
@@ -6,6 +6,9 @@
 constexpr int kItems = 8;
 constexpr int kTile = kThreads * kItems;
 constexpr int kWaves = kThreads / 64;
+#ifndef LIO_HIST_COPIES
+#define LIO_HIST_COPIES 1
+#endif
 
 __device__ __forceinline__ void vg_bbox_atomic_body(const float4* __restrict__ in, uint32_t n, ScanDev* sd) {
     float mn0 = INFINITY, mn1 = INFINITY, mn2 = INFINITY, mx0 = -INFINITY, mx1 = -INFINITY, mx2 = -INFINITY;
@@ -109,7 +112,7 @@
 }
 
 struct VgGrid {
-    int minb[3];
+    int minb[3], maxb[3];
     int mul1, mul2;
     uint32_t total;
     uint32_t pass;
@@ -120,6 +123,7 @@
     g.pass = 0;
     if (n_valid == 0) {
         g.minb[0] = g.minb[1] = g.minb[2] = 0;
+        g.maxb[0] = g.maxb[1] = g.maxb[2] = -1;
         g.mul1 = g.mul2 = 0;
         g.total = 0;
         return g;
@@ -132,7 +136,8 @@
     long long divb[3];
     for (int a = 0; a < 3; a++) {
         g.minb[a] = (int)floorf(mn[a] * inv);
-        divb[a] = (long long)((int)floorf(mx[a] * inv)) - g.minb[a] + 1;
+        g.maxb[a] = (int)floorf(mx[a] * inv);
+        divb[a] = (long long)g.maxb[a] - g.minb[a] + 1;
     }
     const long long total = divb[0] * divb[1] * divb[2];
     if (dx * dy * dz > 2147483647LL || total > 0xFFFFFFF0LL) g.pass = 1;
@@ -204,6 +209,8 @@
         sd->nbits = g.total ? (32 - __clz(g.total)) : 0;
         sd->minb[0] = g.minb[0]; sd->minb[1] = g.minb[1]; sd->minb[2] = g.minb[2];
         sd->mul1 = g.mul1; sd->mul2 = g.mul2;
+        if (!FOLD)
+            for (int a = 0; a < 3; a++) { sd->cell_lo[a] = g.minb[a]; sd->cell_hi[a] = g.maxb[a]; }
     }
 #pragma unroll
     for (int r = 0; r < kItems; r++) {
@@ -223,6 +230,89 @@
     hist[bx * 256u + threadIdx.x] = h[threadIdx.x];
 }
 
+__device__ __forceinline__ void vg_keys_pred_body(const float4* __restrict__ in, uint32_t n, float inv, ScanDev* sd, const int32_t* __restrict__ box_min,
+                                                  const int32_t* __restrict__ box_div, uint32_t* __restrict__ keys, uint32_t* __restrict__ hist, uint32_t bx) {
+    const uint32_t base = bx * kTile;
+    float4 p[kItems];
+#pragma unroll
+    for (int r = 0; r < kItems; r++) {
+        const uint32_t i = base + r * kThreads + threadIdx.x;
+        if (i < n) p[r] = in[i];
+    }
+    __shared__ uint32_t h[256];
+    __shared__ float red[kWaves][6];
+    __shared__ uint32_t redc[kWaves], redo[kWaves];
+    h[threadIdx.x] = 0;
+    const int minb0 = box_min[0], minb1 = box_min[1], minb2 = box_min[2];
+    const uint32_t div0 = (uint32_t)box_div[0], div1 = (uint32_t)box_div[1], div2 = (uint32_t)box_div[2];
+    const uint32_t mul1 = div0, mul2 = div0 * div1, total = mul2 * div2;
+    if (bx == 0 && threadIdx.x == 0) {
+        sd->n_ds_prev = sd->cache_n;
+        sd->passthrough = 0;
+        sd->total_cells = total;
+        sd->nbits = 32 - __clz(total);
+        sd->minb[0] = minb0; sd->minb[1] = minb1; sd->minb[2] = minb2;
+        sd->mul1 = (int)mul1; sd->mul2 = (int)mul2;
+    }
+    __syncthreads();
+    const float fmin0 = (float)minb0, fmin1 = (float)minb1, fmin2 = (float)minb2;
+    const float fdiv0 = (float)div0, fdiv1 = (float)div1, fdiv2 = (float)div2;
+    float mn0 = INFINITY, mn1 = INFINITY, mn2 = INFINITY, mx0 = -INFINITY, mx1 = -INFINITY, mx2 = -INFINITY;
+    uint32_t cnt = 0, outside = 0;
+#pragma unroll
+    for (int r = 0; r < kItems; r++) {
+        const uint32_t i = base + r * kThreads + threadIdx.x;
+        if (i >= n) continue;
+        uint32_t key = total;
+        if (isfinite(p[r].x) && isfinite(p[r].y) && isfinite(p[r].z)) {
+            mn0 = fminf(mn0, p[r].x); mx0 = fmaxf(mx0, p[r].x);
+            mn1 = fminf(mn1, p[r].y); mx1 = fmaxf(mx1, p[r].y);
+            mn2 = fminf(mn2, p[r].z); mx2 = fmaxf(mx2, p[r].z);
+            cnt++;
+            const float f0 = floorf(p[r].x * inv) - fmin0, f1 = floorf(p[r].y * inv) - fmin1, f2 = floorf(p[r].z * inv) - fmin2;
+            if (f0 >= 0.f && f0 < fdiv0 && f1 >= 0.f && f1 < fdiv1 && f2 >= 0.f && f2 < fdiv2)
+                key = (uint32_t)(int)f0 + (uint32_t)(int)f1 * mul1 + (uint32_t)(int)f2 * mul2;
+            else
+                outside = 1u;
+        }
+        keys[i] = key;
+        atomicAdd(&h[key & 255u], 1u);
+    }
+#pragma unroll
+    for (int off = 32; off > 0; off >>= 1) {
+        mn0 = fminf(mn0, __shfl_xor(mn0, off)); mx0 = fmaxf(mx0, __shfl_xor(mx0, off));
+        mn1 = fminf(mn1, __shfl_xor(mn1, off)); mx1 = fmaxf(mx1, __shfl_xor(mx1, off));
+        mn2 = fminf(mn2, __shfl_xor(mn2, off)); mx2 = fmaxf(mx2, __shfl_xor(mx2, off));
+        cnt += __shfl_xor(cnt, off);
+    }
+    const uint32_t wave_out = __ballot(outside != 0u) != 0ull ? 1u : 0u;
+    const int wave = threadIdx.x >> 6, lane = threadIdx.x & 63;
+    if (lane == 0) {
+        red[wave][0] = mn0; red[wave][1] = mn1; red[wave][2] = mn2;
+        red[wave][3] = mx0; red[wave][4] = mx1; red[wave][5] = mx2;
+        redc[wave] = cnt;
+        redo[wave] = wave_out;
+    }
+    __syncthreads();
+    hist[bx * 256u + threadIdx.x] = h[threadIdx.x];
+    if (threadIdx.x == 0) {
+        uint32_t any_out = wave_out;
+        for (int w = 1; w < kWaves; w++) {
+            mn0 = fminf(mn0, red[w][0]); mn1 = fminf(mn1, red[w][1]); mn2 = fminf(mn2, red[w][2]);
+            mx0 = fmaxf(mx0, red[w][3]); mx1 = fmaxf(mx1, red[w][4]); mx2 = fmaxf(mx2, red[w][5]);
+            cnt += redc[w];
+            any_out |= redo[w];
+        }
+        if (cnt > 0) {
+            atomicMin(&sd->bbox_min[0], f2ord(mn0)); atomicMax(&sd->bbox_max[0], f2ord(mx0));
+            atomicMin(&sd->bbox_min[1], f2ord(mn1)); atomicMax(&sd->bbox_max[1], f2ord(mx1));
+            atomicMin(&sd->bbox_min[2], f2ord(mn2)); atomicMax(&sd->bbox_max[2], f2ord(mx2));
+            atomicAdd(&sd->n_valid, cnt);
+        }
+        if (any_out) atomicOr(&sd->err, kErrBoxMiss);
+    }
+}
+
 __device__ inline uint32_t active_passes(const ScanDev* sd) { return (sd->nbits + 7u) >> 3; }
 
 __device__ __forceinline__ void radix_hist_body(const uint32_t* __restrict__ ka, const uint32_t* __restrict__ kb, uint32_t n,
@@ -231,7 +321,9 @@
     uint32_t nbits_w = sd->nbits;
     const uint32_t* keys = (pass & 1) ? kb : ka;
     const int shift = pass * 8;
-    __shared__ uint32_t h[256];
+    constexpr int kCopies = LIO_HIST_COPIES;
+    __shared__ uint32_t hh[kCopies * 257];
+    uint32_t* h = hh + (threadIdx.x & (kCopies - 1)) * 257;
     const uint32_t base = bx * kTile;
     uint4 kq[kItems / 4];
 #pragma unroll
@@ -243,7 +335,8 @@
 #pragma unroll
     for (int r = 0; r < kItems / 4; r++) pin_loaded(kq[r]);
     if ((uint32_t)pass >= ((nbits_w + 7u) >> 3)) return;
-    h[threadIdx.x] = 0;
+#pragma unroll
+    for (int c = 0; c < kCopies; c++) hh[c * 257 + threadIdx.x] = 0;
     __syncthreads();
 #pragma unroll
     for (int r = 0; r < kItems / 4; r++) {
@@ -259,7 +352,10 @@
         }
     }
     __syncthreads();
-    hist[bx * 256u + threadIdx.x] = h[threadIdx.x];
+    uint32_t sum = 0;
+#pragma unroll
+    for (int c = 0; c < kCopies; c++) sum += hh[c * 257 + threadIdx.x];
+    hist[bx * 256u + threadIdx.x] = sum;
 }
 
 template <bool PREFIXED>
@@ -431,6 +527,10 @@
             if (i < n) out[i] = in[i];
         }
         if (bx == 0 && tid == 0) { sd->n_ds = n; host_nds[0] = n; host_nds[1] = 0u; }
+        return;
+    }
+    if (sd->err & kErrBoxMiss) {
+        if (bx == last_block && tid == 0) { sd->n_ds = 0; host_nds[0] = 0; host_nds[1] = kErrBoxMiss; host_nds[2] = active_passes(sd); }
         return;
     }
     const uint32_t act = active_passes(sd);
@@ -819,6 +919,13 @@
     if (!d.active || bx >= d.nblocks) return;
     vg_keys_body<false>(d.raw, d.n_raw, inv, d.sd, d.keys_a, d.hist, d.nblocks, nullptr, bx);
 }
+__global__ void __launch_bounds__(kThreads) vg_keys_pred_batch(const SlotDesc* __restrict__ slots, float inv) {
+    uint32_t slot, bx;
+    vg_slot_tile(gridDim.y, slot, bx);
+    const SlotDesc& d = slots[slot];
+    if (!d.active || bx >= d.nblocks) return;
+    vg_keys_pred_body(d.raw, d.n_raw, inv, d.sd, d.box_min, d.box_div, d.keys_a, d.hist, bx);
+}
 __global__ void __launch_bounds__(kThreads) radix_hist_kernel(const uint32_t* __restrict__ ka, const uint32_t* __restrict__ kb, uint32_t n,
                                                               int pass, uint32_t* __restrict__ hist, uint32_t nblocks, const ScanDev* sd) {
     radix_hist_body(ka, kb, n, pass, hist, nblocks, sd);
@@ -842,9 +949,17 @@
     if (!d.active || bx >= d.nblocks) return;
     radix_scatter_body<true>(d.keys_a, d.vals_a, d.keys_b, d.vals_b, d.n_raw, pass, d.hist, d.nblocks, d.sd, bx);
 }
-__global__ void __launch_bounds__(256) radix_prefix_batch(const SlotDesc* __restrict__ slots, int pass) {
+__global__ void __launch_bounds__(256) radix_prefix_batch(const SlotDesc* __restrict__ slots, int pass, float inv) {
     const SlotDesc& d = slots[blockIdx.x];
     if (!d.active) return;
+    if (inv != 0.f && threadIdx.x == 0) {
+        ScanDev* sd = d.sd;
+        uint32_t bmin[3], bmax[3];
+        for (int a = 0; a < 3; a++) { bmin[a] = sd->bbox_min[a]; bmax[a] = sd->bbox_max[a]; }
+        const VgGrid g = vg_derive(bmin, bmax, sd->n_valid, inv);
+        for (int a = 0; a < 3; a++) { sd->cell_lo[a] = g.minb[a]; sd->cell_hi[a] = g.maxb[a]; }
+        if (g.pass) atomicOr(&sd->err, kErrBoxMiss);
+    }
     if ((uint32_t)pass >= active_passes(d.sd)) return;
     const uint32_t nb = d.nblocks;
     uint32_t* col = d.hist + threadIdx.x;
@@ -944,16 +1059,20 @@
     return LIO_OK;
 }
 
-int vg_downsample_batch(hipStream_t st, const SlotDesc* d_slots, int n_slots, uint32_t max_raw, uint32_t max_ds, float leaf, int passes) {
+int vg_downsample_batch(hipStream_t st, const SlotDesc* d_slots, int n_slots, uint32_t max_raw, uint32_t max_ds, float leaf, int passes, int predicted_box) {
     const float inv = 1.0f / leaf;
     const uint32_t nblocks = (max_raw + kTile - 1) / kTile;
     if (nblocks == 0 || n_slots <= 0) return LIO_OK;
     const uint32_t B = (uint32_t)n_slots;
-    hipLaunchKernelGGL(vg_bbox_batch, dim3(nblocks < 48 ? nblocks : 48, B), kThreads, 0, st, d_slots);
-    hipLaunchKernelGGL(vg_keys_batch, dim3(nblocks, B), kThreads, 0, st, d_slots, inv);
+    if (predicted_box) {
+        hipLaunchKernelGGL(vg_keys_pred_batch, dim3(nblocks, B), kThreads, 0, st, d_slots, inv);
+    } else {
+        hipLaunchKernelGGL(vg_bbox_batch, dim3(nblocks < 48 ? nblocks : 48, B), kThreads, 0, st, d_slots);
+        hipLaunchKernelGGL(vg_keys_batch, dim3(nblocks, B), kThreads, 0, st, d_slots, inv);
+    }
     for (int pass = 0; pass < passes; pass++) {
         if (pass > 0) hipLaunchKernelGGL(radix_hist_batch, dim3(nblocks, B), kThreads, 0, st, d_slots, pass);
-        hipLaunchKernelGGL(radix_prefix_batch, dim3(B), 256, 0, st, d_slots, pass);
+        hipLaunchKernelGGL(radix_prefix_batch, dim3(B), 256, 0, st, d_slots, pass, (predicted_box && pass == 0) ? inv : 0.f);
         hipLaunchKernelGGL(radix_scatter_batch, dim3(nblocks, B), kThreads, 0, st, d_slots, pass);
     }
     hipLaunchKernelGGL(vg_count_heads_batch, dim3(nblocks, B), kThreads, 0, st, d_slots);
diff --git a/lidar-slam-detection_amd/python/lsd_amd/capi.py b/lidar-slam-detection_amd/python/lsd_amd/capi.py
--- a/lidar-slam-detection_amd/python/lsd_amd/capi.py
+++ b/lidar-slam-detection_amd/python/lsd_amd/capi.py
@@ -22,7 +22,7 @@
     "lio_engine_create", "lio_engine_create_shared", "lio_engine_destroy", "lio_engine_map", "lio_engine_scan", "lio_engine_set_state", "lio_engine_get_state",
     "lio_engine_set_cov", "lio_engine_get_cov", "lio_engine_set_flags", "lio_engine_travel", "lio_engine_is_degenerate",
     "lio_engine_update", "lio_engine_pass_log", "lio_engine_process_scan", "lio_engine_process_scan_device", "lio_engine_timings", "lio_engine_flush",
-    "lio_engine_enable_timing", "lio_comm_unique_id", "lio_comm_init", "lio_comm_destroy", "lio_comm_rank", "lio_comm_world", "lio_allgather_normal_eq", "lio_comm_stats", "lio_engine_set_joint", "lio_engine_joint_register", "lio_engine_joint_register_device", "lio_allgather_records", "lio_engines_process_batch", "lio_batch_create", "lio_batch_create_joint", "lio_batch_create_sequences", "lio_batch_sequences_step", "lio_batch_fastlio_main", "lio_batch_set_gather_hook", "lio_batch_exchange_stats", "lio_batch_destroy", "lio_batch_process", "lio_batch_engine", "lio_batch_enable_kernel_timing", "lio_batch_kernel_times", "lio_engine_set_static_map", "lio_scan_enable_kernel_timing", "lio_scan_kernel_times",
+    "lio_engine_enable_timing", "lio_comm_unique_id", "lio_comm_init", "lio_comm_destroy", "lio_comm_rank", "lio_comm_world", "lio_allgather_normal_eq", "lio_comm_stats", "lio_engine_set_joint", "lio_engine_joint_register", "lio_engine_joint_register_device", "lio_allgather_records", "lio_engines_process_batch", "lio_batch_create", "lio_batch_create_joint", "lio_batch_create_sequences", "lio_batch_sequences_step", "lio_batch_fastlio_main", "lio_batch_set_gather_hook", "lio_batch_exchange_stats", "lio_batch_destroy", "lio_batch_process", "lio_batch_engine", "lio_batch_enable_kernel_timing", "lio_batch_kernel_times", "lio_box_union", "lio_box_decide", "lio_batch_set_box_prediction", "lio_batch_box_stats", "lio_engine_set_static_map", "lio_scan_enable_kernel_timing", "lio_scan_kernel_times",
     "lio_state_boxplus", "lio_state_boxminus",
     "lio_localmap_create", "lio_localmap_destroy", "lio_localmap_add_keyframe", "lio_localmap_num_keyframes", "lio_localmap_update",
     "lio_localmap_download",
@@ -401,6 +401,10 @@
     sig("lio_batch_engine", vp, vp, cint, cint)
     sig("lio_batch_enable_kernel_timing", cint, vp, cint)
     sig("lio_batch_kernel_times", cint, vp, C.POINTER(BatchTimes), cint)
+    sig("lio_box_union", None, i32p, i32p, cint)
+    sig("lio_box_decide", cint, i32p, cint, cint, i32p, i32p)
+    sig("lio_batch_set_box_prediction", cint, vp, cint, i32p, i32p)
+    sig("lio_batch_box_stats", cint, vp, C.POINTER(u64), C.POINTER(u64), C.POINTER(u64))
     sig("lio_engine_set_static_map", cint, vp, cint)
     sig("lio_localmap_create", vp, cint, u64, u32, u32)
     sig("lio_localmap_destroy", None, vp)
diff --git a/lidar-slam-detection_amd/python/lsd_amd/lio.py b/lidar-slam-detection_amd/python/lsd_amd/lio.py
--- a/lidar-slam-detection_amd/python/lsd_amd/lio.py
+++ b/lidar-slam-detection_amd/python/lsd_amd/lio.py
@@ -1788,6 +1788,30 @@
     def process(self, jobs):
         return process_batch(None, jobs, batch=self)
 
+    def set_box_prediction(self, mode, minb=None, divb=None):
+        mn = np.ascontiguousarray(minb if minb is not None else [0, 0, 0], dtype=np.int32).reshape(3)
+        dv = np.ascontiguousarray(divb if divb is not None else [0, 0, 0], dtype=np.int32).reshape(3)
+        check(lib().lio_batch_set_box_prediction(self.h, int(mode), ptr(mn, C.c_int32), ptr(dv, C.c_int32)), "set_box_prediction")
+
+    def box_stats(self):
+        a, p, m = C.c_uint64(0), C.c_uint64(0), C.c_uint64(0)
+        check(lib().lio_batch_box_stats(self.h, C.byref(a), C.byref(p), C.byref(m)))
+        return {"rounds_exact": a.value, "rounds_predicted": p.value, "scans_flagged": m.value}
+
+
+def box_union(state, cells):
+    st = np.array(state, dtype=np.int32).reshape(7)
+    c = np.ascontiguousarray(cells, dtype=np.int32).reshape(-1, 6)
+    lib().lio_box_union(ptr(st, C.c_int32), ptr(c, C.c_int32), len(c))
+    return st
+
+
+def predict_box(state, passes, drop=True):
+    st = np.array(state, dtype=np.int32).reshape(7)
+    mn, dv = np.zeros(3, np.int32), np.zeros(3, np.int32)
+    use = lib().lio_box_decide(ptr(st, C.c_int32), int(passes), int(bool(drop)), ptr(mn, C.c_int32), ptr(dv, C.c_int32))
+    return bool(use), mn, dv, st
+
 
 JOB_KEEP_CACHE = 1
 JOB_IDLE = 2
```

Result: faster. 6.222 billion (median of 5 runs) (+1.5%).
